# jlk9/MPAS-Ocean.jl

Hardware: AMD Instinct MI355X
Metric: cell-updates/sec per RK4 step (higher is better)
Workload: dtype f64

## Files before the change

### include/moka_hip.h

```cpp
#ifndef MOKA_HIP_H
#define MOKA_HIP_H
#include <stdint.h>

#ifdef __cplusplus
extern "C" {
#endif

typedef struct moka_ctx   moka_ctx;
typedef struct moka_plan  moka_plan;
typedef struct moka_mesh  moka_mesh;
typedef struct moka_state moka_state;

typedef enum {
    MOKA_OK = 0,
    MOKA_ERR_ARG = -1,
    MOKA_ERR_HIP = -2,
    MOKA_ERR_NO_DEVICE = -3,
    MOKA_ERR_ALLOC = -4,
    MOKA_ERR_UNSUPPORTED = -5,
    MOKA_ERR_COMM = -6
} moka_status;

typedef enum {
    MOKA_ORDER_DEFAULT = 0,
    MOKA_ORDER_NONE = 1,
    MOKA_ORDER_RCM = 2,
    MOKA_ORDER_RCB = 3
} moka_ordering;

typedef struct moka_mesh_desc {
    int32_t nCells, nEdges, nVertices;
    int32_t maxEdges, maxEdges2, vertexDegree;
    int32_t nVertLevels;
    int32_t edgeSignOnVertexLD;
    const double  *xCell, *yCell, *zCell;
    const int32_t *nEdgesOnCell;
    const int32_t *edgesOnCell;
    const int32_t *edgeSignOnCell;
    const double  *areaCell;
    const int32_t *cellsOnEdge;
    const int32_t *verticesOnEdge;
    const int32_t *nEdgesOnEdge;
    const int32_t *edgesOnEdge;
    const double  *weightsOnEdge;
    const double  *dvEdge, *dcEdge, *fEdge;
    const int32_t *edgesOnVertex;
    const int32_t *cellsOnVertex;
    const int32_t *edgeSignOnVertex;
    const double  *areaTriangle;
    const int32_t *maxLevelEdgeTop;
    const double  *restingThicknessSum;
    int32_t ordering;
    int32_t patch_cells;
    const int32_t *cellClass;
    int32_t stateBytes;
    const double *kiteAreasOnVertex;
    const double *fVertex;
} moka_mesh_desc;

typedef struct moka_mesh_info {
    int32_t nCells, nEdges, nVertices, nVertLevels;
    int32_t ordering, patch_cells, nPatches;
    int32_t maxEdgesUsed, maxEdges2Used;
    int32_t lanesPerColumn;
    int64_t meshBytesDevice;
    int64_t cellBandwidth;
    int32_t maxPatchRows;
    int32_t ldsBytesPerBlock;
    int32_t maxPatchCells, maxPatchEdges;
} moka_mesh_info;

enum { MOKA_CELL = 0, MOKA_EDGE = 1, MOKA_VERTEX = 2 };

typedef enum {
    MOKA_F_SSH = 0,
    MOKA_F_NORMAL_VELOCITY = 1,
    MOKA_F_LAYER_THICKNESS = 2,
    MOKA_F_LAYER_THICKNESS_EDGE = 3,
    MOKA_F_THICKNESS_FLUX = 4,
    MOKA_F_VELOCITY_DIV_CELL = 5,
    MOKA_F_RELATIVE_VORTICITY = 6,
    MOKA_F_TEND_NORMAL_VELOCITY = 7,
    MOKA_F_TEND_LAYER_THICKNESS = 8
} moka_field;

#define MOKA_FE_STALE_HEDGE      1
#define MOKA_FE_ACCUM_VORT       2
#define MOKA_FE_LEVEL1_ONLY      4
#define MOKA_FE_REFERENCE_COMPAT 7

typedef enum { MOKA_FORWARD_EULER = 0, MOKA_RUNGE_KUTTA_4 = 1 } moka_integrator;

const char *moka_version(void);
int  moka_ctx_create(int device, moka_ctx **out);
void moka_ctx_destroy(moka_ctx *ctx);
const char *moka_last_error(const moka_ctx *ctx);
int  moka_sync(moka_ctx *ctx);
int  moka_timer_start(moka_ctx *ctx);
int  moka_timer_stop(moka_ctx *ctx, float *elapsed_ms);

int  moka_plan_create(const moka_mesh_desc *desc, moka_plan **out);
void moka_plan_destroy(moka_plan *plan);
int  moka_plan_info(const moka_plan *plan, moka_mesh_info *info);
int  moka_plan_permutation(const moka_plan *plan, int kind, int32_t *new_to_old);
int  moka_plan_patch_ranges(const moka_plan *plan, int32_t *cellStart, int32_t *edgeStart, int32_t *vertexStart);
int  moka_plan_class_ranges(const moka_plan *plan, int32_t capacity, int32_t *nClasses, int32_t *patchStart,
                            int32_t *cellStart, int32_t *edgeStart);

enum {
    MOKA_PA_EOC = 0, MOKA_PA_COC, MOKA_PA_MLTC, MOKA_PA_SDV, MOKA_PA_INVAREA, MOKA_PA_AREACELL, MOKA_PA_RSUM,
    MOKA_PA_EHDR, MOKA_PA_EOE, MOKA_PA_WOE, MOKA_PA_GINVDC, MOKA_PA_DCEDGE, MOKA_PA_DVEDGE, MOKA_PA_FEDGE,
    MOKA_PA_EOV, MOKA_PA_CV, MOKA_PA_HALO_START, MOKA_PA_HALO_EDGE, MOKA_PA_LEOC, MOKA_PA_LEOE,
    MOKA_PA_CREC, MOKA_PA_EREC, MOKA_PA_FEOE, MOKA_PA_PVSTART, MOKA_PA_PVLIST, MOKA_PA_LVOE,
    MOKA_PA_NLEV
};
int  moka_plan_array(const moka_plan *plan, int which, const void **data, int64_t *count);

int  moka_mesh_create(moka_ctx *ctx, const moka_mesh_desc *desc, moka_mesh **out);
void moka_mesh_destroy(moka_mesh *mesh);
int  moka_mesh_info_get(const moka_mesh *mesh, moka_mesh_info *info);

int moka_gradient_on_edge(moka_mesh *mesh, const double *scalarCell, double *gradEdge);
int moka_divergence_on_cell(moka_mesh *mesh, const double *vecEdge, double *tempEdge, double *divCell);
int moka_curl_on_vertex(moka_mesh *mesh, const double *vecEdge, double *curlVertex);
int moka_interpolate_cell2edge(moka_mesh *mesh, const double *cellValue, double *edgeValue, int nlev);

int moka_gradient_on_edge_vjp(moka_mesh *mesh, double *dGradEdge , double *dScalarCell );
int moka_gradient_on_edge_jvp(moka_mesh *mesh, const double *dScalarCell, double *dGradEdge);
int moka_divergence_on_cell_vjp(moka_mesh *mesh, double *dDivCell , double *dVecEdge ,
                                double *dTempEdge );
int moka_divergence_on_cell_jvp(moka_mesh *mesh, const double *dVecEdge, double *dTempEdge , double *dDivCell);
int moka_curl_on_vertex_vjp(moka_mesh *mesh, const double *dCurlVertex, double *dVecEdge );
int moka_curl_on_vertex_jvp(moka_mesh *mesh, const double *dVecEdge, double *dCurlVertex );

int  moka_state_create(moka_ctx *ctx, moka_mesh *mesh, moka_state **out);
void moka_state_destroy(moka_state *st);
int  moka_state_upload(moka_state *st, int field, int time_level, const double *host);
int  moka_state_download(moka_state *st, int field, int time_level, double *host);

int  moka_state_download_rows(moka_state *st, int field, int time_level, int64_t nRows, const int32_t *rows, double *host);

int  moka_state_array_address(moka_state *st, int field, int time_level, uint64_t *address);

int  moka_state_optimize_placement(moka_state *st, int max_tries, double *ms_before, double *ms_after);
typedef struct { int32_t field; double ms_old, ms_new; int32_t kept; } moka_placement_trial;
int  moka_state_placement_log(const moka_state *st, int32_t capacity, moka_placement_trial *out, int32_t *n);
int64_t moka_state_placement_launches(const moka_state *st);

int moka_advance_time_levels(moka_state *st, int flags);
int moka_diagnostic_compute(moka_state *st, int flags);
int moka_compute_normal_velocity_tendency(moka_state *st, int flags);
int moka_compute_layer_thickness_tendency(moka_state *st, int flags);
int moka_tendencies(moka_state *st);
int moka_step_fe(moka_state *st, double dt, int flags);
int moka_step_rk4(moka_state *st, double dt);
int moka_run(moka_state *st, int integrator, double dt, int64_t nsteps, int flags);
int moka_sum_sq(moka_state *st, int field, int time_level, double *out);

typedef struct moka_halo moka_halo;
int  moka_ctx_streams(moka_ctx *ctx, void **compute_stream, void **comm_stream);
int  moka_mesh_permutation(const moka_mesh *mesh, int kind, int32_t *new_to_old);
int  moka_mesh_class_ranges(const moka_mesh *mesh, int32_t capacity, int32_t *nClasses, int32_t *patchStart,
                            int32_t *cellStart, int32_t *edgeStart);
int  moka_halo_create(moka_state *st, int32_t nNeighbors, const int32_t *sendCells, const int64_t *sendCellOff,
                      const int32_t *sendEdges, const int64_t *sendEdgeOff, const int32_t *recvCells,
                      const int64_t *recvCellOff, const int32_t *recvEdges, const int64_t *recvEdgeOff,
                      int32_t nPatchesBoundary, int32_t nPatchesOwned, moka_halo **out);
void moka_halo_destroy(moka_halo *h);
int  moka_halo_buffer_elems(const moka_halo *h, int64_t *sendElems, int64_t *recvElems);
int  moka_halo_pack(moka_halo *h, int what, void *sendbuf_device);
int  moka_halo_unpack(moka_halo *h, int what, const void *recvbuf_device);

typedef struct {
    unsigned char ipc[15][64];
    uint64_t ptr[15];
    uint64_t flagPtr;
    char     shmName[64];
    int32_t  dstCell, dstEdge;
    int32_t  nCells, nEdges;
    int32_t  slot;
    int32_t  nNeighbors, pid, device, stateBytes, nVertLevels;
} moka_halo_peer_info;
int  moka_halo_set_overlap(moka_halo *h, int mode);
int  moka_halo_set_acquire(moka_halo *h, int on);
int  moka_halo_pack_fields(moka_halo *h, const void *uField, const void *hField, const void *sField, void *sendbuf);
int  moka_halo_unpack_fields(moka_halo *h, void *uField, void *hField, void *sField, const void *recvbuf);
int  moka_halo_direct_available(const moka_halo *h);
int  moka_halo_export(moka_halo *h, int32_t nbr, int32_t shared, moka_halo_peer_info *out);
int  moka_halo_connect(moka_halo *h, int32_t nbr, const moka_halo_peer_info *peer, int32_t shared);
int  moka_halo_push_begin(moka_halo *h, int what);
int  moka_halo_push_signal(moka_halo *h);
int  moka_halo_push_wait(moka_halo *h, double timeout_s);

int  moka_halo_set_stream_flags(moka_halo *h, int on);

typedef struct {
    int64_t steps, exchanges, boundary_launches, interior_launches;
    double host_step_ms, host_signal_wait_ms, host_flag_store_ms, host_wait_ms, boundary_launch_ms, interior_launch_ms;
} moka_halo_stats;
int  moka_halo_stats_enable(moka_halo *h, int on);
int  moka_halo_stats_read(moka_halo *h, moka_halo_stats *out);

int  moka_rk4_dist_begin(moka_halo *h, double dt);
int  moka_rk4_dist_stage(moka_halo *h, int stage, int part);
int  moka_rk4_dist_parts_available(const moka_halo *h);
int  moka_rk4_dist_stage_launch(moka_halo *h, int stage);
int  moka_rk4_dist_end(moka_halo *h);
typedef int (*moka_transport_fn)(void *user, int what, void *sendbuf_device, void *recvbuf_device);
int  moka_rk4_dist_step(moka_halo *h, double dt, moka_transport_fn transport, void *user, void *sendbuf_device,
                        void *recvbuf_device, double timeout_s);
int  moka_fe_dist_launch(moka_halo *h, double dt, int flags, int part);
int  moka_fe_dist_end(moka_halo *h);
int  moka_fe_dist_step(moka_halo *h, double dt, int flags, moka_transport_fn transport, void *user, void *sendbuf_device,
                       void *recvbuf_device, double timeout_s);

int moka_kernel_variant_available(int variant);
int moka_set_kernel_variant(moka_ctx *ctx, int variant);
int moka_set_tuning(int key, int value);
int moka_get_tuning(int key, int *value);
int moka_state_rk4_streams(const moka_state *st);
int moka_stage_timing(moka_ctx *ctx, int enable);
int moka_stage_timing_read(moka_ctx *ctx, double ms[4], int64_t *steps);
int moka_ctx_pci_bus_id(moka_ctx *ctx, char *buf, int32_t len);
int moka_mark(moka_ctx *ctx);
int moka_marks_reset(moka_ctx *ctx);
int moka_marks_read(moka_ctx *ctx, int64_t capacity, double *ms, int64_t *n);
int moka_bw_probe(moka_ctx *ctx, int64_t bytes, int iters, double gbs[4]);
int moka_bw_probe_streams(moka_ctx *ctx, int iters, double *gbs);
int moka_bw_probe_reread(moka_ctx *ctx, int64_t region, int reps, int iters, double *gbs);
int moka_bw_probe_gather_big(moka_ctx *ctx, int64_t bytes, int iters, double *gbs);
int moka_last_fe_path(const moka_state *st);
int moka_fe_lazy_pending(const moka_state *st);

int  moka_set_nonlinear(moka_state *st, int on);
int  moka_set_viscosity_del2(moka_state *st, double viscDel2);
int  moka_set_viscosity_del4(moka_state *st, double viscDel4, const double *meshScalingDel4);
int  moka_state_del4_path(const moka_state *st);

int  moka_set_tracers(moka_state *st, int32_t nTracers);
int  moka_tracer_upload(moka_state *st, int32_t j, int time_level, const double *host);
int  moka_tracer_download(moka_state *st, int32_t j, int time_level, double *host);
int  moka_state_tracer_path(const moka_state *st);
int  moka_set_tracer_diffusion(moka_state *st, const double *kappa);
int  moka_tracer_diffusion(const moka_state *st, int32_t j, double *out);
int  moka_set_tracer_biharmonic(moka_state *st, const double *kappa4);
int  moka_tracer_biharmonic(const moka_state *st, int32_t j, double *out);
int  moka_tracer_source_upload(moka_state *st, int32_t j, const double *host);
int  moka_tracer_source_download(moka_state *st, int32_t j, double *host);
int  moka_tracer_has_source(const moka_state *st, int32_t j, int *out);
int  moka_set_tracer_vertical_diffusion(moka_state *st, const double *kappaV);
int  moka_tracer_vertical_diffusion(const moka_state *st, int32_t j, double *out);
int  moka_state_tracer_vmix_path(const moka_state *st);
int  moka_tracer_vertical_field_upload(moka_state *st, int32_t j, const double *host);
int  moka_tracer_vertical_field_download(moka_state *st, int32_t j, double *host);
int  moka_tracer_has_vertical_field(const moka_state *st, int32_t j, int *out);

int  moka_set_vertical_viscosity(moka_state *st, double nuV, double bottomDrag);
int  moka_vertical_viscosity(const moka_state *st, double *nuV, double *bottomDrag);
int  moka_surface_stress_upload(moka_state *st, const double *host);
int  moka_surface_stress_download(moka_state *st, double *host);
int  moka_has_surface_stress(const moka_state *st, int *out);
int  moka_state_momentum_vmix_path(const moka_state *st);

typedef struct moka_tracer_tape moka_tracer_tape;
int  moka_tracer_tape_create(moka_state *st, int64_t capacity_steps, moka_tracer_tape **out);
void moka_tracer_tape_destroy(moka_tracer_tape *t);
int  moka_step_rk4_tracer_taped(moka_tracer_tape *t, double dt);
int  moka_tracer_tape_steps(const moka_tracer_tape *t, int64_t *n);
int  moka_tracer_adjoint_seed(moka_tracer_tape *t, int32_t j, const double *host);
int  moka_tracer_adjoint_sweep(moka_tracer_tape *t);
int  moka_tracer_adjoint_download(moka_tracer_tape *t, int32_t j, double *host);
int  moka_tracer_adjoint_path(const moka_tracer_tape *t);
int  moka_tracer_adjoint_vmix_path(const moka_tracer_tape *t);
int  moka_tracer_adjoint_want_source_gradient(moka_tracer_tape *t, int32_t j, int on);
int  moka_tracer_adjoint_source_download(moka_tracer_tape *t, int32_t j, double *host);
enum { MOKA_TRACER_GRAD_KAPPA = 1, MOKA_TRACER_GRAD_KAPPA4 = 2 };
int  moka_tracer_adjoint_want_diffusivity_gradient(moka_tracer_tape *t, int32_t j, int what, int on);
int  moka_tracer_adjoint_diffusivity_gradient(moka_tracer_tape *t, int32_t j, int what, double *out);
int  moka_tracer_adjoint_diffusivity_density_download(moka_tracer_tape *t, int32_t j, int what, double *host);
int  moka_tracer_adjoint_want_vertical_gradient(moka_tracer_tape *t, int32_t j, int on);
int  moka_tracer_adjoint_vertical_gradient(moka_tracer_tape *t, int32_t j, double *out);
enum { MOKA_VGRAD_INTERFACE = 0, MOKA_VGRAD_CELL = 1, MOKA_VGRAD_PROFILE = 2 };
int  moka_tracer_adjoint_vertical_density_download(moka_tracer_tape *t, int32_t j, int view, double *host);

typedef struct moka_tape moka_tape;
int  moka_tape_create(moka_state *st, int64_t capacity_steps, moka_tape **out);
void moka_tape_destroy(moka_tape *t);
int  moka_step_fe_taped(moka_tape *t, double dt, int flags);
int  moka_step_rk4_taped(moka_tape *t, double dt);
int  moka_adjoint_seed_sum_sq_ssh(moka_tape *t);
int  moka_adjoint_sweep(moka_tape *t);
int  moka_tape_record_rk4(moka_tape *t, int slot, int what);
int  moka_tape_commit_rk4(moka_tape *t, double dt);
int  moka_adjoint_rk4_stage_fields(moka_tape *t, int stage, void **fieldU, void **fieldH, void **scratchS);
int  moka_adjoint_rk4_stage(moka_tape *t, int stage);
int  moka_adjoint_rk4_stage_part(moka_tape *t, int stage, int part);
int  moka_adjoint_rk4_parts_available(const moka_tape *t);
int  moka_adjoint_rk4_stage_out_fields(moka_tape *t, int stage, void **fieldU, void **fieldH, void **scratchS);
int  moka_tape_record_fe(moka_tape *t, int flags, int after);
int  moka_tape_commit_fe(moka_tape *t, double dt, int flags);
int  moka_adjoint_fe_step_fields(moka_tape *t, void **fieldU, void **fieldH, void **fieldS);
int  moka_adjoint_fe_step(moka_tape *t);
int  moka_adjoint_download(moka_tape *t, int field, double *host);

#ifdef __cplusplus
}
#endif
#endif
```

### mpas-ocean.jl_amd/csrc/api.hip

```cpp
#include <hip/hip_runtime.h>

#include <algorithm>
#include <atomic>
#include <climits>
#include <cmath>
#include <cstdio>
#include <cstdlib>
#include <cstring>
#include <map>
#include <mutex>
#include <new>
#include <string>
#include <unordered_set>
#include <utility>
#include <vector>

#include <mutex>
#include <unordered_set>

#include "state.hpp"

namespace moka {

void fill_mesh_info(const Plan &p, moka_mesh_info *info);

struct TuningEntry {
    int mask, max;
    std::atomic<int> value;
    TuningEntry(int def, int m, int x) : mask(m), max(x), value(def) {}
    bool accepts(int v) const { return mask ? (v & ~mask) == 0 : v >= 0 && v <= max; }
};
static TuningEntry g_tuning[] = {
    {0, 0, -1},
    {1 << 0, 0x7f | 1 << 10 | 1 << 11, 0},
    {1, 0, 1},
    {1, 0, 1},
    {1, 0, 1},
    {0, 0, 3},
    {0, 0, INT_MAX},
    {0, 0, 1},
    {1 << 0 | 1 << 1 | 1 << 7, 0xf | 7 << 7 | 1 << 16, 0},
    {1, 0, 1},
};
constexpr int N_TUNING = sizeof(g_tuning) / sizeof(g_tuning[0]);

int tuning(TuningKey key) { return g_tuning[key].value.load(); }

}

namespace mk {

static std::mutex g_liveMutex;
static std::unordered_set<const moka_state *> g_liveStates;
void state_attach(moka_state *st, bool halo)
{
    std::lock_guard<std::mutex> lk(g_liveMutex);
    if (g_liveStates.count(st)) { ++st->attached; st->halos += halo; }
}
void state_detach(moka_state *st, bool halo)
{
    std::lock_guard<std::mutex> lk(g_liveMutex);
    if (g_liveStates.count(st)) { --st->attached; st->halos -= halo; }
}

int fail(moka_ctx *ctx, int code, const std::string &msg)
{
    set_error(msg);
    if (ctx) ctx->err = msg;
    return code;
}

int lanes_per_column(int K)
{
    int l = 1;
    while (l < K && l < 64) l <<= 1;
    return l;
}

int h2d(moka_ctx *ctx, void *dst, const void *src, size_t bytes)
{
    if (!bytes) return MOKA_OK;
    HIPCHK(ctx, hipMemcpyAsync(dst, src, bytes, hipMemcpyHostToDevice, ctx->stream));
    HIPCHK(ctx, hipStreamSynchronize(ctx->stream));
    return MOKA_OK;
}

template <class T>
int upload_vec(moka_mesh *m, const std::vector<T> &v, const T **out)
{
    void *d = nullptr;
    const size_t bytes = std::max<size_t>(v.size() * sizeof(T), 16);
    HIPCHK(m->ctx, hipMalloc(&d, bytes));
    m->allocs.push_back(d);
    if (int rc = h2d(m->ctx, d, v.data(), v.size() * sizeof(T))) return rc;
    *out = static_cast<const T *>(d);
    return MOKA_OK;
}

int ensure_op_bufs(moka_mesh *m)
{
    const Plan &p = m->plan;
    const size_t need = (size_t)p.K * std::max(p.nE, std::max(p.nC, p.nV));
    if (m->opBufElems >= need) return MOKA_OK;
    for (auto &b : m->opBuf) {
        if (b) HIPCHK(m->ctx, hipFree(b));
        b = nullptr;
    }
    for (auto &b : m->opBuf) HIPCHK(m->ctx, hipMalloc((void **)&b, need * sizeof(double)));
    m->opBufElems = need;
    return MOKA_OK;
}

int alloc_field(moka_state *st, double **out, size_t elems, size_t elemBytes)
{
    void *d = nullptr;
    HIPCHK(st->ctx, hipMalloc(&d, std::max<size_t>(elems * elemBytes, 16)));
    st->allocs.push_back(d);
    HIPCHK(st->ctx, hipMemsetAsync(d, 0, elems * elemBytes, st->ctx->stream));
    *out = static_cast<double *>(d);
    return MOKA_OK;
}

int ensure_rk_bufs(moka_state *st)
{
    if (st->rk[1].ssh) return MOKA_OK;
    const Plan &p = st->mesh->plan;
    LevelBufs tmp[2];
    const size_t mark = st->allocs.size();
    const size_t sb = st->f32 ? 4 : 8;
    int rc = MOKA_OK;
    for (auto &r : tmp) {
        if (rc == MOKA_OK) rc = alloc_field(st, &r.u, (size_t)p.K * p.nE, sb);
        if (rc == MOKA_OK) rc = alloc_field(st, &r.h, (size_t)p.K * p.nC, sb);
        if (rc == MOKA_OK) rc = alloc_field(st, &r.ssh, (size_t)p.nC, sb);
    }
    if (rc != MOKA_OK) {
        (void)hipStreamSynchronize(st->ctx->stream);
        while (st->allocs.size() > mark) { (void)hipFree(st->allocs.back()); st->allocs.pop_back(); }
        return rc;
    }
    st->rk[0] = tmp[0]; st->rk[1] = tmp[1];
    st->phys[2] = tmp[0]; st->phys[3] = tmp[1];
    return MOKA_OK;
}

int ensure_spare(moka_state *st)
{
    if (st->spare.ssh) return MOKA_OK;
    const Plan &p = st->mesh->plan;
    LevelBufs tmp;
    const size_t mark = st->allocs.size();
    const size_t sb = st->f32 ? 4 : 8;
    int rc = alloc_field(st, &tmp.u, (size_t)p.K * p.nE, sb);
    if (rc == MOKA_OK) rc = alloc_field(st, &tmp.h, (size_t)p.K * p.nC, sb);
    if (rc == MOKA_OK) rc = alloc_field(st, &tmp.ssh, (size_t)p.nC, sb);
    if (rc != MOKA_OK) {
        (void)hipStreamSynchronize(st->ctx->stream);
        while (st->allocs.size() > mark) { (void)hipFree(st->allocs.back()); st->allocs.pop_back(); }
        return rc;
    }
    st->spare = tmp;
    st->phys[4] = tmp;
    return MOKA_OK;
}

LevelBufs &fe_new_level(moka_state *st) { return st->spare.ssh ? st->spare : st->lev[0]; }

void fe_rotate_levels(moka_state *st)
{
    if (st->spare.ssh) {
        const LevelBufs oldPrev = st->lev[0];
        st->lev[0] = st->lev[1];
        st->lev[1] = st->spare;
        st->spare = oldPrev;
    } else {
        std::swap(st->lev[0], st->lev[1]);
    }
}

struct FieldRef {
    double *ptr;
    int kind;
    int64_t n;
    int K;
    bool f32 = false;
};

int field_ref(moka_state *st, int field, int level, FieldRef *r)
{
    const Plan &p = st->mesh->plan;
    if (level != 0 && level != 1) return fail(st->ctx, MOKA_ERR_ARG, "time_level must be 0 (previous) or 1 (current)");
    switch (field) {
        case MOKA_F_SSH: *r = {st->lev[level].ssh, MOKA_CELL, p.nC, 1}; break;
        case MOKA_F_NORMAL_VELOCITY: *r = {st->lev[level].u, MOKA_EDGE, p.nE, p.K}; break;
        case MOKA_F_LAYER_THICKNESS: *r = {st->lev[level].h, MOKA_CELL, p.nC, p.K}; break;
        case MOKA_F_LAYER_THICKNESS_EDGE: *r = {st->hEdge[0], MOKA_EDGE, p.nE, p.K}; break;
        case MOKA_F_THICKNESS_FLUX: *r = {st->F, MOKA_EDGE, p.nE, p.K}; break;
        case MOKA_F_VELOCITY_DIV_CELL: *r = {st->div, MOKA_CELL, p.nC, p.K}; break;
        case MOKA_F_RELATIVE_VORTICITY: *r = {st->vort, MOKA_VERTEX, p.nV, p.K}; break;
// ... 365 lines not shown
    ctx->marksUsed = 0;
    return MOKA_OK;
}

int moka_marks_read(moka_ctx *ctx, int64_t capacity, double *ms, int64_t *n)
{
    if (!ctx || !n || (capacity > 0 && !ms)) return fail(ctx, MOKA_ERR_ARG, "NULL argument");
    HIPCHK(ctx, hipStreamSynchronize(ctx->stream));
    const int64_t have = ctx->marksUsed > 0 ? (int64_t)ctx->marksUsed - 1 : 0;
    *n = have;
    for (int64_t i = 0; i < have && i < capacity; ++i) {
        float t = 0.f;
        HIPCHK(ctx, hipEventElapsedTime(&t, ctx->marks[i], ctx->marks[i + 1]));
        ms[i] = t;
    }
    return MOKA_OK;
}

int moka_bw_probe(moka_ctx *ctx, int64_t bytes, int iters, double gbs[4])
{
    if (!ctx) return fail(nullptr, MOKA_ERR_ARG, "ctx is NULL");
    HIPCHK(ctx, hipSetDevice(ctx->device));
    if (bytes <= 0) {
        HIPCHK(ctx, hipStreamSynchronize(ctx->stream));
        if (ctx->bwBuf) HIPCHK(ctx, hipFree(ctx->bwBuf));
        ctx->bwBuf = nullptr; ctx->bwBytes = 0;
        return MOKA_OK;
    }
    if (!gbs || iters < 1) return fail(ctx, MOKA_ERR_ARG, "gbs is NULL or iters < 1");
    const size_t half = ((size_t)bytes / 2) & ~(size_t)4095;
    if (half < ((size_t)1 << 20)) return fail(ctx, MOKA_ERR_ARG, "bandwidth probe: at least 2 MiB");
    hipStream_t s = ctx->stream;
    if (ctx->bwBytes != 2 * half) {
        if (ctx->bwBuf) { HIPCHK(ctx, hipStreamSynchronize(s)); HIPCHK(ctx, hipFree(ctx->bwBuf)); ctx->bwBuf = nullptr; ctx->bwBytes = 0; }
        hipError_t e = hipMalloc(&ctx->bwBuf, 2 * half + 64);
        if (e != hipSuccess) return fail(ctx, MOKA_ERR_ALLOC, std::string("bandwidth probe: hipMalloc: ") + hipGetErrorString(e));
        ctx->bwBytes = 2 * half;
        HIPCHK(ctx, hipMemsetAsync(ctx->bwBuf, 0x5A, 2 * half + 64, s));
    }
    unsigned char *a = static_cast<unsigned char *>(ctx->bwBuf), *b = a + half;
    uint32_t *sink = reinterpret_cast<uint32_t *>(a + 2 * half);
    double bestCopy = 0.0, bestRead = 0.0, sumCopy = 0.0, bestGather = 0.0;
    const uint32_t rowB = 480;
    for (int pass = 0; pass < 3; ++pass)
        for (int i = 0; i < iters; ++i) {
            HIPCHK(ctx, hipEventRecord(ctx->ev0, s));
            if (pass == 0) HIPCHK(ctx, launch_bw_copy(b, a, (int64_t)half, ctx->nCUs, s));
            else if (pass == 1) HIPCHK(ctx, launch_bw_read(a, (int64_t)(2 * half), sink, ctx->nCUs, s));
            else HIPCHK(ctx, launch_bw_gather(a, (int64_t)(2 * half), rowB, sink, ctx->nCUs, s));
            HIPCHK(ctx, hipEventRecord(ctx->ev1, s));
            HIPCHK(ctx, hipEventSynchronize(ctx->ev1));
            float ms = 0.f;
            HIPCHK(ctx, hipEventElapsedTime(&ms, ctx->ev0, ctx->ev1));
            const double r = (double)(2 * half) / ((double)ms * 1e-3) / 1e9;
            if (pass == 0) { bestCopy = std::max(bestCopy, r); sumCopy += r; }
            else if (pass == 1) bestRead = std::max(bestRead, r);
            else bestGather = std::max(bestGather, (double)((2 * half) / rowB * rowB) / ((double)ms * 1e-3) / 1e9);
        }
    gbs[0] = bestCopy; gbs[1] = bestRead; gbs[2] = sumCopy / iters; gbs[3] = bestGather;
    return MOKA_OK;
}

int moka_bw_probe_streams(moka_ctx *ctx, int iters, double *gbs)
{
    if (!ctx || !gbs || iters < 1) return fail(ctx, MOKA_ERR_ARG, "NULL argument or iters < 1");
    if (!ctx->bwBuf || ctx->bwBytes < ((size_t)5 << 20)) return fail(ctx, MOKA_ERR_ARG, "moka_bw_probe first: it owns the buffer");
    HIPCHK(ctx, hipSetDevice(ctx->device));
    hipStream_t s = ctx->stream;
    const int64_t n = (int64_t)(ctx->bwBytes / 5 / 16);
    double best = 0.0;
    for (int i = 0; i < iters; ++i) {
        HIPCHK(ctx, hipEventRecord(ctx->ev0, s));
        HIPCHK(ctx, launch_bw_streams(ctx->bwBuf, (int64_t)ctx->bwBytes, s));
        HIPCHK(ctx, hipEventRecord(ctx->ev1, s));
        HIPCHK(ctx, hipEventSynchronize(ctx->ev1));
        float ms = 0.f;
        HIPCHK(ctx, hipEventElapsedTime(&ms, ctx->ev0, ctx->ev1));
        best = std::max(best, (double)(5 * 16 * n) / ((double)ms * 1e-3) / 1e9);
    }
    HIPCHK(ctx, hipMemsetAsync(ctx->bwBuf, 0x5A, ctx->bwBytes + 64, s));
    *gbs = best;
    return MOKA_OK;
}

int moka_bw_probe_reread(moka_ctx *ctx, int64_t region, int reps, int iters, double *gbs)
{
    if (!ctx || !gbs || iters < 1 || reps < 1) return fail(ctx, MOKA_ERR_ARG, "NULL argument or iters / reps < 1");
    if (!ctx->bwBuf || region < ((int64_t)1 << 20) || (size_t)region > ctx->bwBytes) return fail(ctx, MOKA_ERR_ARG, "moka_bw_probe first: it owns the buffer (region must fit it)");
    HIPCHK(ctx, hipSetDevice(ctx->device));
    hipStream_t s = ctx->stream;
    unsigned char *a = static_cast<unsigned char *>(ctx->bwBuf);
    uint32_t *sink = reinterpret_cast<uint32_t *>(a + ctx->bwBytes);
    region &= ~(int64_t)4095;
    double best = 0.0;
    HIPCHK(ctx, launch_bw_read(a, region, sink, ctx->nCUs, s));
    for (int i = 0; i < iters; ++i) {
        HIPCHK(ctx, hipEventRecord(ctx->ev0, s));
        for (int r = 0; r < reps; ++r) HIPCHK(ctx, launch_bw_read(a, region, sink, ctx->nCUs, s));
        HIPCHK(ctx, hipEventRecord(ctx->ev1, s));
        HIPCHK(ctx, hipEventSynchronize(ctx->ev1));
        float ms = 0.f;
        HIPCHK(ctx, hipEventElapsedTime(&ms, ctx->ev0, ctx->ev1));
        best = std::max(best, (double)region * reps / ((double)ms * 1e-3) / 1e9);
    }
    *gbs = best;
    return MOKA_OK;
}

int moka_bw_probe_gather_big(moka_ctx *ctx, int64_t bytes, int iters, double *gbs)
{
    if (!ctx || !gbs || iters < 1 || bytes < ((int64_t)1 << 24)) return fail(ctx, MOKA_ERR_ARG, "NULL argument, iters < 1 or less than 16 MiB");
    HIPCHK(ctx, hipSetDevice(ctx->device));
    hipStream_t s = ctx->stream;
    void *buf = nullptr;
    hipError_t e = hipMalloc(&buf, (size_t)bytes + 64);
    if (e != hipSuccess) return fail(ctx, MOKA_ERR_ALLOC, std::string("big gather probe: hipMalloc: ") + hipGetErrorString(e));
    const uint32_t rowB = 480;
    const int64_t nRows = bytes / rowB, nFetch = nRows / 4;
    uint32_t *sink = reinterpret_cast<uint32_t *>(static_cast<unsigned char *>(buf) + bytes);
    double best = 0.0;
    hipError_t rc = hipMemsetAsync(buf, 0x5A, (size_t)bytes + 64, s);
    for (int i = 0; i < iters && rc == hipSuccess; ++i) {
        if ((rc = hipEventRecord(ctx->ev0, s)) != hipSuccess) break;
        if ((rc = launch_bw_gather_n(buf, nRows, rowB, nFetch, sink, ctx->nCUs, s)) != hipSuccess) break;
        if ((rc = hipEventRecord(ctx->ev1, s)) != hipSuccess) break;
        if ((rc = hipEventSynchronize(ctx->ev1)) != hipSuccess) break;
        float ms = 0.f;
        if ((rc = hipEventElapsedTime(&ms, ctx->ev0, ctx->ev1)) != hipSuccess) break;
        best = std::max(best, (double)nFetch * rowB / ((double)ms * 1e-3) / 1e9);
    }
    (void)hipStreamSynchronize(s);
    (void)hipFree(buf);
    HIPCHK(ctx, rc);
    *gbs = best;
    return MOKA_OK;
}

int moka_set_tuning(int key, int value)
{
    if (key < 1 || key >= N_TUNING) return fail(nullptr, MOKA_ERR_ARG, "unknown tuning key");
    if (!g_tuning[key].accepts(value)) return fail(nullptr, MOKA_ERR_ARG, "tuning key " + std::to_string(key) + ": value names no kernel instance");
    g_tuning[key].value.store(value);
    return MOKA_OK;
}

int moka_get_tuning(int key, int *value)
{
    if (!value) return fail(nullptr, MOKA_ERR_ARG, "value is NULL");
    if (key < 1 || key >= N_TUNING) return fail(nullptr, MOKA_ERR_ARG, "unknown tuning key");
    *value = g_tuning[key].value.load();
    return MOKA_OK;
}

int moka_kernel_variant_available(int variant)
{
    return variant == 0 || variant == 3 || variant == 4 || variant == 11;
}

int moka_set_kernel_variant(moka_ctx *ctx, int variant)
{
    if (!ctx) return fail(nullptr, MOKA_ERR_ARG, "ctx is NULL");
    if (variant < 0 || variant > 14) return fail(ctx, MOKA_ERR_ARG, "variant must be 0..14");
    if (!moka_kernel_variant_available(variant))
        return fail(ctx, MOKA_ERR_UNSUPPORTED, "this kernel variant was an experiment of rounds 1-3 and no longer exists (0, 3, 4, 11 do)");
    ctx->variant = variant;
    return MOKA_OK;
}

int moka_mesh_create(moka_ctx *ctx, const moka_mesh_desc *desc, moka_mesh **out)
{
    if (!ctx || !out) return fail(ctx, MOKA_ERR_ARG, "NULL argument");
    *out = nullptr;
    moka_mesh *m = new (std::nothrow) moka_mesh();
    if (!m) return fail(ctx, MOKA_ERR_ALLOC, "out of host memory");
    m->ctx = ctx;
    int rc;
    try {
        rc = build_plan(desc, m->plan);
    } catch (const std::bad_alloc &) {
        rc = fail(ctx, MOKA_ERR_ALLOC, "out of host memory while building the mesh plan");
    }
    if (rc != MOKA_OK) {
        ctx->err = moka::get_error();
        delete m;
        return rc;
    }
    const Plan &p = m->plan;
    if (p.ME > 8 || p.ME2 > 14) {
        delete m;
        return fail(ctx, MOKA_ERR_UNSUPPORTED, "cells with more than 8 edges are not supported by the gfx950 kernels");
    }
    HIPCHK(ctx, hipSetDevice(ctx->device));
    MeshDev &d = m->dev;
    d.nC = p.nC; d.nE = p.nE; d.nV = p.nV; d.K = p.K; d.ME = p.ME; d.ME2 = p.ME2; d.VD = p.VD; d.nPatches = p.nPatches;
    d.tailPatch = -1;
    m->lpc = lanes_per_column(p.K);
#define UP(field)                                                \
    if ((rc = upload_vec(m, p.field, &d.field)) != MOKA_OK) {    \
        moka_mesh_destroy(m);                                    \
        return rc;                                               \
    }
    UP(patchCellStart) UP(patchEdgeStart) UP(patchVertStart)
    UP(eoc) UP(coc) UP(mltc) UP(sdv) UP(invArea) UP(areaCell) UP(rsum)
    UP(ehdr) UP(eoe) UP(woe) UP(gInvDc) UP(dcEdge) UP(dvEdge) UP(fEdge)
    UP(eov) UP(cv) UP(cellN2O) UP(edgeN2O) UP(vertN2O)
    UP(leoe) UP(cRec) UP(eRec) UP(feoe) UP(vRec) UP(rowStart) UP(rowEdge)
    if (p.nlOk) { UP(voe) UP(cov) UP(kite) UP(invAreaTri) UP(fVertex) UP(keCoef) UP(invDc) UP(keoc) UP(rowVoe) }
    if (p.nl5Ok) { UP(pvStart) UP(pvList) UP(lvoe) }
#undef UP
    d.maxPV = p.nl5Ok ? p.maxPV : 0;
    if (!p.nl5Ok) { d.pvStart = nullptr; d.pvList = nullptr; d.lvoe = nullptr; }
    d.CI = p.CI; d.EI = p.EI;
    m->colOk = p.colOk;

    d.maxRows = p.maxRows; d.maxOwnE = p.maxOwnE; d.maxOwnC = p.maxOwnC;
    d.maxOwnV = p.maxOwnV;
    if (p.vRec.empty()) d.vRec = nullptr;
    *out = m;
    return MOKA_OK;
}

void moka_mesh_destroy(moka_mesh *mesh)
{
    if (!mesh) return;
    (void)hipSetDevice(mesh->ctx->device);
    (void)hipStreamSynchronize(mesh->ctx->stream);
    for (void *q : mesh->allocs) (void)hipFree(q);
    for (auto b : mesh->opBuf)
        if (b) (void)hipFree(b);
    delete mesh;
}

int moka_mesh_permutation(const moka_mesh *mesh, int kind, int32_t *new_to_old)
{
    if (!mesh || !new_to_old) return fail(nullptr, MOKA_ERR_ARG, "NULL argument");
    const Plan &p = mesh->plan;
    const std::vector<int32_t> *v = kind == MOKA_CELL ? &p.cellN2O : kind == MOKA_EDGE ? &p.edgeN2O : kind == MOKA_VERTEX ? &p.vertN2O : nullptr;
    if (!v) return fail(mesh->ctx, MOKA_ERR_ARG, "kind must be MOKA_CELL, MOKA_EDGE or MOKA_VERTEX");
    std::copy(v->begin(), v->end(), new_to_old);
    return MOKA_OK;
}

int moka_mesh_class_ranges(const moka_mesh *mesh, int32_t capacity, int32_t *nClasses, int32_t *patchStart, int32_t *cellStart,
                           int32_t *edgeStart)
{
    if (!mesh || !nClasses) return fail(nullptr, MOKA_ERR_ARG, "NULL argument");
    const Plan &p = mesh->plan;
    const int n = (int)p.classPatchStart.size() - 1;
    *nClasses = n;
    for (int k = 0; k <= n && k < capacity; ++k) {
        if (patchStart) patchStart[k] = p.classPatchStart[k];
        if (cellStart) cellStart[k] = p.classCellStart[k];
        if (edgeStart) edgeStart[k] = p.classEdgeStart[k];
    }
    return MOKA_OK;
}

int moka_mesh_info_get(const moka_mesh *mesh, moka_mesh_info *info)
{
    if (!mesh || !info) return fail(nullptr, MOKA_ERR_ARG, "NULL argument");
    fill_mesh_info(mesh->plan, info);
    return MOKA_OK;
}

static int run_operator(moka_mesh *m, int op, int nlev, const double *in, int inKind, double *out, int outKind,
                        bool out_is_inout)
{
    if (!m || !in || !out) return fail(m ? m->ctx : nullptr, MOKA_ERR_ARG, "NULL argument");
    const Plan &p = m->plan;
    auto count = [&](int kind) -> int64_t { return kind == MOKA_CELL ? p.nC : kind == MOKA_EDGE ? p.nE : p.nV; };
    int rc = ensure_op_bufs(m);
    if (rc) return rc;
    hipStream_t s = m->ctx->stream;
    HIPCHK(m->ctx, hipSetDevice(m->ctx->device));
    if ((rc = put_rows(m, m->opBuf[0], in, inKind, count(inKind), p.K))) return rc;
    if (out_is_inout) {
        if ((rc = put_rows(m, m->opBuf[1], out, outKind, count(outKind), p.K))) return rc;
    } else {
        if (op == OP_INTERP && nlev < p.K) {
            if ((rc = put_rows(m, m->opBuf[1], out, outKind, count(outKind), p.K))) return rc;
        }
    }
    OpArgs a{op, nlev, m->opBuf[0], m->opBuf[1]};
    HIPCHK(m->ctx, launch_operator(m->dev, a, m->lpc, s));
    return get_rows(m, out, m->opBuf[1], outKind, count(outKind), p.K);
}

int moka_gradient_on_edge(moka_mesh *mesh, const double *scalarCell, double *gradEdge)
{
    return run_operator(mesh, OP_GRADIENT, 0, scalarCell, MOKA_CELL, gradEdge, MOKA_EDGE, false);
}

int moka_interpolate_cell2edge(moka_mesh *mesh, const double *cellValue, double *edgeValue, int nlev)
{
    if (mesh && (nlev < 1 || nlev > mesh->plan.K)) return fail(mesh->ctx, MOKA_ERR_ARG, "nlev out of range");
    return run_operator(mesh, OP_INTERP, nlev, cellValue, MOKA_CELL, edgeValue, MOKA_EDGE, false);
}

int moka_curl_on_vertex(moka_mesh *mesh, const double *vecEdge, double *curlVertex)
{
    return run_operator(mesh, OP_CURL, 0, vecEdge, MOKA_EDGE, curlVertex, MOKA_VERTEX, true);
}

static int ensure_op_transposes(moka_mesh *m)
{
    if (m->opESign) return MOKA_OK;
    const Plan &p = m->plan;
    std::vector<std::vector<std::pair<std::pair<int32_t, int32_t>, int32_t>>> lists(p.nE);
    for (int v = 0; v < p.nV; ++v)
        for (int j = 0; j < p.VD; ++j) {
            const int e = p.eov[(size_t)v * p.VD + j];
            if (e >= 0) lists[e].push_back({{p.vertN2O[v], j}, v});
        }
    int W = 1;
    for (auto &l : lists) { std::sort(l.begin(), l.end()); W = std::max(W, (int)l.size()); }
    std::vector<int32_t> tv((size_t)p.nE * W, -1);
    std::vector<double> tc((size_t)p.nE * W, 0.0), es((size_t)p.nE * 2, 0.0);
    for (int e = 0; e < p.nE; ++e) {
        for (size_t q = 0; q < lists[e].size(); ++q) {
            const int v = lists[e][q].second, j = lists[e][q].first.second;
            tv[(size_t)e * W + q] = v;
            tc[(size_t)e * W + q] = p.cv[(size_t)v * p.VD + j];
        }
        for (int q = 0; q < 2; ++q) {
            const int c = p.ehdr[(size_t)e * 4 + q];
            for (int i = 0; i < p.ME; ++i)
                if (p.eoc[(size_t)c * p.ME + i] == e) { es[(size_t)e * 2 + q] = p.sdv[(size_t)c * p.ME + i] < 0.0 ? -1.0 : 1.0; break; }
        }
    }
    int rc;
    if ((rc = upload_vec(m, tv, &m->opTVert)) || (rc = upload_vec(m, tc, &m->opTCoef))) return rc;
    if ((rc = upload_vec(m, es, &m->opESign))) return rc;
    m->opTW = W;
    return MOKA_OK;
}

int moka_gradient_on_edge_vjp(moka_mesh *m, double *dGradEdge, double *dScalarCell)
{
    if (!m || !dGradEdge || !dScalarCell) return fail(m ? m->ctx : nullptr, MOKA_ERR_ARG, "NULL argument");
    const Plan &p = m->plan;
    int rc = ensure_op_bufs(m);
    if (rc) return rc;
    HIPCHK(m->ctx, hipSetDevice(m->ctx->device));
    if ((rc = put_rows(m, m->opBuf[0], dGradEdge, MOKA_EDGE, p.nE, p.K))) return rc;
    if ((rc = put_rows(m, m->opBuf[1], dScalarCell, MOKA_CELL, p.nC, p.K))) return rc;
    OpArgs a{OP_GRAD_T, 0, m->opBuf[0], m->opBuf[1]};
    HIPCHK(m->ctx, launch_operator(m->dev, a, m->lpc, m->ctx->stream));
    if ((rc = get_rows(m, dScalarCell, m->opBuf[1], MOKA_CELL, p.nC, p.K))) return rc;
    std::memset(dGradEdge, 0, sizeof(double) * (size_t)p.K * p.nE);
    return MOKA_OK;
}

int moka_gradient_on_edge_jvp(moka_mesh *m, const double *dScalarCell, double *dGradEdge)
{
    return moka_gradient_on_edge(m, dScalarCell, dGradEdge);
}

int moka_divergence_on_cell_vjp(moka_mesh *m, double *dDivCell, double *dVecEdge, double *dTempEdge)
{
    if (!m || !dDivCell || !dVecEdge) return fail(m ? m->ctx : nullptr, MOKA_ERR_ARG, "NULL argument");
    const Plan &p = m->plan;
    int rc = ensure_op_bufs(m);
    if (rc) return rc;
    HIPCHK(m->ctx, hipSetDevice(m->ctx->device));
    if ((rc = ensure_op_transposes(m))) return rc;
    if ((rc = put_rows(m, m->opBuf[0], dDivCell, MOKA_CELL, p.nC, p.K))) return rc;
    if ((rc = put_rows(m, m->opBuf[1], dVecEdge, MOKA_EDGE, p.nE, p.K))) return rc;
    if (dTempEdge && (rc = put_rows(m, m->opBuf[3], dTempEdge, MOKA_EDGE, p.nE, p.K))) return rc;
    OpArgs a{OP_DIV_T, 0, m->opBuf[0], m->opBuf[1]};
    a.in2 = dTempEdge ? m->opBuf[3] : nullptr;
// ... 2286 lines not shown
```

### mpas-ocean.jl_amd/csrc/kernels.hip

```cpp
#include <mutex>
#include <set>
#include <utility>

#include "kernels_common.hpp"

namespace moka {


template <int ME, int ME2, int MODE, int NT = BLOCK>
__global__ __launch_bounds__(NT) void k_stage_rec2c(const ColMesh m, const StageArgs a, int maxOwnE, int maxOwnC)
{
    extern __shared__ __align__(16) unsigned char smem[];
    const int pl_ = patch_of_block(m.nPatches);
    if (pl_ >= m.nPatches) return;
    const int p = m.pairEnd ? m.patchBegin + 2 * pl_ : (m.tailPlus1 && pl_ == m.nPatches - 1) ? m.tailPlus1 - 1 : pl_ + m.patchBegin;
    const int pEnd = m.pairEnd ? (p + 2 < m.pairEnd ? p + 2 : m.pairEnd) : p + 1;
    constexpr int NG = NT / 32;
    const int tid = threadIdx.x;
    const int grp = tid >> 5, l = tid & 31;
    const int K = m.K, K2 = K >> 1;
    const uint32_t voff = (uint32_t)l * 16u, rowB = (uint32_t)K * 8u;
    const RecLds L = rec_carve(smem, m, ME, ME2, maxOwnE, maxOwnC);
    const size_t recBytes = ((size_t)maxOwnE * (2 * ME2 + 1) * 8 + (size_t)maxOwnC * (ME + 2) * 8 +
                             ((size_t)maxOwnE * m.EI + (size_t)maxOwnC * m.CI) * 4 + 15) & ~(size_t)15;
    double2 *ubuf2 = reinterpret_cast<double2 *>(smem + recBytes);
    const unsigned char *ubytes = reinterpret_cast<const unsigned char *>(ubuf2) + voff;
    const int c0 = cptr(m.patchCellStart)[p], c1 = cptr(m.patchCellStart)[pEnd];
    const int e0 = cptr(m.patchEdgeStart)[p], e1 = cptr(m.patchEdgeStart)[pEnd];
    const int nOwnC = c1 - c0, nOwnE = e1 - e0;
    const uint32_t e0B = (uint32_t)e0 * rowB, nOwnB = (uint32_t)nOwnE * rowB;
    double *Lvw = reinterpret_cast<double *>(smem + recBytes + (size_t)maxOwnE * rowB);
    uint32_t *Lvo = reinterpret_cast<uint32_t *>(Lvw + (size_t)m.maxOwnV * 3);
    constexpr bool LEAN = MODE >= 10;
    constexpr int BASE = LEAN ? MODE - 5 : MODE;
    constexpr bool FE = BASE >= 4 && BASE <= 6, STALE = BASE == 4, PREV = BASE == 6;
    int v0 = 0, nOwnV = 0;
    if constexpr (FE) {
        if (a.vort) {
            v0 = cptr(m.patchVertStart)[p];
            nOwnV = cptr(m.patchVertStart)[p + 1] - v0;
        }
    }

    {
        const double2 *src = reinterpret_cast<const double2 *>(a.pu) + (size_t)e0 * K2;
        const int nU = nOwnE * K2, nER = nOwnE * m.EI, nW = nOwnE * ME2, nCR = nOwnC * m.CI, nS = nOwnC * ME;
        constexpr int UU = 6, UE = 3, UW = 2;
        double2 vU[UU];
        uint32_t vE[UE], vC;
        double vW[UW], vF[UW], vG, vS, vA, vR;
#pragma unroll
        for (int j = 0; j < UU; ++j) vU[j] = (tid + j * NT < nU) ? src[tid + j * NT] : make_double2(0.0, 0.0);
#pragma unroll
        for (int j = 0; j < UE; ++j) vE[j] = (tid + j * NT < nER) ? m.eRec[(size_t)e0 * m.EI + tid + j * NT] : 0u;
#pragma unroll
        for (int j = 0; j < UW; ++j) {
            vW[j] = (tid + j * NT < nW) ? m.woe[(size_t)e0 * ME2 + tid + j * NT] : 0.0;
            vF[j] = (tid + j * NT < nW) ? m.feoe[(size_t)e0 * ME2 + tid + j * NT] : 0.0;
        }
        vG = tid < nOwnE ? m.gInvDc[e0 + tid] : 0.0;
        vC = tid < nCR ? m.cRec[(size_t)c0 * m.CI + tid] : 0u;
        vS = tid < nS ? m.sdv[(size_t)c0 * ME + tid] : 0.0;
        vA = tid < nOwnC ? m.invArea[c0 + tid] : 0.0;
        vR = tid < nOwnC ? m.rsum[c0 + tid] : 0.0;
        uint32_t vVo = 0u;
        double vVw = 0.0;
        if constexpr (FE) {
            if (tid < nOwnV * 4) vVo = m.vRec[(size_t)v0 * 4 + tid];
            if (tid < nOwnV * 3) vVw = m.cv[(size_t)v0 * 3 + tid];
        }
#pragma unroll
        for (int j = 0; j < UU; ++j) if (tid + j * NT < nU) ubuf2[tid + j * NT] = vU[j];
#pragma unroll
        for (int j = 0; j < UE; ++j) if (tid + j * NT < nER) L.eRec[tid + j * NT] = vE[j];
#pragma unroll
        for (int j = 0; j < UW; ++j)
            if (tid + j * NT < nW) {
                L.woe[tid + j * NT] = vW[j];
                L.feoe[tid + j * NT] = vF[j];
            }
        if (tid < nOwnE) L.g[tid] = vG;
        if (tid < nCR) L.cRec[tid] = vC;
        if (tid < nS) L.sdv[tid] = vS;
        if (tid < nOwnC) {
            L.invA[tid] = vA;
            L.rsum[tid] = vR;
        }
        if constexpr (FE) {
            if (tid < nOwnV * 4) Lvo[tid] = vVo;
            if (tid < nOwnV * 3) Lvw[tid] = vVw;
            for (int i = tid + NT; i < nOwnV * 4; i += NT) Lvo[i] = m.vRec[(size_t)v0 * 4 + i];
            for (int i = tid + NT; i < nOwnV * 3; i += NT) Lvw[i] = m.cv[(size_t)v0 * 3 + i];
        }
        for (int i = tid + UU * NT; i < nU; i += NT) ubuf2[i] = src[i];
        for (int i = tid + UE * NT; i < nER; i += NT) L.eRec[i] = m.eRec[(size_t)e0 * m.EI + i];
        for (int i = tid + UW * NT; i < nW; i += NT) {
            L.woe[i] = m.woe[(size_t)e0 * ME2 + i];
            L.feoe[i] = m.feoe[(size_t)e0 * ME2 + i];
        }
        for (int i = tid + NT; i < nOwnE; i += NT) L.g[i] = m.gInvDc[e0 + i];
        for (int i = tid + NT; i < nCR; i += NT) L.cRec[i] = m.cRec[(size_t)c0 * m.CI + i];
        for (int i = tid + NT; i < nS; i += NT) L.sdv[i] = m.sdv[(size_t)c0 * ME + i];
        for (int i = tid + NT; i < nOwnC; i += NT) {
            L.invA[i] = m.invArea[c0 + i];
            L.rsum[i] = m.rsum[c0 + i];
        }
    }
    __syncthreads();

    const int k0 = 2 * l;
    const bool act = k0 < K;
    const lds_bytes_t ubytesL = (lds_bytes_t)ubytes;
    const glb_bytes_t puG = (glb_bytes_t)a.pu;
    const uint32_t ldsU = (uint32_t)(size_t)ubytesL;
    auto urow_addr = [&](uint32_t off, bool &cached) -> uint32_t {
        const uint32_t loc = off - e0B;
        cached = loc < nOwnB;
        return ldsU + (cached ? loc : 0u);
    };

    double2 pA = make_double2(0.0, 0.0), pB = pA, pD = pA, pE = pA;
    double pS = 0.0;
    uint32_t pOff = 0;
    int pC = 0;
    bool pend = false;
    auto flush_cell = [&]() {
        if (act) {
            if constexpr (MODE == 0) gstore2o(a.tendH, pOff, pA);
            if constexpr (MODE == 1 || MODE == 2) {
                gstore2o(a.ph_out, pOff, pA);
                gstore2o(a.nh_out, pOff, pB);
            }
            if constexpr (MODE == 3 || MODE == 9) gstore2o(a.nh_out, pOff, pB);
            if constexpr (MODE == 7 || MODE == 8) gstore2o(a.ph_out, pOff, pA);
            if constexpr (LEAN) gstore2o(a.ph_out, pOff, pA);
            if constexpr (FE && !LEAN) {
                if (a.ph_out) gstore2o(a.ph_out, pOff, pA);
                if (a.tendH) gstore2o(a.tendH, pOff, pB);
                if (a.div) gstore2o(a.div, pOff, pD);
            }
        }
        if constexpr (MODE != 0)
            if (l == 0 && (!FE || LEAN || a.ssh_out)) a.ssh_out[pC] = pS;
    };
#pragma nounroll
    for (int ci = grp; ci < nOwnC; ci += NG) {
        const int c = c0 + ci;
        const uint32_t *r = L.cRec + (size_t)ci * m.CI;
        const double *rs = L.sdv + (size_t)ci * ME;
        const uint32_t mask = r[2 * ME], all = r[2 * ME + 1];
        const double invA = L.invA[ci];
        const uint32_t own = (uint32_t)c * rowB + voff;
        double2 hc = make_double2(0.0, 0.0), uv[ME], hv[ME], cur = hc, nin = hc, hpc = hc, q3 = hc;
        if (act) {
            bool cached[ME];
            uint32_t ad[ME], goff[ME];
            v4u_t raw[ME];
            hc = gload2(a.ph, own);
            if constexpr (PREV) hpc = gload2(a.hPrev, own);
#pragma unroll
            for (int i = 0; i < ME; ++i) {
                const uint32_t off = r[i];
                hv[i] = STALE ? gload2(a.hEdgeOld, off + voff) : gload2(PREV ? a.hPrev : a.ph, r[ME + i] + voff);
                ad[i] = urow_addr(off, cached[i]);
                goff[i] = off + voff;
                asm("" : "+v"(goff[i]));
            }
            lds_burst<ME>(raw, ad);
#pragma unroll
            for (int i = 0; i < ME; ++i) {
                uv[i] = __builtin_bit_cast(double2, raw[i]);
                if (!cached[i]) uv[i] = glb_row2(puG + goff[i]);
            }
            if constexpr (MODE == 2 || MODE == 8 || MODE == 9) cur = gload2(a.ch, own);
            if constexpr (MODE == 2 || MODE == 3 || MODE == 9) nin = gload2(a.nh_in, own);
            if constexpr (MODE == 9) q3 = gload2(a.q3h, own);
        }
        double area = 1.0;
        if constexpr (FE && !LEAN) if (a.div) area = a.areaCell[c];
        __builtin_amdgcn_s_waitcnt(0x0F70);
        if (pend) flush_cell();
        double2 t = make_double2(0.0, 0.0);
        const bool plain = __builtin_amdgcn_ballot_w64(!(mask == (1u << ME) - 1u && all)) == 0;
        double2 dv = make_double2(0.0, 0.0);
        const double2 hself = PREV ? hpc : hc;
        auto hE = [&](int i) { return STALE ? hv[i] : make_double2(0.5 * (hself.x + hv[i].x), 0.5 * (hself.y + hv[i].y)); };
        if (plain) {
            if (act) {
#pragma unroll
                for (int i = 0; i < ME; ++i) {
                    const double2 he = hE(i);
                    t.x += uv[i].x * he.x * rs[i] * invA;
                    t.y += uv[i].y * he.y * rs[i] * invA;
                    if constexpr (FE && !LEAN) {
                        dv.x -= uv[i].x * rs[i];
                        dv.y -= uv[i].y * rs[i];
                    }
                }
            }
        } else if (act) {
#pragma unroll
            for (int i = 0; i < ME; ++i) {
                const int ml = all ? K : cptr(m.mltc)[(size_t)c * ME + i];
                const bool on = (mask >> i) & 1u;
                const double2 he = hE(i);
                const double dx = uv[i].x * he.x * rs[i] * invA;
                const double dy = uv[i].y * he.y * rs[i] * invA;
                if (on && k0 < ml) t.x += dx;
                if (on && k0 + 1 < ml) t.y += dy;
                if constexpr (FE && !LEAN) {
                    if (on) {
                        dv.x -= uv[i].x * rs[i];
                        dv.y -= uv[i].y * rs[i];
                    }
                }
            }
        }
        double2 hs = make_double2(0.0, 0.0);
        if (act) {
            if constexpr (MODE == 0) pA = t;
            if constexpr (MODE == 1 || MODE == 2) {
                const double2 hcur = MODE == 2 ? cur : hc;
                const double2 nb = MODE == 2 ? nin : hcur;
                hs = make_double2(hcur.x + a.a * t.x, hcur.y + a.a * t.y);
                pA = hs;
                pB = make_double2(nb.x + a.b * t.x, nb.y + a.b * t.y);
            }
            if constexpr (MODE == 3) {
                hs = make_double2(nin.x + a.b * t.x, nin.y + a.b * t.y);
                pB = hs;
            }
            if constexpr (MODE == 7 || MODE == 8) {
                const double2 hcur = MODE == 8 ? cur : hc;
                hs = make_double2(hcur.x + a.a * t.x, hcur.y + a.a * t.y);
                pA = hs;
            }
            if constexpr (MODE == 9) {
                hs = make_double2(rk13_combine(cur.x, nin.x, q3.x, hc.x, a.b, t.x), rk13_combine(cur.y, nin.y, q3.y, hc.y, a.b, t.y));
                pB = hs;
            }
            if constexpr (FE) {
                hs = make_double2(hc.x + a.a * t.x, hc.y + a.a * t.y);
                pA = hs;
                if constexpr (!LEAN) {
                    pB = t;
                    if (a.div) pD = make_double2(dv.x / area, dv.y / area);
                }
            }
        }
        if constexpr (MODE != 0) {
#pragma unroll
            for (int sft = 16; sft >= 1; sft >>= 1) {
                const double ox = __shfl_xor(hs.x, sft, 32), oy = __shfl_xor(hs.y, sft, 32);
                hs = make_double2(hs.x + ox, hs.y + oy);
            }
            pS = (hs.x + hs.y) - L.rsum[ci];
        }
        pOff = own;
        pC = c;
        pend = true;
    }
    if (pend) flush_cell();
    pend = false;
    auto flush_edge = [&]() {
        if (act) {
            if constexpr (MODE == 0) gstore2o(a.tendU, pOff, pA);
            if constexpr (MODE == 1 || MODE == 2) {
                gstore2o(a.pu_out, pOff, pA);
                gstore2o(a.nu_out, pOff, pB);
            }
            if constexpr (MODE == 3 || MODE == 9) gstore2o(a.nu_out, pOff, pB);
            if constexpr (MODE == 7 || MODE == 8) gstore2o(a.pu_out, pOff, pA);
            if constexpr (LEAN) gstore2o(a.pu_out, pOff, pA);
            if constexpr (FE && !LEAN) {
                if (a.pu_out) gstore2o(a.pu_out, pOff, pA);
                if (a.tendU) gstore2o(a.tendU, pOff, pB);
                if (a.F) gstore2o(a.F, pOff, pD);
                if (a.hEdgeNew) gstore2o(a.hEdgeNew, pOff, pE);
            }
        }
    };

#pragma nounroll
    for (int ei = grp; ei < nOwnE; ei += NG) {
        const int e = e0 + ei;
        const uint32_t *r = L.eRec + (size_t)ei * m.EI;
        const double *rw = L.woe + (size_t)ei * ME2;
        const double *rf = L.feoe + (size_t)ei * ME2;
        const uint32_t mask = r[ME2 + 2];
        const int mlt = (int)r[ME2 + 3];
        const double g = L.g[ei];
        const uint32_t own = (uint32_t)e * rowB + voff;
        double sv = 0.0;
        double2 uv[ME2], cur = make_double2(0.0, 0.0), nin = cur, hx = cur, hy = cur, hEo = cur, q3 = cur;
        if (act) {
            bool cached[ME2];
            uint32_t ad[ME2], goff[ME2];
            v4u_t raw[ME2];
#pragma unroll
            for (int i = 0; i < ME2; ++i) {
                const uint32_t off = r[i];
                ad[i] = urow_addr(off, cached[i]);
                goff[i] = off + voff;
                asm("" : "+v"(goff[i]));
            }
            lds_burst<ME2>(raw, ad);
#pragma unroll
            for (int i = 0; i < ME2; ++i) {
                uv[i] = __builtin_bit_cast(double2, raw[i]);
                if (!cached[i]) uv[i] = glb_row2(puG + goff[i]);
            }
            if constexpr (MODE == 2 || MODE == 8 || MODE == 9) cur = gload2(a.cu, own);
            if constexpr (MODE == 2 || MODE == 3 || MODE == 9) nin = gload2(a.nu_in, own);
            if constexpr (MODE == 9) q3 = gload2(a.q3u, own);
            if constexpr (FE && !LEAN) {
                if (a.hEdgeNew || (MODE == 5 && a.F)) {
                    hx = gload2(a.ph, r[ME2] * rowB + voff);
                    hy = gload2(a.ph, r[ME2 + 1] * rowB + voff);
                }
                if (a.F) {
                    if constexpr (STALE) hEo = gload2(a.hEdgeOld, own);
                    if constexpr (PREV) {
                        const double2 px = gload2(a.hPrev, r[ME2] * rowB + voff), py = gload2(a.hPrev, r[ME2 + 1] * rowB + voff);
                        hEo = make_double2(0.5 * (px.x + py.x), 0.5 * (px.y + py.y));
                    }
                }
            }
        }
        if (l < 2) sv = a.ssh[r[ME2 + l]];
        __builtin_amdgcn_s_waitcnt(0x0F70);
        if (pend) flush_edge();
        const double ds = __shfl(sv, 1, 32) - __shfl(sv, 0, 32);
        const bool plain = __builtin_amdgcn_ballot_w64(!(mask == (1u << ME2) - 1u && mlt >= K)) == 0;
        if (act) {
            const bool ax = k0 < mlt, ay = k0 + 1 < mlt;
            double2 t = make_double2(0.0, 0.0);
            if (plain) {
                t.x -= g * ds;
                t.y -= g * ds;
#pragma unroll
                for (int i = 0; i < ME2; ++i) {
                    t.x += rw[i] * uv[i].x * rf[i];
                    t.y += rw[i] * uv[i].y * rf[i];
                }
            } else {
                if (ax) t.x -= g * ds;
                if (ay) t.y -= g * ds;
#pragma unroll
                for (int i = 0; i < ME2; ++i) {
                    const bool on = (mask >> i) & 1u;
                    const double px = rw[i] * uv[i].x * rf[i], py = rw[i] * uv[i].y * rf[i];
                    if (on && ax) t.x += px;
                    if (on && ay) t.y += py;
                }
            }
            if constexpr (MODE == 0) pA = t;
            if constexpr (MODE == 1) {
                const double2 up = ubuf2[(size_t)ei * K2 + l];
                pA = make_double2(up.x + a.a * t.x, up.y + a.a * t.y);
                pB = make_double2(up.x + a.b * t.x, up.y + a.b * t.y);
            }
            if constexpr (MODE == 2) {
                pA = make_double2(cur.x + a.a * t.x, cur.y + a.a * t.y);
                pB = make_double2(nin.x + a.b * t.x, nin.y + a.b * t.y);
            }
            if constexpr (MODE == 3) pB = make_double2(nin.x + a.b * t.x, nin.y + a.b * t.y);
            if constexpr (MODE == 7) {
                const double2 up = ubuf2[(size_t)ei * K2 + l];
                pA = make_double2(up.x + a.a * t.x, up.y + a.a * t.y);
            }
            if constexpr (MODE == 8) pA = make_double2(cur.x + a.a * t.x, cur.y + a.a * t.y);
            if constexpr (MODE == 9) {
                const double2 up = ubuf2[(size_t)ei * K2 + l];
                pB = make_double2(rk13_combine(cur.x, nin.x, q3.x, up.x, a.b, t.x), rk13_combine(cur.y, nin.y, q3.y, up.y, a.b, t.y));
            }
            if constexpr (LEAN) {
                const double2 up = ubuf2[(size_t)ei * K2 + l];
                pA = make_double2(up.x + a.a * t.x, up.y + a.a * t.y);
            }
            if constexpr (FE && !LEAN) {
                const double2 up = ubuf2[(size_t)ei * K2 + l];
                pE = make_double2(0.5 * (hx.x + hy.x), 0.5 * (hx.y + hy.y));
                const double2 hF = (STALE || PREV) ? hEo : pE;
                pD = make_double2(up.x * hF.x, up.y * hF.y);
                pA = make_double2(up.x + a.a * t.x, up.y + a.a * t.y);
                pB = t;
            }
        }
        pOff = own;
        pend = true;
    }
    if (pend) flush_edge();

    if constexpr (FE) {
#pragma nounroll
        for (int vi = grp; vi < nOwnV; vi += NG) {
            if (!act) continue;
            const uint32_t *rv = Lvo + (size_t)vi * 4;
            const double *wv = Lvw + (size_t)vi * 3;
            const uint32_t own = (uint32_t)(v0 + vi) * rowB + voff;
            bool cached[3];
            uint32_t ad[3], goff[3];
            v4u_t raw[3];
            double2 uv[3];
#pragma unroll
            for (int j = 0; j < 3; ++j) {
                const uint32_t off = rv[j];
                ad[j] = urow_addr(off, cached[j]);
                goff[j] = off + voff;
                asm("" : "+v"(goff[j]));
            }
            double2 c = a.accumVort ? gload2(a.vort, own) : make_double2(0.0, 0.0);
            lds_burst<3>(raw, ad);
#pragma unroll
            for (int j = 0; j < 3; ++j) {
                uv[j] = __builtin_bit_cast(double2, raw[j]);
                if (!cached[j]) uv[j] = glb_row2(puG + goff[j]);
            }
#pragma unroll
            for (int j = 0; j < 3; ++j) {
                c.x += wv[j] * uv[j].x;
                c.y += wv[j] * uv[j].y;
            }
            gstore2(a.vort, own, c);
        }
    }
}

struct d4 {
    double x, y, z, w;
};
__device__ __forceinline__ d4 widen4(float4 v) { return d4{(double)v.x, (double)v.y, (double)v.z, (double)v.w}; }
__device__ __forceinline__ float4 narrow4(d4 v) { return make_float4((float)v.x, (float)v.y, (float)v.z, (float)v.w); }
__device__ __forceinline__ float4 gload4f(const double *base, uint32_t off)
{
    return *reinterpret_cast<const float4 *>(reinterpret_cast<const char *>(base) + off);
}
__device__ __forceinline__ d4 gload4(const double *base, uint32_t off)
{
    return widen4(*reinterpret_cast<const float4 *>(reinterpret_cast<const char *>(base) + off));
}
__device__ __forceinline__ void gstore4(double *base, uint32_t off, d4 v)
{
    *reinterpret_cast<float4 *>(reinterpret_cast<char *>(base) + off) = narrow4(v);
}
__device__ __forceinline__ d4 axpy4(d4 x, double a, d4 t)
{
    return d4{x.x + a * t.x, x.y + a * t.y, x.z + a * t.z, x.w + a * t.w};
}
__device__ __forceinline__ d4 round4(d4 v) { return widen4(narrow4(v)); }

template <int ME, int ME2, int MODE, int NT = BLOCK, int WPE = 3>
__global__ __launch_bounds__(NT, WPE) void k_stage_rec2c_f32(const ColMesh m, const StageArgs a, int maxOwnE, int maxOwnC)
{
    extern __shared__ __align__(16) unsigned char smem[];
    const int pl_ = patch_of_block(m.nPatches);
    if (pl_ >= m.nPatches) return;
    const int p = (m.tailPlus1 && pl_ == m.nPatches - 1) ? m.tailPlus1 - 1 : pl_ + m.patchBegin;
    const int tid = threadIdx.x;
    const int K = m.K, K4 = K >> 2;
    const int EPW = 64 / K4, NG = (NT / 64) * EPW;
    const int lane = tid & 63, sub = lane / K4;
    const int l = lane - sub * K4, gbase = sub * K4;
    const bool lane_on = sub < EPW;
    const int grp = lane_on ? (tid >> 6) * EPW + sub : (1 << 28);
    auto gxor = [&](double v, int sft) -> double {
        const int pl = l ^ sft;
        const double o = __shfl(v, gbase + (pl < K4 ? pl : l), 64);
        return pl < K4 ? o : 0.0;
    };
    const uint32_t voff = (uint32_t)l * 16u, rowB = (uint32_t)K * 4u;
    const RecLds L = rec_carve(smem, m, ME, ME2, maxOwnE, maxOwnC);
    const size_t recBytes = ((size_t)maxOwnE * (2 * ME2 + 1) * 8 + (size_t)maxOwnC * (ME + 2) * 8 +
                             ((size_t)maxOwnE * m.EI + (size_t)maxOwnC * m.CI) * 4 + 15) & ~(size_t)15;
    float4 *ubuf4 = reinterpret_cast<float4 *>(smem + recBytes);
    const unsigned char *ubytes = reinterpret_cast<const unsigned char *>(ubuf4) + voff;
    const int c0 = cptr(m.patchCellStart)[p], c1 = cptr(m.patchCellStart)[p + 1];
    const int e0 = cptr(m.patchEdgeStart)[p], e1 = cptr(m.patchEdgeStart)[p + 1];
    const int nOwnC = c1 - c0, nOwnE = e1 - e0;
    const uint32_t e0B = (uint32_t)e0 * rowB, nOwnB = (uint32_t)nOwnE * rowB;
    const float *sshf = reinterpret_cast<const float *>(a.ssh);
    double *Lvw = reinterpret_cast<double *>(smem + recBytes + (((size_t)maxOwnE * rowB + 15) & ~(size_t)15));
    uint32_t *Lvo = reinterpret_cast<uint32_t *>(Lvw + (size_t)m.maxOwnV * 3);
    constexpr bool LEAN = MODE >= 10;
    constexpr int BASE = LEAN ? MODE - 5 : MODE;
    int v0 = 0, nOwnV = 0;
    if constexpr (BASE >= 4) {
        if (a.vort) {
            v0 = cptr(m.patchVertStart)[p];
            nOwnV = cptr(m.patchVertStart)[p + 1] - v0;
        }
    }

    {
        const float4 *src = reinterpret_cast<const float4 *>(a.pu) + (size_t)e0 * K4;
        const int nU = nOwnE * K4, nER = nOwnE * m.EI, nW = nOwnE * ME2, nCR = nOwnC * m.CI, nS = nOwnC * ME;
        constexpr int UU = 6, UE = 4, UW = 3, UC = 2;
        float4 vU[UU];
        uint32_t vE[UE], vC[UC];
        double vW[UW], vF[UW], vG, vS, vA, vR;
#pragma unroll
        for (int j = 0; j < UU; ++j) vU[j] = (tid + j * NT < nU) ? src[tid + j * NT] : make_float4(0.f, 0.f, 0.f, 0.f);
#pragma unroll
        for (int j = 0; j < UE; ++j) vE[j] = (tid + j * NT < nER) ? m.eRec[(size_t)e0 * m.EI + tid + j * NT] : 0u;
// ... 790 lines not shown

hipError_t launch_bw_streams(void *buf, int64_t bytes, hipStream_t s)
{
    const int64_t n = bytes / 5 / 16;
    bw_v4u *p = static_cast<bw_v4u *>(buf);
    hipLaunchKernelGGL(k_bw_streams, dim3((unsigned)((n + BLOCK - 1) / BLOCK)), dim3(BLOCK), 0, s, p + 3 * n, p + 4 * n, p, p + n, p + 2 * n, n);
    return hipGetLastError();
}

hipError_t launch_bw_copy(void *dst, const void *src, int64_t bytes, int, hipStream_t s)
{
    const int64_t n = bytes / 16;
    hipLaunchKernelGGL(k_bw_copy, dim3((unsigned)((n + BLOCK - 1) / BLOCK)), dim3(BLOCK), 0, s, static_cast<bw_v4u *>(dst),
                       static_cast<const bw_v4u *>(src), n);
    return hipGetLastError();
}

hipError_t launch_bw_read(const void *src, int64_t bytes, uint32_t *sink, int, hipStream_t s)
{
    const int64_t n = bytes / 16;
    hipLaunchKernelGGL(k_bw_read, dim3((unsigned)((n + 4 * BLOCK - 1) / (4 * BLOCK))), dim3(BLOCK), 0, s, static_cast<const bw_v4u *>(src), n, sink);
    return hipGetLastError();
}

hipError_t launch_bw_gather(const void *src, int64_t bytes, uint32_t rowB, uint32_t *sink, int nCUs, hipStream_t s)
{
    const int64_t nRows = bytes / rowB;
    hipLaunchKernelGGL(k_bw_gather, dim3((unsigned)(nCUs * 16)), dim3(BLOCK), 0, s, static_cast<const unsigned char *>(src), nRows, rowB, nRows, sink);
    return hipGetLastError();
}

hipError_t launch_bw_gather_n(const void *src, int64_t nRows, uint32_t rowB, int64_t nFetch, uint32_t *sink, int nCUs, hipStream_t s)
{
    hipLaunchKernelGGL(k_bw_gather, dim3((unsigned)(nCUs * 16)), dim3(BLOCK), 0, s, static_cast<const unsigned char *>(src), nRows, rowB, nFetch, sink);
    return hipGetLastError();
}

template <int LPC>
static hipError_t launch_fe_lpc(const MeshDev &m, const FeArgs &a, hipStream_t s)
{
    const dim3 g(patch_grid(m)), b(BLOCK);
    if (m.ME == 6 && m.ME2 == 10) hipLaunchKernelGGL((k_fe<LPC, 6, 10>), g, b, 0, s, m, a);
    else if (m.ME == 8 && m.ME2 == 14) hipLaunchKernelGGL((k_fe<LPC, 8, 14>), g, b, 0, s, m, a);
    else if (m.ME <= 6 && m.ME2 <= 14) hipLaunchKernelGGL((k_fe<LPC, 6, 14>), g, b, 0, s, m, a);
    else return hipErrorInvalidValue;
    return hipGetLastError();
}


template <int ME, int ME2, int NT>
static bool launch_rec2c_nt(const ColMesh &m, const StageArgs &a, int mode, dim3 g, size_t lds, int mE, int mC, hipStream_t s)
{
    const dim3 b(NT);
    switch (mode) {
        case 0: hipLaunchKernelGGL((k_stage_rec2c<ME, ME2, 0, NT>), g, b, lds, s, m, a, mE, mC); return true;
        case 1: hipLaunchKernelGGL((k_stage_rec2c<ME, ME2, 1, NT>), g, b, lds, s, m, a, mE, mC); return true;
        case 2: hipLaunchKernelGGL((k_stage_rec2c<ME, ME2, 2, NT>), g, b, lds, s, m, a, mE, mC); return true;
        case 3: hipLaunchKernelGGL((k_stage_rec2c<ME, ME2, 3, NT>), g, b, lds, s, m, a, mE, mC); return true;
        case 4: hipLaunchKernelGGL((k_stage_rec2c<ME, ME2, 4, NT>), g, b, lds, s, m, a, mE, mC); return true;
        case 5: hipLaunchKernelGGL((k_stage_rec2c<ME, ME2, 5, NT>), g, b, lds, s, m, a, mE, mC); return true;
        case 6: hipLaunchKernelGGL((k_stage_rec2c<ME, ME2, 6, NT>), g, b, lds, s, m, a, mE, mC); return true;
        case 7: hipLaunchKernelGGL((k_stage_rec2c<ME, ME2, 7, NT>), g, b, lds, s, m, a, mE, mC); return true;
        case 8: hipLaunchKernelGGL((k_stage_rec2c<ME, ME2, 8, NT>), g, b, lds, s, m, a, mE, mC); return true;
        case 9: hipLaunchKernelGGL((k_stage_rec2c<ME, ME2, 9, NT>), g, b, lds, s, m, a, mE, mC); return true;
        case 10: hipLaunchKernelGGL((k_stage_rec2c<ME, ME2, 10, NT>), g, b, lds, s, m, a, mE, mC); return true;
        case 11: hipLaunchKernelGGL((k_stage_rec2c<ME, ME2, 11, NT>), g, b, lds, s, m, a, mE, mC); return true;
    }
    return false;
}

template <int ME, int ME2>
static bool launch_rec2c(const ColMesh &m, const StageArgs &a, int mode, dim3 g, dim3, size_t lds, int mE, int mC, hipStream_t s)
{
    if (m.nPatches <= 512) return launch_rec2c_nt<ME, ME2, 512>(m, a, mode, g, lds, mE, mC, s);
    return launch_rec2c_nt<ME, ME2, BLOCK>(m, a, mode, g, lds, mE, mC, s);
}

hipError_t raise_dyn_lds(std::initializer_list<const void *> fns, int bytes)
{
    static std::mutex mu;
    static std::set<std::pair<int, const void *>> done;
    int dev = 0;
    if (hipError_t e = hipGetDevice(&dev); e != hipSuccess) return e;
    std::lock_guard<std::mutex> lk(mu);
    for (const void *fn : fns) {
        if (done.count({dev, fn})) continue;
        if (hipError_t e = hipFuncSetAttribute(fn, hipFuncAttributeMaxDynamicSharedMemorySize, bytes); e != hipSuccess) return e;
        done.insert({dev, fn});
    }
    return hipSuccess;
}

template <int ME, int ME2>
static hipError_t launch_rec2c_pair(const ColMesh &m, const StageArgs &a, int mode, dim3 g, size_t lds, int mE, int mC, hipStream_t s)
{
    const dim3 b(512);
#define PAIR_CASE(M)                                                                                                   \
    case M:                                                                                                            \
        if (lds > 64 * 1024)                                                                                           \
            if (hipError_t e = raise_dyn_lds({(const void *)k_stage_rec2c<ME, ME2, M, 512>}, 160 * 1024); e != hipSuccess) \
                return e;                                                                                              \
        hipLaunchKernelGGL((k_stage_rec2c<ME, ME2, M, 512>), g, b, lds, s, m, a, mE, mC);                               \
        return hipGetLastError();
    switch (mode) {
        PAIR_CASE(0) PAIR_CASE(1) PAIR_CASE(2) PAIR_CASE(3) PAIR_CASE(7) PAIR_CASE(8) PAIR_CASE(9)
    }
#undef PAIR_CASE
    return hipErrorNotSupported;
}

size_t rec2c_lds_bytes(const MeshDev &md)
{
    return ((rec_lds_bytes(md) + 15) & ~(size_t)15) + (size_t)md.maxOwnE * md.K * 8 + 16;
}

static inline size_t vert_lds_bytes(const MeshDev &md) { return (size_t)md.maxOwnV * (3 * 8 + 4 * 4) + 16; }

bool stage_curl_fused(const MeshDev &md)
{
    return tuning(TUNE_CURL_FUSED) && md.vRec != nullptr && md.VD == 3 && md.patchVertStart != nullptr && md.maxOwnV > 0;
}

bool stage_curl_fits(const MeshDev &md, bool f32)
{
    if (!stage_curl_fused(md)) return false;
    const size_t rows = (size_t)md.maxOwnE * md.K * (f32 ? 4 : 8);
    const size_t lds = ((rec_lds_bytes(md) + 15) & ~(size_t)15) + rows + 16 + vert_lds_bytes(md) + 16;
    return f32 ? (stage_f32_supported(md) && lds <= 160 * 1024) : (rec2c_supported(md) && lds <= 64 * 1024);
}

static inline ColMesh col_mesh(const MeshDev &md, int nLaunch)
{
    return ColMesh{md.nC, md.nE, md.K, nLaunch, md.patchBegin, md.CI, md.EI, md.patchCellStart, md.patchEdgeStart,
                   md.cRec, md.eRec, md.mltc, md.sdv, md.invArea, md.rsum, md.woe, md.feoe, md.gInvDc, md.tailPatch >= 0 ? md.tailPatch + 1 : 0,
                   md.patchVertStart, md.vRec, md.cv, md.maxOwnV, 0};
}

bool rec2c_supported(const MeshDev &md)
{
    const bool shape = (md.ME == 6 && md.ME2 == 10) || (md.ME == 8 && md.ME2 == 14) || (md.ME <= 6 && md.ME2 <= 14);
    return md.cRec && md.eRec && md.K <= 64 && !(md.K & 1) && rec2c_lds_bytes(md) <= 64 * 1024 && md.maxOwnC >= 1 && md.maxOwnE >= 1 && shape;
}

hipError_t launch_stage_rec2c(const MeshDev &md, const StageArgs &a, hipStream_t s)
{
    const int nLaunch = md.nPatches + (md.tailPatch >= 0 ? 1 : 0);
    const dim3 g(8 * ((nLaunch + 7) / 8)), b(BLOCK);
    const ColMesh m = col_mesh(md, nLaunch);
    int mode = colp_mode(a);
    if (a.vort && (mode < 4 || !stage_curl_fused(md))) return hipErrorNotSupported;
    if (tuning(TUNE_FE_LEAN_INST) && colp_lean(a, mode)) mode += 5;
    const size_t lds = rec2c_lds_bytes(md) + (a.vort ? vert_lds_bytes(md) : 0);
    if (mode < 0 || md.K > 64 || (md.K & 1) || lds > 64 * 1024 || md.maxOwnC < 1 || md.maxOwnE < 1) return hipErrorNotSupported;
    const int pair = tuning(TUNE_PAIR);
    if (((pair >> mode) & 1) && md.tailPatch < 0 && (md.nPatches >= 4096 || ((pair >> 16) & 1)) && md.nPatches >= 2 &&
        md.ME == 6 && md.ME2 == 10) {
        MeshDev two = md;
        two.maxOwnE = 2 * md.maxOwnE; two.maxOwnC = 2 * md.maxOwnC;
        const size_t lds2 = rec2c_lds_bytes(two);
        if (2 * lds2 + 2048 <= 160 * 1024) {
            const int nPair = (md.nPatches + 1) / 2;
            ColMesh mp = col_mesh(md, nPair);
            mp.pairEnd = md.patchBegin + md.nPatches;
            const hipError_t e = launch_rec2c_pair<6, 10>(mp, a, mode, dim3(8 * ((nPair + 7) / 8)), lds2, two.maxOwnE, two.maxOwnC, s);
            if (e != hipErrorNotSupported) return e;
        }
    }
    bool ok = false;
    if (md.ME == 6 && md.ME2 == 10) ok = launch_rec2c<6, 10>(m, a, mode, g, b, lds, md.maxOwnE, md.maxOwnC, s);
    else if (md.ME == 8 && md.ME2 == 14) ok = launch_rec2c<8, 14>(m, a, mode, g, b, lds, md.maxOwnE, md.maxOwnC, s);
    else if (md.ME <= 6 && md.ME2 <= 14) ok = launch_rec2c<6, 14>(m, a, mode, g, b, lds, md.maxOwnE, md.maxOwnC, s);
    return ok ? hipGetLastError() : hipErrorNotSupported;
}

template <int ME, int ME2, int NT, int WPE>
static hipError_t launch_rec2c_f32_nt(const ColMesh &m, const StageArgs &a, int mode, dim3 g, size_t lds, int mE, int mC, hipStream_t s)
{
    if (lds > 64 * 1024) {
        const hipError_t e = raise_dyn_lds({(const void *)k_stage_rec2c_f32<ME, ME2, 0, NT, WPE>, (const void *)k_stage_rec2c_f32<ME, ME2, 1, NT, WPE>,
                                            (const void *)k_stage_rec2c_f32<ME, ME2, 2, NT, WPE>, (const void *)k_stage_rec2c_f32<ME, ME2, 3, NT, WPE>,
                                            (const void *)k_stage_rec2c_f32<ME, ME2, 4, NT, WPE>, (const void *)k_stage_rec2c_f32<ME, ME2, 5, NT, WPE>,
                                            (const void *)k_stage_rec2c_f32<ME, ME2, 6, NT, WPE>, (const void *)k_stage_rec2c_f32<ME, ME2, 10, NT, WPE>,
                                            (const void *)k_stage_rec2c_f32<ME, ME2, 11, NT, WPE>},
                                           160 * 1024);
        if (e != hipSuccess) return e;
    }
    const dim3 b(NT);
    switch (mode) {
        case 0: hipLaunchKernelGGL((k_stage_rec2c_f32<ME, ME2, 0, NT, WPE>), g, b, lds, s, m, a, mE, mC); return hipGetLastError();
        case 1: hipLaunchKernelGGL((k_stage_rec2c_f32<ME, ME2, 1, NT, WPE>), g, b, lds, s, m, a, mE, mC); return hipGetLastError();
        case 2: hipLaunchKernelGGL((k_stage_rec2c_f32<ME, ME2, 2, NT, WPE>), g, b, lds, s, m, a, mE, mC); return hipGetLastError();
        case 3: hipLaunchKernelGGL((k_stage_rec2c_f32<ME, ME2, 3, NT, WPE>), g, b, lds, s, m, a, mE, mC); return hipGetLastError();
        case 4: hipLaunchKernelGGL((k_stage_rec2c_f32<ME, ME2, 4, NT, WPE>), g, b, lds, s, m, a, mE, mC); return hipGetLastError();
        case 5: hipLaunchKernelGGL((k_stage_rec2c_f32<ME, ME2, 5, NT, WPE>), g, b, lds, s, m, a, mE, mC); return hipGetLastError();
        case 6: hipLaunchKernelGGL((k_stage_rec2c_f32<ME, ME2, 6, NT, WPE>), g, b, lds, s, m, a, mE, mC); return hipGetLastError();
        case 10: hipLaunchKernelGGL((k_stage_rec2c_f32<ME, ME2, 10, NT, WPE>), g, b, lds, s, m, a, mE, mC); return hipGetLastError();
        case 11: hipLaunchKernelGGL((k_stage_rec2c_f32<ME, ME2, 11, NT, WPE>), g, b, lds, s, m, a, mE, mC); return hipGetLastError();
    }
    return hipErrorNotSupported;
}

template <int ME, int ME2>
static hipError_t launch_rec2c_f32(const ColMesh &m, const StageArgs &a, int mode, dim3 g, size_t lds, int mE, int mC, hipStream_t s)
{
    if (((tuning(TUNE_F32_WIDE) >> mode) & 1) && 2 * lds <= 160 * 1024)
        return launch_rec2c_f32_nt<ME, ME2, 512, 4>(m, a, mode, g, lds, mE, mC, s);
    return launch_rec2c_f32_nt<ME, ME2, BLOCK, 3>(m, a, mode, g, lds, mE, mC, s);
}

bool stage_f32_supported(const MeshDev &md)
{
    const size_t lds = ((rec_lds_bytes(md) + 15) & ~(size_t)15) + (size_t)md.maxOwnE * md.K * 4 + 16;
    const bool shape = (md.ME == 6 && md.ME2 == 10) || (md.ME == 8 && md.ME2 == 14) || (md.ME <= 6 && md.ME2 <= 14);
    return md.cRec && md.eRec && md.K >= 4 && md.K <= 128 && (md.K & 3) == 0 && lds <= 160 * 1024 && md.maxOwnC >= 1 &&
           md.maxOwnE >= 1 && shape;
}

hipError_t launch_stage_rec2c_f32(const MeshDev &md, const StageArgs &a, hipStream_t s)
{
    const int nLaunch = md.nPatches + (md.tailPatch >= 0 ? 1 : 0);
    const dim3 g(8 * ((nLaunch + 7) / 8));
    const ColMesh m = col_mesh(md, nLaunch);
    int mode = colp_mode(a);
    if (mode < 0 || !stage_f32_supported(md)) return hipErrorNotSupported;
    if (a.vort && (mode < 4 || !stage_curl_fused(md))) return hipErrorNotSupported;
    if (tuning(TUNE_FE_LEAN_INST) && colp_lean(a, mode)) mode += 5;
    const size_t lds = ((rec_lds_bytes(md) + 15) & ~(size_t)15) + (size_t)md.maxOwnE * md.K * 4 + 16 + (a.vort ? vert_lds_bytes(md) + 16 : 0);
    if (lds > 160 * 1024) return hipErrorNotSupported;
    if (md.ME == 6 && md.ME2 == 10) return launch_rec2c_f32<6, 10>(m, a, mode, g, lds, md.maxOwnE, md.maxOwnC, s);
    if (md.ME == 8 && md.ME2 == 14) return launch_rec2c_f32<8, 14>(m, a, mode, g, lds, md.maxOwnE, md.maxOwnC, s);
    if (md.ME <= 6 && md.ME2 <= 14) return launch_rec2c_f32<6, 14>(m, a, mode, g, lds, md.maxOwnE, md.maxOwnC, s);
    return hipErrorNotSupported;
}

hipError_t launch_curl2(const MeshDev &m, const double *u, double *vort, bool accum, hipStream_t s)
{
    if (m.K > 64 || (m.K & 1) || (size_t)std::max(m.nE, m.nV) * m.K * 8 >= ((size_t)1 << 32)) return hipErrorNotSupported;
    if (m.VD == 3) hipLaunchKernelGGL((k_curl3<3>), dim3(patch_grid(m)), dim3(BLOCK), 0, s, m, u, vort, accum ? 1 : 0);
    else hipLaunchKernelGGL(k_curl2, dim3(patch_grid(m)), dim3(BLOCK), 0, s, m, u, vort, accum ? 1 : 0);
    return hipGetLastError();
}

hipError_t launch_curl_f32(const MeshDev &m, const float *u, float *vort, bool accum, hipStream_t s)
{
    if ((m.K & 3) || m.VD != 3) return hipErrorNotSupported;
    hipLaunchKernelGGL((k_curl3_f32<3>), dim3(patch_grid(m)), dim3(BLOCK), 0, s, m, u, vort, accum ? 1 : 0);
    return hipGetLastError();
}

hipError_t launch_fe(const MeshDev &m, const FeArgs &a, int lpc, hipStream_t s)
{
#define CALL(L) launch_fe_lpc<L>(m, a, s)
    DISPATCH_LPC(lpc, CALL)
#undef CALL
}

template <int LPC>
static hipError_t launch_operator_lpc(const MeshDev &m, const OpArgs &a, hipStream_t s)
{
    hipLaunchKernelGGL((k_operator<LPC>), dim3(patch_grid(m)), dim3(BLOCK), 0, s, m, a);
    return hipGetLastError();
}

hipError_t launch_operator(const MeshDev &m, const OpArgs &a, int lpc, hipStream_t s)
{
#define CALL(L) launch_operator_lpc<L>(m, a, s)
    DISPATCH_LPC(lpc, CALL)
#undef CALL
}

template <int LPC, class T>
static hipError_t launch_update_ssh_lpc(const MeshDev &m, const T *h, T *ssh, int nlev, hipStream_t s)
{
    const int ng = BLOCK / LPC;
    int grid = (m.nC + ng - 1) / ng;
    if (grid > 16384) grid = 16384;
    hipLaunchKernelGGL((k_update_ssh<LPC, T>), dim3(grid), dim3(BLOCK), 0, s, m, h, ssh, nlev);
    return hipGetLastError();
}

hipError_t launch_update_ssh(const MeshDev &m, const double *h, double *ssh, int nlev, int lpc, hipStream_t s)
{
#define CALL(L) launch_update_ssh_lpc<L, double>(m, h, ssh, nlev, s)
    DISPATCH_LPC(lpc, CALL)
#undef CALL
}

hipError_t launch_update_ssh_f32(const MeshDev &m, const float *h, float *ssh, int nlev, int lpc, hipStream_t s)
{
#define CALL(L) launch_update_ssh_lpc<L, float>(m, h, ssh, nlev, s)
    DISPATCH_LPC(lpc, CALL)
#undef CALL
}

hipError_t launch_permute_rows(double *dst, const double *src, const int32_t *n2o, int64_t n, int K, int to_device,
                               hipStream_t s)
{
    int64_t blocks = (n * K + BLOCK - 1) / BLOCK;
    if (blocks > 65536) blocks = 65536;
    if (blocks < 1) blocks = 1;
    hipLaunchKernelGGL(k_permute_rows, dim3((unsigned)blocks), dim3(BLOCK), 0, s, dst, src, n2o, n, K, to_device);
    return hipGetLastError();
}

hipError_t launch_sum_sq_serial(const double *a, int64_t n, double *out, hipStream_t s)
{
    hipLaunchKernelGGL(k_sum_sq_serial, dim3(1), dim3(64), 0, s, a, n, out);
    return hipGetLastError();
}

hipError_t launch_pack_rows(double *buf, const double *field, const int32_t *rows, int64_t n, int K, int unpack, hipStream_t s)
{
    if (n <= 0) return hipSuccess;
    int64_t blocks = (n * K + BLOCK - 1) / BLOCK;
    if (blocks > 16384) blocks = 16384;
    hipLaunchKernelGGL(k_pack_rows, dim3((unsigned)blocks), dim3(BLOCK), 0, s, buf, const_cast<double *>(field), rows, n, K, unpack);
    return hipGetLastError();
}
// ... 42 lines not shown
```

### mpas-ocean.jl_amd/csrc/kernels.hpp

```cpp
#pragma once
#include <hip/hip_runtime.h>

#include <initializer_list>

#include "moka_internal.hpp"

namespace moka {

struct StageArgs {
    const double *pu, *ph;
    const double *ssh;
    const double *cu, *ch;
    const double *nu_in, *nh_in;
    double *nu_out, *nh_out;
    double *pu_out, *ph_out;
    double *ssh_out;
    double *tendU, *tendH;
    double a, b;
    int feMode;
    const double *hEdgeOld;
    const double *hPrev;
    double *hEdgeNew, *F, *div;
    const double *areaCell;
    double *vort;
    int accumVort;
    int rkMode;
    const double *q3u, *q3h;
};

struct ColMesh {
    int32_t nC, nE, K, nPatches, patchBegin, CI, EI;
    const int32_t *patchCellStart, *patchEdgeStart;
    const uint32_t *cRec, *eRec;
    const int32_t *mltc;
    const double *sdv, *invArea, *rsum, *woe, *feoe, *gInvDc;
    int32_t tailPlus1;
    const int32_t *patchVertStart;
    const uint32_t *vRec;
    const double *cv;
    int32_t maxOwnV;
    int32_t pairEnd;
};

enum : int {
    FE_FLUX = 1, FE_DIV = 2, FE_CURL = 4, FE_HEDGE = 8, FE_TENDU = 16, FE_TENDH = 32, FE_UPDATE = 64,
    FE_TENDH_FROM_F = 128
};

struct FeArgs {
    int ops, flags, nlev;
    double dt;
    const double *u, *h, *ssh;
    const double *hEdgeOld;
    const double *Fin;
    double *hEdgeNew, *F, *div, *vort, *tendU, *tendH;
    double *u_new, *h_new, *ssh_new;
};

enum : int { OP_GRADIENT = 0, OP_INTERP = 1, OP_DIV_P1 = 2, OP_DIV_P2 = 3, OP_CURL = 4, OP_GRAD_T = 5, OP_DIV_T = 6, OP_CURL_T = 7 };

struct OpArgs {
    int op, nlev;
    const double *in;
    double *out;
    const double *in2 = nullptr;
    const int32_t *auxI = nullptr;
    const double *auxD = nullptr;
    int auxW = 0;
};

hipError_t launch_stage(const MeshDev &m, const StageArgs &a, int lpc, hipStream_t s);
hipError_t launch_stage_col(const MeshDev &m, const StageArgs &a, hipStream_t s);
hipError_t launch_stage_rec2c(const MeshDev &m, const StageArgs &a, hipStream_t s);
bool rec2c_supported(const MeshDev &m);
bool stage_curl_fused(const MeshDev &m);
bool stage_curl_fits(const MeshDev &m, bool f32);
bool stage_f32_supported(const MeshDev &m);
hipError_t launch_stage_rec2c_f32(const MeshDev &m, const StageArgs &a, hipStream_t s);

enum TuningKey : int {
    TUNE_F32_WIDE = 1,
    TUNE_FE_PREV = 2,
    TUNE_CURL_FUSED = 3,
    TUNE_FE_LEAN = 4,
    TUNE_NL_SHAPE = 5,
    TUNE_NL_CAP = 6,
    TUNE_RK13 = 7,
    TUNE_PAIR = 8,
    TUNE_FE_LEAN_INST = 9,
};
int tuning(TuningKey key);

hipError_t raise_dyn_lds(std::initializer_list<const void *> fns, int bytes);
hipError_t launch_update_ssh_f32(const MeshDev &m, const float *h, float *ssh, int nlev, int lpc, hipStream_t s);
hipError_t launch_permute_rows_f32(void *dst, const void *src, const int32_t *n2o, int64_t n, int K, int to_device,
                                   hipStream_t s);
hipError_t launch_halo_map_f32(float *buf, float *h, float *ssh, float *u, const uint32_t *map, int64_t n, int unpack,
                               hipStream_t s);
hipError_t launch_fe(const MeshDev &m, const FeArgs &a, int lpc, hipStream_t s);
hipError_t launch_curl2(const MeshDev &m, const double *u, double *vort, bool accum, hipStream_t s);
hipError_t launch_curl_f32(const MeshDev &m, const float *u, float *vort, bool accum, hipStream_t s);
hipError_t launch_operator(const MeshDev &m, const OpArgs &a, int lpc, hipStream_t s);
hipError_t launch_update_ssh(const MeshDev &m, const double *h, double *ssh, int nlev, int lpc, hipStream_t s);
hipError_t launch_permute_rows(double *dst, const double *src, const int32_t *n2o, int64_t n, int K, int to_device,
                               hipStream_t s);
hipError_t launch_sum_sq_serial(const double *a, int64_t n, double *out, hipStream_t s);
hipError_t launch_copy(double *dst, const double *src, int64_t n, hipStream_t s);
hipError_t launch_bw_copy(void *dst, const void *src, int64_t bytes, int nCUs, hipStream_t s);
hipError_t launch_bw_streams(void *buf, int64_t bytes, hipStream_t s);
hipError_t launch_bw_gather_n(const void *src, int64_t nRows, uint32_t rowB, int64_t nFetch, uint32_t *sink, int nCUs, hipStream_t s);
hipError_t launch_bw_read(const void *src, int64_t bytes, uint32_t *sink, int nCUs, hipStream_t s);
hipError_t launch_bw_gather(const void *src, int64_t bytes, uint32_t rowB, uint32_t *sink, int nCUs, hipStream_t s);
hipError_t launch_halo_map(double *buf, double *h, double *ssh, double *u, const uint32_t *map, int64_t n, int unpack,
                           hipStream_t s);
hipError_t launch_pack_rows(double *buf, const double *field, const int32_t *rows, int64_t n, int K, int unpack, hipStream_t s);

struct NlArgs {
    double *qv;
    double *fq;
    double *ke;
    double *zv;
    double *divc;
    double visc;
    const double *div4;
    const double *curl4;
    const double *coef4;
};
bool nl_stage_is_nl5(const MeshDev &m, int lpc, bool rowsOk, int form);
bool nl_patch_forms(const MeshDev &m, int lpc, int form);
hipError_t launch_nl_prepare(const MeshDev &m, const double *u, const double *h, const NlArgs &nl, int lpc, int form, hipStream_t s);
hipError_t launch_stage_nl(const MeshDev &m, const StageArgs &a, const NlArgs &nl, int lpc, bool rowsOk, int form, hipStream_t s);
struct D4Rows {
    const int32_t *start;
    const int32_t *row;
    const uint16_t *locC;
    const uint16_t *locV;
    int32_t maxRows;
};
int del4_path(const MeshDev &m, const D4Rows &r, int lpc, int form);
hipError_t launch_del4(const MeshDev &m, const D4Rows &r, const double *divc, const double *zv, double *div4, double *curl4, int path,
                       hipStream_t s);

struct TracerArgs {
    int nT, stage;
    int64_t stride;
    const double *pu, *ph;
    const double *hcur;
    const double *hnext;
    const double *pphi;
    const double *cphi;
    double *pphi_out;
    double *qn;
    double a, b;
    const double *kappa, *dvdc;
    const double *const *src;
    const double *kappa4, *lap;
};
struct TracerKernel {
    int form;
    size_t lds;
    int chunk;
};
TracerKernel tracer_kernel(const MeshDev &m, int lpc, int nT, bool generic, bool diff, bool bih);
hipError_t launch_tracers(const MeshDev &m, const TracerArgs &a, int lpc, bool generic, hipStream_t s);

struct TracerLapArgs {
    int nT;
    int64_t stride;
    const double *ph;
    const double *x;
    const double *kappa4, *dvdc;
    double *out;
};
hipError_t launch_tracer_lap(const MeshDev &m, const TracerLapArgs &a, int lpc, bool generic, hipStream_t s);

struct TracerAdjArgs {
    int nT, rs;
    int64_t stride;
    const double *pu, *ph;
    const double *y;
    const double *g;
    double *S;
    double *out;
    double cb, ca;
    const double *kappa, *dvdc;
    double *const *G;
    const double *kappa4, *lapy;
};
inline TracerKernel tracer_adjoint_kernel(const MeshDev &m, int lpc, int nT, bool generic, bool diff, bool bih)
{
    return tracer_kernel(m, lpc, nT, generic, diff, bih);
}
hipError_t launch_tracer_adjoint(const MeshDev &m, const TracerAdjArgs &a, int lpc, bool generic, hipStream_t s);
hipError_t launch_tracer_adj_seed(const MeshDev &m, const double *X, const double *hn, double *g, double *y, double b4, int nT,
                                  double *const *G, hipStream_t s);

struct TracerKgradArgs {
    int nF;
    int64_t stride;
    const double *ph, *L, *y, *M;
    const int32_t *tracer;
    double *const *W;
};
hipError_t launch_tracer_kgrad(const MeshDev &m, const TracerKgradArgs &a, int lpc, hipStream_t s);

struct VmixArgs {
    int nT, nC, K;
    int64_t stride;
    const double *h;
    double *x;
    const double *kv;
    double dt;
    const int32_t *nLev;
    double *scratch;
    const int32_t *gslot;
    const double *p;
    double *D;
    const double *const *fld;
};
struct VmixKernel {
    int form;
    size_t lds;
    int tc;
};
VmixKernel vmix_kernel(int K, bool generic, int sets = 3);
hipError_t launch_tracer_vmix(const VmixArgs &a, bool reverse, bool generic, hipStream_t s);

struct MomVmixArgs {
    int nE, K;
    const int32_t *ehdr;
    double *u;
    const double *h;
    const double *tau;
    double dt, nu, drag;
    double *scratch;
};
int momentum_vmix_form(int K, bool generic);
hipError_t launch_momentum_vmix(const MomVmixArgs &a, bool generic, hipStream_t s);

struct AdjMesh {
    int32_t nC, nE, K, ME, W;
    const int32_t *eoc;
    const int32_t *csgn;
    const int32_t *ehdr;
// ... 32 lines not shown
```

### mpas-ocean.jl_amd/csrc/moka_internal.hpp

```cpp
#pragma once
#include <cstdint>
#include <string>
#include <vector>

#include "../../include/moka_hip.h"

namespace moka {

void set_error(const std::string &msg);
const char *get_error();

struct Plan {
    int32_t nC = 0, nE = 0, nV = 0, K = 1;
    int32_t ME = 0;
    int32_t ME2 = 0;
    int32_t VD = 3;
    int32_t ordering = 0, P = 0, nPatches = 0;
    int32_t stateBytes = 8;
    int64_t cellBandwidth = 0;

    std::vector<int32_t> cellN2O, cellO2N, edgeN2O, edgeO2N, vertN2O, vertO2N;
    std::vector<int32_t> patchCellStart, patchEdgeStart, patchVertStart;
    std::vector<int32_t> classPatchStart, classCellStart, classEdgeStart;

    std::vector<int32_t> eoc;
    std::vector<int32_t> coc;
    std::vector<int32_t> mltc;
    std::vector<double>  sdv;
    std::vector<double>  dvdc;
    std::vector<int32_t> nLev;
    std::vector<double>  invArea;
    std::vector<double>  areaCell;
    std::vector<double>  rsum;
    std::vector<int32_t> ehdr;
    std::vector<int32_t> eoe;
    std::vector<double>  woe;
    std::vector<double>  gInvDc;
    std::vector<double>  dcEdge, dvEdge, fEdge;
    std::vector<uint32_t> cRec, eRec;
    std::vector<double>   feoe;
    std::vector<uint32_t> vRec;
    int32_t maxOwnV = 0;
    int32_t CI = 0, EI = 0;
    bool colOk = false;
    std::vector<int32_t> rowStart;
    std::vector<int32_t> rowEdge;
    std::vector<int32_t> haloStart;
    std::vector<int32_t> haloEdge;
    std::vector<uint8_t> leoc;
    std::vector<uint8_t> leoe;
    int32_t maxRows = 0, maxOwnE = 0, maxOwnC = 0;
    int32_t maxOwnELaunch = 0, maxOwnCLaunch = 0, nPatchesLaunch = 0;
    bool ldsOk = false;
    std::vector<int32_t> eov;
    std::vector<double>  cv;
    bool nlOk = false;
    std::vector<int32_t> voe;
    std::vector<int32_t> cov;
    std::vector<double>  kite;
    std::vector<double>  invAreaTri, fVertex;
    std::vector<double>  keCoef, invDc;
    std::vector<double>  keoc;
    std::vector<int32_t> rowVoe;
    std::vector<int32_t> pvStart, pvList;
    std::vector<uint16_t> lvoe;
    int32_t maxPV = 0;
    bool nl5Ok = false;
};

int build_plan(const moka_mesh_desc *d, Plan &out);

struct MeshDev {
    int32_t nC, nE, nV, K, ME, ME2, VD, nPatches;
    int32_t patchBegin;
    const int32_t *patchCellStart, *patchEdgeStart, *patchVertStart;
    const int32_t *eoc, *coc, *mltc;
    const double  *sdv, *invArea, *areaCell, *rsum;
    const int32_t *ehdr, *eoe;
    const double  *woe, *gInvDc, *dcEdge, *dvEdge, *fEdge;
    const int32_t *eov;
    const double  *cv;
    const int32_t *cellN2O, *edgeN2O, *vertN2O;
    const uint32_t *cRec, *eRec;
    const double *feoe;
    const uint32_t *vRec;
    int32_t maxOwnV;
    int32_t CI, EI;
    const int32_t *rowStart, *rowEdge;
    const uint8_t *leoe;
    int32_t maxRows, maxOwnE, maxOwnC;
    const int32_t *voe, *cov;
    const double *kite, *invAreaTri, *fVertex, *keCoef, *invDc, *keoc;
    const int32_t *rowVoe;
    const int32_t *pvStart, *pvList;
    const uint16_t *lvoe;
    int32_t maxPV, pvCap;
    int32_t tailPatch;
};

inline int64_t lds_stage_bytes(int K, int ME, int ME2, int maxRows, int maxOwnE, int maxOwnC)
{
    int64_t dbl = (int64_t)maxRows * K + maxRows + (int64_t)maxOwnE * ME2 + maxOwnE + (int64_t)maxOwnC * ME + 2 * maxOwnC;
    int64_t i32 = (int64_t)maxOwnE * 4 + 2 * (int64_t)maxOwnC * ME + (int64_t)maxOwnE * 4 + (int64_t)maxOwnC * 2;
    return dbl * 8 + i32 * 4 + 16;
}

}

struct moka_plan {
    moka::Plan p;
};
```

### mpas-ocean.jl_amd/csrc/plan.cpp

```cpp
#include <algorithm>
#include <array>
#include <cmath>
#include <new>
#include <numeric>
#include <queue>

#include "moka_internal.hpp"

namespace moka {

static thread_local std::string g_err;
void set_error(const std::string &msg) { g_err = msg; }
const char *get_error() { return g_err.c_str(); }

namespace {

inline int64_t IX(int i, int64_t j, int ld) { return j * ld + i; }

#define REQUIRE(cond, msg)                 \
    do {                                   \
        if (!(cond)) {                     \
            set_error(msg);                \
            return MOKA_ERR_ARG;           \
        }                                  \
    } while (0)

std::vector<int> partition_by_class(const moka_mesh_desc *d, std::vector<int32_t> &n2o)
{
    std::vector<int> bounds{0};
    if (!d->cellClass) { bounds.push_back((int)n2o.size()); return bounds; }
    int maxc = 0;
    for (int c = 0; c < d->nCells; ++c) maxc = std::max(maxc, (int)d->cellClass[c]);
    std::vector<int32_t> out;
    out.reserve(n2o.size());
    for (int k = 0; k <= maxc; ++k) {
        for (int32_t c : n2o) if (d->cellClass[c] == k) out.push_back(c);
        bounds.push_back((int)out.size());
    }
    n2o.swap(out);
    return bounds;
}

void rcb_order(const moka_mesh_desc *d, int P, std::vector<int32_t> &n2o)
{
    const int n = d->nCells;
    n2o.resize(n);
    std::iota(n2o.begin(), n2o.end(), 0);
    const double *X[3] = {d->xCell, d->yCell, d->zCell};
    struct Range { int lo, hi; };
    std::vector<Range> stack;
    {
        const std::vector<int> b = partition_by_class(d, n2o);
        for (size_t i = b.size() - 1; i >= 1; --i) if (b[i] > b[i - 1]) stack.push_back({b[i - 1], b[i]});
    }
    while (!stack.empty()) {
        Range r = stack.back();
        stack.pop_back();
        const int cnt = r.hi - r.lo;
        if (cnt <= P) {
            continue;
        }
        int axis = 0;
        double best = -1.0;
        for (int a = 0; a < 3; ++a) {
            if (!X[a]) continue;
            double mn = 1e300, mx = -1e300;
            for (int i = r.lo; i < r.hi; ++i) {
                double v = X[a][n2o[i]];
                mn = std::min(mn, v);
                mx = std::max(mx, v);
            }
            if (mx - mn > best) { best = mx - mn; axis = a; }
        }
        const int leaves = (cnt + P - 1) / P;
        const int left = (leaves / 2) * P;
        const double *xa = X[axis];
        std::nth_element(n2o.begin() + r.lo, n2o.begin() + r.lo + left, n2o.begin() + r.hi,
                         [xa](int32_t a, int32_t b) { return xa[a] < xa[b] || (xa[a] == xa[b] && a < b); });
        stack.push_back({r.lo + left, r.hi});
        stack.push_back({r.lo, r.lo + left});
    }
}

void rcm_order(const moka_mesh_desc *d, std::vector<int32_t> &n2o)
{
    const int n = d->nCells;
    std::vector<int32_t> deg(n, 0), start(n + 1, 0), adj;
    for (int64_t e = 0; e < d->nEdges; ++e) {
        int a = d->cellsOnEdge[2 * e] - 1, b = d->cellsOnEdge[2 * e + 1] - 1;
        if (a >= 0 && b >= 0 && a != b) { ++deg[a]; ++deg[b]; }
    }
    for (int i = 0; i < n; ++i) start[i + 1] = start[i] + deg[i];
    adj.resize(start[n]);
    std::vector<int32_t> fill(start.begin(), start.end() - 1);
    for (int64_t e = 0; e < d->nEdges; ++e) {
        int a = d->cellsOnEdge[2 * e] - 1, b = d->cellsOnEdge[2 * e + 1] - 1;
        if (a >= 0 && b >= 0 && a != b) { adj[fill[a]++] = b; adj[fill[b]++] = a; }
    }
    std::vector<char> seen(n, 0);
    std::vector<int32_t> order;
    order.reserve(n);
    auto bfs_far = [&](int s, std::vector<int32_t> &lvl) {
        std::vector<int32_t> q{s};
        lvl.assign(n, -1);
        lvl[s] = 0;
        size_t h = 0;
        while (h < q.size()) {
            int u = q[h++];
            for (int k = start[u]; k < start[u + 1]; ++k)
                if (lvl[adj[k]] < 0 && !seen[adj[k]]) { lvl[adj[k]] = lvl[u] + 1; q.push_back(adj[k]); }
        }
        return q.back();
    };
    std::vector<int32_t> lvl;
    for (int s0 = 0; s0 < n; ++s0) {
        if (seen[s0]) continue;
        int s = bfs_far(bfs_far(s0, lvl), lvl);
        std::vector<int32_t> q{s};
        seen[s] = 1;
        size_t h = 0;
        std::vector<int32_t> nb;
        while (h < q.size()) {
            int u = q[h++];
            nb.clear();
            for (int k = start[u]; k < start[u + 1]; ++k)
                if (!seen[adj[k]]) { seen[adj[k]] = 1; nb.push_back(adj[k]); }
            std::sort(nb.begin(), nb.end(), [&](int a, int b) { return deg[a] < deg[b] || (deg[a] == deg[b] && a < b); });
            q.insert(q.end(), nb.begin(), nb.end());
        }
        order.insert(order.end(), q.begin(), q.end());
    }
    n2o.assign(order.rbegin(), order.rend());
}

}

int build_plan(const moka_mesh_desc *d, Plan &p)
{
    REQUIRE(d != nullptr, "mesh descriptor is NULL");
    REQUIRE(d->nCells > 0 && d->nEdges > 0 && d->nVertices > 0, "mesh counts must be positive");
    REQUIRE(d->nVertLevels >= 1, "nVertLevels must be >= 1");
    REQUIRE(d->maxEdges >= 3 && d->maxEdges2 >= 1 && d->vertexDegree >= 3, "bad maxEdges/maxEdges2/vertexDegree");
    REQUIRE(d->nEdgesOnCell && d->edgesOnCell && d->edgeSignOnCell && d->areaCell, "PrimaryCells arrays missing");
    REQUIRE(d->cellsOnEdge && d->nEdgesOnEdge && d->edgesOnEdge && d->weightsOnEdge && d->dvEdge && d->dcEdge && d->fEdge,
            "Edges arrays missing");
    REQUIRE(d->edgesOnVertex && d->edgeSignOnVertex && d->areaTriangle, "DualCells arrays missing");
    REQUIRE(d->restingThicknessSum, "restingThicknessSum missing");
    const int nC = d->nCells, nE = d->nEdges, nV = d->nVertices, VD = d->vertexDegree;
    const int ldSV = d->edgeSignOnVertexLD > 0 ? d->edgeSignOnVertexLD : VD;
    REQUIRE(ldSV >= VD, "edgeSignOnVertexLD < vertexDegree");

    int maxEoC = 0, maxEoE = 0;
    for (int c = 0; c < nC; ++c) {
        int n = d->nEdgesOnCell[c];
        REQUIRE(n >= 1 && n <= d->maxEdges, "nEdgesOnCell out of range");
// ... 200 lines not shown
        for (int q = 0; q < p.nPatches; ++q) { ce[q + 1] += ce[q]; cv[q + 1] += cv[q]; }
        p.patchEdgeStart = ce;
        p.patchVertStart = cv;
        p.classEdgeStart.resize(p.classPatchStart.size());
        for (size_t k = 0; k < p.classPatchStart.size(); ++k) p.classEdgeStart[k] = ce[p.classPatchStart[k]];
    }

    const int ME = p.ME, ME2 = p.ME2;
    p.eoc.assign((size_t)nC * ME, -1);
    p.coc.assign((size_t)nC * ME, -1);
    p.mltc.assign((size_t)nC * ME, 0);
    p.sdv.assign((size_t)nC * ME, 0.0);
    p.dvdc.assign((size_t)nC * ME, 0.0);
    p.nLev.assign(nC, 0);
    p.invArea.resize(nC); p.areaCell.resize(nC); p.rsum.resize(nC);
    p.cellBandwidth = 0;
    for (int cn = 0; cn < nC; ++cn) {
        const int co = p.cellN2O[cn];
        const int n = d->nEdgesOnCell[co];
        for (int i = 0; i < n; ++i) {
            const int eo = d->edgesOnCell[IX(i, co, d->maxEdges)] - 1;
            const int a = d->cellsOnEdge[2 * (int64_t)eo] - 1, b = d->cellsOnEdge[2 * (int64_t)eo + 1] - 1;
            REQUIRE(a == co || b == co, "edgesOnCell / cellsOnEdge are inconsistent");
            const int other = (a == co) ? b : a;
            p.eoc[IX(i, cn, ME)] = p.edgeO2N[eo];
            p.coc[IX(i, cn, ME)] = p.cellO2N[other];
            p.mltc[IX(i, cn, ME)] = d->maxLevelEdgeTop ? d->maxLevelEdgeTop[eo] : 1;
            p.sdv[IX(i, cn, ME)] = d->dvEdge[eo] * (double)d->edgeSignOnCell[IX(i, co, d->maxEdges)];
            p.dvdc[IX(i, cn, ME)] = d->dvEdge[eo] / d->dcEdge[eo];
            p.nLev[cn] = std::max(p.nLev[cn], std::min(p.mltc[IX(i, cn, ME)], p.K));
            p.cellBandwidth = std::max<int64_t>(p.cellBandwidth, std::abs((int64_t)p.cellO2N[other] - cn));
        }
        p.invArea[cn] = 1. / d->areaCell[co];
        p.areaCell[cn] = d->areaCell[co];
        p.rsum[cn] = d->restingThicknessSum[co];
    }
    p.ehdr.resize((size_t)nE * 4);
    p.eoe.assign((size_t)nE * ME2, -1);
    p.woe.assign((size_t)nE * ME2, 0.0);
    p.gInvDc.resize(nE); p.dcEdge.resize(nE); p.dvEdge.resize(nE); p.fEdge.resize(nE);
    for (int en = 0; en < nE; ++en) {
        const int eo = p.edgeN2O[en];
        const int n = d->nEdgesOnEdge[eo];
        p.ehdr[4 * (size_t)en + 0] = p.cellO2N[d->cellsOnEdge[2 * (int64_t)eo] - 1];
        p.ehdr[4 * (size_t)en + 1] = p.cellO2N[d->cellsOnEdge[2 * (int64_t)eo + 1] - 1];
        p.ehdr[4 * (size_t)en + 2] = n;
        p.ehdr[4 * (size_t)en + 3] = d->maxLevelEdgeTop ? d->maxLevelEdgeTop[eo] : 1;
        for (int i = 0; i < n; ++i) {
            const int x = d->edgesOnEdge[IX(i, eo, d->maxEdges2)];
            p.eoe[IX(i, en, ME2)] = x == 0 ? -1 : p.edgeO2N[x - 1];
            p.woe[IX(i, en, ME2)] = d->weightsOnEdge[IX(i, eo, d->maxEdges2)];
        }
        const double invDc = 1. / d->dcEdge[eo];
        p.gInvDc[en] = 9.80616 * invDc;
        p.dcEdge[en] = d->dcEdge[eo];
        p.dvEdge[en] = d->dvEdge[eo];
        p.fEdge[en] = d->fEdge[eo];
    }
    p.eov.resize((size_t)nV * VD);
    p.cv.resize((size_t)nV * VD);
    for (int vn = 0; vn < nV; ++vn) {
        const int vo = p.vertN2O[vn];
        const double invA = 1.0 / d->areaTriangle[vo];
        for (int j = 0; j < VD; ++j) {
            const int eo = d->edgesOnVertex[IX(j, vo, VD)] - 1;
            p.eov[IX(j, vn, VD)] = p.edgeO2N[eo];
            p.cv[IX(j, vn, VD)] = (d->dcEdge[eo] * invA) * (double)d->edgeSignOnVertex[IX(j, vo, ldSV)];
        }
    }
    p.nlOk = d->kiteAreasOnVertex && d->fVertex && d->verticesOnEdge && d->cellsOnVertex;
    if (p.nlOk) {
        p.voe.resize((size_t)nE * 2); p.cov.resize((size_t)nV * VD); p.kite.resize((size_t)nV * VD);
        p.invAreaTri.resize(nV); p.fVertex.resize(nV); p.keCoef.resize(nE); p.invDc.resize(nE);
        for (int en = 0; en < nE; ++en) {
            const int eo = p.edgeN2O[en];
            for (int q = 0; q < 2; ++q) {
                const int v = d->verticesOnEdge[2 * (int64_t)eo + q];
                REQUIRE(v >= 1 && v <= nV, "verticesOnEdge out of range");
                p.voe[(size_t)en * 2 + q] = p.vertO2N[v - 1];
            }
            p.keCoef[en] = 0.25 * d->dcEdge[eo] * d->dvEdge[eo];
            p.invDc[en] = 1. / d->dcEdge[eo];
        }
        for (int vn = 0; vn < nV; ++vn) {
            const int vo = p.vertN2O[vn];
            p.invAreaTri[vn] = 1.0 / d->areaTriangle[vo];
            p.fVertex[vn] = d->fVertex[vo];
            for (int j = 0; j < VD; ++j) {
                const int c = d->cellsOnVertex[IX(j, vo, VD)];
                REQUIRE(c >= 1 && c <= nC, "cellsOnVertex out of range");
                p.cov[IX(j, vn, VD)] = p.cellO2N[c - 1];
                p.kite[IX(j, vn, VD)] = d->kiteAreasOnVertex[IX(j, vo, VD)];
            }
        }
    }

    {
        const uint64_t rowB = (uint64_t)p.K * p.stateBytes;
        p.colOk = rowB * (uint64_t)std::max(nE, std::max(nC, nV)) < (1ull << 32) - 1024;
        p.CI = ((2 * ME + 2) + 3) & ~3;
        p.EI = ((ME2 + 4) + 3) & ~3;
        p.cRec.clear(); p.eRec.clear(); p.feoe.clear();
        if (p.colOk) {
            p.cRec.assign((size_t)nC * p.CI, 0u);
            p.eRec.assign((size_t)nE * p.EI, 0u);
            p.feoe.assign((size_t)nE * ME2, 0.0);
            for (int c = 0; c < nC; ++c) {
                uint32_t *r = &p.cRec[(size_t)c * p.CI];
                uint32_t mask = 0, all = 1;
                for (int i = 0; i < ME; ++i) {
                    const int e = p.eoc[IX(i, c, ME)];
                    if (e >= 0) {
                        mask |= 1u << i;
                        r[i] = (uint32_t)((uint64_t)e * rowB);
                        r[ME + i] = (uint32_t)((uint64_t)p.coc[IX(i, c, ME)] * rowB);
                        if (p.mltc[IX(i, c, ME)] < p.K) all = 0;
                    } else {
                        r[i] = (uint32_t)((uint64_t)p.eoc[IX(0, c, ME)] * rowB);
                        r[ME + i] = (uint32_t)((uint64_t)c * rowB);
                    }
                }
                r[2 * ME] = mask;
                r[2 * ME + 1] = all;
            }
            for (int e = 0; e < nE; ++e) {
                uint32_t *r = &p.eRec[(size_t)e * p.EI];
                uint32_t mask = 0;
                for (int i = 0; i < ME2; ++i) {
                    const int x = p.eoe[IX(i, e, ME2)];
                    if (x >= 0) {
                        mask |= 1u << i;
                        r[i] = (uint32_t)((uint64_t)x * rowB);
                        p.feoe[IX(i, e, ME2)] = p.fEdge[x];
                    } else {
                        r[i] = (uint32_t)((uint64_t)e * rowB);
                    }
                }
                r[ME2] = (uint32_t)p.ehdr[4 * (size_t)e];
                r[ME2 + 1] = (uint32_t)p.ehdr[4 * (size_t)e + 1];
                r[ME2 + 2] = mask;
                r[ME2 + 3] = (uint32_t)p.ehdr[4 * (size_t)e + 3];
            }
        }
        p.vRec.clear();
        if (p.colOk && p.VD == 3) {
            p.vRec.assign((size_t)nV * 4, 0u);
            for (int v = 0; v < nV; ++v)
                for (int j = 0; j < 3; ++j) p.vRec[(size_t)v * 4 + j] = (uint32_t)((uint64_t)p.eov[(size_t)v * 3 + j] * rowB);
        }
        p.maxOwnV = 0;
        for (int q = 0; q < p.nPatches; ++q) p.maxOwnV = std::max(p.maxOwnV, p.patchVertStart[q + 1] - p.patchVertStart[q]);
    }

    p.haloStart.assign(p.nPatches + 1, 0);
    p.haloEdge.clear();
    p.leoc.assign((size_t)nC * 8, 0xFF);
    p.leoe.assign((size_t)nE * 16, 0xFF);
    p.maxRows = p.maxOwnE = p.maxOwnC = 0;
    p.maxOwnELaunch = p.maxOwnCLaunch = 0;
    for (int q = 0; q < p.nPatches; ++q) {
        const int nE_q = p.patchEdgeStart[q + 1] - p.patchEdgeStart[q], nC_q = p.patchCellStart[q + 1] - p.patchCellStart[q];
        p.maxOwnE = std::max(p.maxOwnE, nE_q);
        p.maxOwnC = std::max(p.maxOwnC, nC_q);
        const bool launched = !d->cellClass || d->cellClass[p.cellN2O[p.patchCellStart[q]]] < 2;
        if (launched) {
            p.nPatchesLaunch = q + 1;
            p.maxOwnELaunch = std::max(p.maxOwnELaunch, nE_q);
            p.maxOwnCLaunch = std::max(p.maxOwnCLaunch, nC_q);
        }
    }
    p.ldsOk = (ME <= 8 && ME2 <= 16);
    {
        std::vector<int32_t> local(nE, -1), touched;
        for (int q = 0; q < p.nPatches && p.ldsOk; ++q) {
            const int c0 = p.patchCellStart[q], c1 = p.patchCellStart[q + 1];
            const int e0 = p.patchEdgeStart[q], e1 = p.patchEdgeStart[q + 1];
            const int nOwn = e1 - e0;
            int rows = nOwn;
            touched.clear();
            auto local_of = [&](int e) {
                if (e >= e0 && e < e1) return e - e0;
                if (local[e] < 0) { local[e] = rows++; touched.push_back(e); p.haloEdge.push_back(e); }
                return local[e];
            };
            for (int c = c0; c < c1; ++c)
                for (int i = 0; i < ME; ++i) {
                    const int e = p.eoc[IX(i, c, ME)];
                    if (e >= 0) { int r = local_of(e); p.leoc[(size_t)c * 8 + i] = (uint8_t)std::min(r, 255); }
                }
            for (int e = e0; e < e1; ++e)
                for (int i = 0; i < ME2; ++i) {
                    const int x = p.eoe[IX(i, e, ME2)];
                    if (x >= 0) { int r = local_of(x); p.leoe[(size_t)e * 16 + i] = (uint8_t)std::min(r, 255); }
                }
            for (int e : touched) local[e] = -1;
            p.haloStart[q + 1] = (int32_t)p.haloEdge.size();
            if (rows > 254) p.ldsOk = false;
            p.maxRows = std::max(p.maxRows, rows);
        }
        if (!p.ldsOk) { p.haloEdge.clear(); std::fill(p.haloStart.begin(), p.haloStart.end(), 0); }
        p.haloEdge.push_back(0);
    }
    p.rowStart.assign(p.nPatches + 1, 0);
    p.rowEdge.clear();
    if (p.ldsOk) {
        for (int q = 0; q < p.nPatches; ++q) {
            for (int e = p.patchEdgeStart[q]; e < p.patchEdgeStart[q + 1]; ++e) p.rowEdge.push_back(e);
            for (int j = p.haloStart[q]; j < p.haloStart[q + 1]; ++j) p.rowEdge.push_back(p.haloEdge[j]);
            p.rowStart[q + 1] = (int32_t)p.rowEdge.size();
        }
    }
    p.rowEdge.push_back(0);
    if (p.nlOk) {
        p.rowVoe.resize(2 * p.rowEdge.size());
        for (size_t r = 0; r < p.rowEdge.size(); ++r) {
            p.rowVoe[2 * r] = p.voe[2 * (size_t)p.rowEdge[r]]; p.rowVoe[2 * r + 1] = p.voe[2 * (size_t)p.rowEdge[r] + 1];
        }
        p.keoc.assign((size_t)nC * ME, 0.0);
        for (int c = 0; c < nC; ++c)
            for (int i = 0; i < ME; ++i)
                if (p.eoc[IX(i, c, ME)] >= 0) p.keoc[IX(i, c, ME)] = p.keCoef[p.eoc[IX(i, c, ME)]];
    }
    p.pvStart.assign(p.nPatches + 1, 0);
    p.pvList.clear(); p.lvoe.clear();
    p.maxPV = 0; p.nl5Ok = false;
    if (p.nlOk && ME2 <= 10) {
        p.nl5Ok = true;
        p.lvoe.assign((size_t)nE * 24, 0);
        std::vector<int32_t> lv(p.nV, -1);
        for (int q = 0; q < p.nPatches; ++q) {
            const size_t base = p.pvList.size();
            auto lid = [&](int v) {
                if (lv[v] < 0) { lv[v] = (int32_t)(p.pvList.size() - base); p.pvList.push_back(v); }
                return (uint16_t)std::min(lv[v], 65535);
            };
            for (int e = p.patchEdgeStart[q]; e < p.patchEdgeStart[q + 1]; ++e) {
                uint16_t *r = &p.lvoe[(size_t)e * 24];
                r[20] = lid(p.voe[2 * (size_t)e]); r[21] = lid(p.voe[2 * (size_t)e + 1]);
                for (int i = 0; i < 10; ++i) {
                    const int x = i < ME2 ? p.eoe[IX(i, e, ME2)] : -1;
                    r[2 * i] = x >= 0 ? lid(p.voe[2 * (size_t)x]) : r[20];
                    r[2 * i + 1] = x >= 0 ? lid(p.voe[2 * (size_t)x + 1]) : r[21];
                }
            }
            const int n = (int)(p.pvList.size() - base);
            if (n > 65535) p.nl5Ok = false;
            p.maxPV = std::max(p.maxPV, n);
            for (size_t j = base; j < p.pvList.size(); ++j) lv[p.pvList[j]] = -1;
            p.pvStart[q + 1] = (int32_t)p.pvList.size();
        }
    }
    p.pvList.push_back(0);

    return MOKA_OK;
}

}

extern "C" {

int moka_plan_create(const moka_mesh_desc *desc, moka_plan **out)
{
    if (!out) { moka::set_error("out is NULL"); return MOKA_ERR_ARG; }
    *out = nullptr;
    moka_plan *pl = new (std::nothrow) moka_plan();
    if (!pl) { moka::set_error("out of host memory"); return MOKA_ERR_ALLOC; }
    int rc;
    try {
        rc = moka::build_plan(desc, pl->p);
    } catch (const std::bad_alloc &) {
        moka::set_error("out of host memory while building the mesh plan");
        rc = MOKA_ERR_ALLOC;
    }
    if (rc != MOKA_OK) { delete pl; return rc; }
    *out = pl;
    return MOKA_OK;
}

void moka_plan_destroy(moka_plan *plan) { delete plan; }

static int lanes_per_column(int K)
{
    int l = 1;
    while (l < K && l < 64) l <<= 1;
    return l;
}

static void fill_info(const moka::Plan &p, moka_mesh_info *info)
{
    info->nCells = p.nC; info->nEdges = p.nE; info->nVertices = p.nV; info->nVertLevels = p.K;
    info->ordering = p.ordering; info->patch_cells = p.P; info->nPatches = p.nPatches;
    info->maxEdgesUsed = p.ME; info->maxEdges2Used = p.ME2;
    info->lanesPerColumn = lanes_per_column(p.K);
    info->cellBandwidth = p.cellBandwidth;
    info->maxPatchRows = p.maxRows;
    info->maxPatchCells = p.maxOwnC;
    info->maxPatchEdges = p.maxOwnE;
    info->ldsBytesPerBlock = (p.ldsOk && p.K % 2 == 0)
                                 ? (int32_t)moka::lds_stage_bytes(p.K, p.ME, p.ME2, p.maxRows, p.maxOwnE, p.maxOwnC) : 0;
    info->meshBytesDevice =
        (int64_t)p.nC * (p.ME * (3 * 4 + 8) + 3 * 8) + (int64_t)p.nE * (16 + p.ME2 * 12 + 4 * 8) +
        (int64_t)p.nV * p.VD * 12 + (int64_t)(p.nPatches + 1) * 12 + 4ll * (p.nC + p.nE + p.nV);
}

int moka_plan_info(const moka_plan *plan, moka_mesh_info *info)
{
    if (!plan || !info) { moka::set_error("NULL argument"); return MOKA_ERR_ARG; }
    fill_info(plan->p, info);
    return MOKA_OK;
}

int moka_plan_permutation(const moka_plan *plan, int kind, int32_t *new_to_old)
{
    if (!plan || !new_to_old) { moka::set_error("NULL argument"); return MOKA_ERR_ARG; }
    const std::vector<int32_t> *v = kind == MOKA_CELL ? &plan->p.cellN2O : kind == MOKA_EDGE ? &plan->p.edgeN2O
                                  : kind == MOKA_VERTEX ? &plan->p.vertN2O : nullptr;
    if (!v) { moka::set_error("kind must be MOKA_CELL, MOKA_EDGE or MOKA_VERTEX"); return MOKA_ERR_ARG; }
    std::copy(v->begin(), v->end(), new_to_old);
    return MOKA_OK;
}

int moka_plan_patch_ranges(const moka_plan *plan, int32_t *cellStart, int32_t *edgeStart, int32_t *vertexStart)
{
    if (!plan) { moka::set_error("NULL argument"); return MOKA_ERR_ARG; }
    const moka::Plan &p = plan->p;
    if (cellStart) std::copy(p.patchCellStart.begin(), p.patchCellStart.end(), cellStart);
    if (edgeStart) std::copy(p.patchEdgeStart.begin(), p.patchEdgeStart.end(), edgeStart);
    if (vertexStart) std::copy(p.patchVertStart.begin(), p.patchVertStart.end(), vertexStart);
    return MOKA_OK;
}

int moka_plan_class_ranges(const moka_plan *plan, int32_t capacity, int32_t *nClasses, int32_t *patchStart, int32_t *cellStart,
                           int32_t *edgeStart)
{
    if (!plan || !nClasses) { moka::set_error("NULL argument"); return MOKA_ERR_ARG; }
    const moka::Plan &p = plan->p;
    const int n = (int)p.classPatchStart.size() - 1;
    *nClasses = n;
    for (int k = 0; k <= n && k < capacity; ++k) {
        if (patchStart) patchStart[k] = p.classPatchStart[k];
        if (cellStart) cellStart[k] = p.classCellStart[k];
        if (edgeStart) edgeStart[k] = p.classEdgeStart[k];
    }
    return MOKA_OK;
}

int moka_plan_array(const moka_plan *plan, int which, const void **data, int64_t *count)
{
    if (!plan || !data || !count) { moka::set_error("NULL argument"); return MOKA_ERR_ARG; }
    const moka::Plan &p = plan->p;
#define VEC(id, v) case id: *data = p.v.data(); *count = (int64_t)p.v.size(); return MOKA_OK;
    switch (which) {
        VEC(MOKA_PA_EOC, eoc) VEC(MOKA_PA_COC, coc) VEC(MOKA_PA_MLTC, mltc) VEC(MOKA_PA_SDV, sdv)
        VEC(MOKA_PA_INVAREA, invArea) VEC(MOKA_PA_AREACELL, areaCell) VEC(MOKA_PA_RSUM, rsum)
        VEC(MOKA_PA_EHDR, ehdr) VEC(MOKA_PA_EOE, eoe) VEC(MOKA_PA_WOE, woe) VEC(MOKA_PA_GINVDC, gInvDc)
        VEC(MOKA_PA_DCEDGE, dcEdge) VEC(MOKA_PA_DVEDGE, dvEdge) VEC(MOKA_PA_FEDGE, fEdge)
        VEC(MOKA_PA_EOV, eov) VEC(MOKA_PA_CV, cv)
        VEC(MOKA_PA_HALO_START, haloStart) VEC(MOKA_PA_HALO_EDGE, haloEdge) VEC(MOKA_PA_LEOC, leoc) VEC(MOKA_PA_LEOE, leoe)
        VEC(MOKA_PA_CREC, cRec) VEC(MOKA_PA_EREC, eRec) VEC(MOKA_PA_FEOE, feoe)
        VEC(MOKA_PA_PVSTART, pvStart) VEC(MOKA_PA_PVLIST, pvList) VEC(MOKA_PA_LVOE, lvoe)
        VEC(MOKA_PA_NLEV, nLev)
        default: moka::set_error("unknown plan array id"); return MOKA_ERR_ARG;
    }
#undef VEC
}

}

namespace moka { void fill_mesh_info(const Plan &p, moka_mesh_info *info) { fill_info(p, info); } }
```

### mpas-ocean.jl_amd/moka_hip/lib.py

```python
from __future__ import annotations

import ctypes as C
import os
import subprocess

import numpy as np

PKG_DIR = os.path.dirname(os.path.dirname(os.path.abspath(__file__)))
LIB_PATH = os.environ.get("MOKA_HIP_LIB") or os.path.join(PKG_DIR, "libmoka_hip.so")

_i32p = C.POINTER(C.c_int32)
_f64p = C.POINTER(C.c_double)

OK = 0
ERR_ARG, ERR_HIP, ERR_NO_DEVICE, ERR_ALLOC, ERR_UNSUPPORTED, ERR_COMM = -1, -2, -3, -4, -5, -6
ORDER_DEFAULT, ORDER_NONE, ORDER_RCM, ORDER_RCB = 0, 1, 2, 3
TRACER_GRAD_KAPPA, TRACER_GRAD_KAPPA4 = 1, 2
VGRAD_INTERFACE, VGRAD_CELL, VGRAD_PROFILE = 0, 1, 2
CELL, EDGE, VERTEX = 0, 1, 2
(F_SSH, F_NORMAL_VELOCITY, F_LAYER_THICKNESS, F_LAYER_THICKNESS_EDGE, F_THICKNESS_FLUX,
 F_VELOCITY_DIV_CELL, F_RELATIVE_VORTICITY, F_TEND_NORMAL_VELOCITY, F_TEND_LAYER_THICKNESS) = range(9)
FE_STALE_HEDGE, FE_ACCUM_VORT, FE_LEVEL1_ONLY, FE_REFERENCE_COMPAT = 1, 2, 4, 7
FORWARD_EULER, RUNGE_KUTTA_4 = 0, 1


class MokaError(RuntimeError):

    def __init__(self, code, msg):
        super().__init__(f"libmoka_hip error {code}: {msg}")
        self.code = code


class MeshDesc(C.Structure):
    _fields_ = [
        ("nCells", C.c_int32), ("nEdges", C.c_int32), ("nVertices", C.c_int32),
        ("maxEdges", C.c_int32), ("maxEdges2", C.c_int32), ("vertexDegree", C.c_int32),
        ("nVertLevels", C.c_int32), ("edgeSignOnVertexLD", C.c_int32),
        ("xCell", _f64p), ("yCell", _f64p), ("zCell", _f64p),
        ("nEdgesOnCell", _i32p), ("edgesOnCell", _i32p), ("edgeSignOnCell", _i32p), ("areaCell", _f64p),
        ("cellsOnEdge", _i32p), ("verticesOnEdge", _i32p), ("nEdgesOnEdge", _i32p), ("edgesOnEdge", _i32p),
        ("weightsOnEdge", _f64p), ("dvEdge", _f64p), ("dcEdge", _f64p), ("fEdge", _f64p),
        ("edgesOnVertex", _i32p), ("cellsOnVertex", _i32p), ("edgeSignOnVertex", _i32p), ("areaTriangle", _f64p),
        ("maxLevelEdgeTop", _i32p), ("restingThicknessSum", _f64p),
        ("ordering", C.c_int32), ("patch_cells", C.c_int32),
        ("cellClass", _i32p),
        ("stateBytes", C.c_int32),
        ("kiteAreasOnVertex", _f64p), ("fVertex", _f64p),
    ]


class HaloStats(C.Structure):
    _fields_ = [("steps", C.c_int64), ("exchanges", C.c_int64), ("boundary_launches", C.c_int64), ("interior_launches", C.c_int64),
                ("host_step_ms", C.c_double), ("host_signal_wait_ms", C.c_double), ("host_flag_store_ms", C.c_double),
                ("host_wait_ms", C.c_double), ("boundary_launch_ms", C.c_double), ("interior_launch_ms", C.c_double)]


class PlacementTrial(C.Structure):
    _fields_ = [("field", C.c_int32), ("ms_old", C.c_double), ("ms_new", C.c_double), ("kept", C.c_int32)]


class MeshInfo(C.Structure):
    _fields_ = [
        ("nCells", C.c_int32), ("nEdges", C.c_int32), ("nVertices", C.c_int32), ("nVertLevels", C.c_int32),
        ("ordering", C.c_int32), ("patch_cells", C.c_int32), ("nPatches", C.c_int32),
        ("maxEdgesUsed", C.c_int32), ("maxEdges2Used", C.c_int32), ("lanesPerColumn", C.c_int32),
        ("meshBytesDevice", C.c_int64), ("cellBandwidth", C.c_int64),
        ("maxPatchRows", C.c_int32), ("ldsBytesPerBlock", C.c_int32),
        ("maxPatchCells", C.c_int32), ("maxPatchEdges", C.c_int32),
    ]

    def as_dict(self):
        return {n: getattr(self, n) for n, _ in self._fields_}


EXPORTS = [
    "moka_version", "moka_ctx_create", "moka_ctx_destroy", "moka_last_error", "moka_sync",
    "moka_timer_start", "moka_timer_stop",
    "moka_plan_create", "moka_plan_destroy", "moka_plan_info", "moka_plan_permutation", "moka_plan_patch_ranges", "moka_plan_array",
    "moka_mesh_create", "moka_mesh_destroy", "moka_mesh_info_get",
    "moka_gradient_on_edge", "moka_divergence_on_cell", "moka_curl_on_vertex", "moka_interpolate_cell2edge",
    "moka_state_create", "moka_state_destroy", "moka_state_upload", "moka_state_download",
    "moka_advance_time_levels", "moka_diagnostic_compute", "moka_compute_normal_velocity_tendency",
    "moka_compute_layer_thickness_tendency", "moka_tendencies", "moka_step_fe", "moka_step_rk4", "moka_run",
    "moka_sum_sq", "moka_set_kernel_variant", "moka_kernel_variant_available", "moka_stage_timing", "moka_stage_timing_read",
    "moka_ctx_streams", "moka_halo_create", "moka_halo_destroy", "moka_halo_buffer_elems", "moka_halo_pack",
    "moka_halo_unpack", "moka_rk4_dist_begin", "moka_rk4_dist_stage", "moka_rk4_dist_end",
    "moka_plan_class_ranges", "moka_mesh_class_ranges", "moka_mesh_permutation", "moka_halo_direct_available", "moka_halo_set_overlap", "moka_halo_pack_fields", "moka_halo_unpack_fields",
    "moka_tape_record_rk4", "moka_tape_commit_rk4", "moka_adjoint_rk4_stage_fields", "moka_adjoint_rk4_stage",
    "moka_tape_record_fe", "moka_tape_commit_fe", "moka_adjoint_fe_step_fields", "moka_adjoint_fe_step",
    "moka_halo_export", "moka_halo_connect", "moka_halo_push_begin", "moka_halo_push_signal", "moka_halo_push_wait",
    "moka_rk4_dist_stage_launch", "moka_rk4_dist_step", "moka_fe_dist_launch", "moka_fe_dist_end", "moka_fe_dist_step",
    "moka_set_nonlinear", "moka_last_fe_path", "moka_set_viscosity_del2", "moka_set_viscosity_del4", "moka_state_del4_path", "moka_tape_create", "moka_tape_destroy", "moka_step_fe_taped", "moka_step_rk4_taped", "moka_adjoint_seed_sum_sq_ssh", "moka_adjoint_sweep",
    "moka_adjoint_download",
    "moka_mark", "moka_marks_reset", "moka_marks_read", "moka_bw_probe", "moka_bw_probe_streams", "moka_bw_probe_reread", "moka_bw_probe_gather_big", "moka_ctx_pci_bus_id", "moka_halo_set_acquire", "moka_set_tuning", "moka_get_tuning", "moka_rk4_dist_parts_available", "moka_adjoint_rk4_stage_part", "moka_adjoint_rk4_parts_available", "moka_adjoint_rk4_stage_out_fields",
    "moka_gradient_on_edge_vjp", "moka_gradient_on_edge_jvp", "moka_divergence_on_cell_vjp", "moka_divergence_on_cell_jvp",
    "moka_curl_on_vertex_vjp", "moka_curl_on_vertex_jvp", "moka_fe_lazy_pending",
    "moka_state_optimize_placement", "moka_state_placement_log", "moka_state_download_rows",
    "moka_halo_stats_enable", "moka_halo_stats_read", "moka_halo_set_stream_flags", "moka_state_array_address", "moka_state_placement_launches",
    "moka_state_rk4_streams",
    "moka_set_tracers", "moka_tracer_upload", "moka_tracer_download", "moka_state_tracer_path",
    "moka_set_tracer_diffusion", "moka_tracer_diffusion",
    "moka_set_tracer_biharmonic", "moka_tracer_biharmonic",
    "moka_set_tracer_vertical_diffusion", "moka_tracer_vertical_diffusion", "moka_state_tracer_vmix_path", "moka_tracer_adjoint_vmix_path",
    "moka_tracer_source_upload", "moka_tracer_source_download", "moka_tracer_has_source",
    "moka_tracer_vertical_field_upload", "moka_tracer_vertical_field_download", "moka_tracer_has_vertical_field",
    "moka_set_vertical_viscosity", "moka_vertical_viscosity", "moka_surface_stress_upload", "moka_surface_stress_download",
    "moka_has_surface_stress", "moka_state_momentum_vmix_path",
    "moka_tracer_adjoint_want_source_gradient", "moka_tracer_adjoint_source_download",
    "moka_tracer_adjoint_want_diffusivity_gradient", "moka_tracer_adjoint_diffusivity_gradient",
    "moka_tracer_adjoint_diffusivity_density_download",
    "moka_tracer_adjoint_want_vertical_gradient", "moka_tracer_adjoint_vertical_gradient",
    "moka_tracer_adjoint_vertical_density_download",
    "moka_tracer_tape_create", "moka_tracer_tape_destroy", "moka_step_rk4_tracer_taped", "moka_tracer_tape_steps",
    "moka_tracer_adjoint_seed", "moka_tracer_adjoint_sweep", "moka_tracer_adjoint_download", "moka_tracer_adjoint_path",
]


def build(force: bool = False) -> str:
    if force:
        subprocess.check_call(["make", "-C", PKG_DIR, "--no-print-directory", "clean"])
    subprocess.check_call(["make", "-C", PKG_DIR, "--no-print-directory", "-j4"])
    return LIB_PATH


_lib = None


def lib():
    global _lib
    if _lib is not None:
        return _lib
    if not os.path.exists(LIB_PATH):
        raise MokaError(ERR_NO_DEVICE, f"{LIB_PATH} is missing: build it with `make -C {PKG_DIR}` "
                                       "(there is no CPU fallback for the HIP path)")
    try:
        import torch
    except ImportError:
        pass
    L = C.CDLL(LIB_PATH)
    vp = C.c_void_p
    L.moka_version.restype = C.c_char_p
    L.moka_last_error.restype = C.c_char_p
    L.moka_last_error.argtypes = [vp]
    L.moka_ctx_create.argtypes = [C.c_int, C.POINTER(vp)]
    L.moka_ctx_destroy.argtypes = [vp]
    L.moka_ctx_destroy.restype = None
    L.moka_sync.argtypes = [vp]
    L.moka_timer_start.argtypes = [vp]
    L.moka_timer_stop.argtypes = [vp, C.POINTER(C.c_float)]
    L.moka_plan_create.argtypes = [C.POINTER(MeshDesc), C.POINTER(vp)]
    L.moka_plan_destroy.argtypes = [vp]
    L.moka_plan_destroy.restype = None
    L.moka_plan_info.argtypes = [vp, C.POINTER(MeshInfo)]
    L.moka_plan_permutation.argtypes = [vp, C.c_int, _i32p]
    L.moka_plan_patch_ranges.argtypes = [vp, _i32p, _i32p, _i32p]
    L.moka_plan_array.argtypes = [vp, C.c_int, C.POINTER(vp), C.POINTER(C.c_int64)]
    L.moka_mesh_create.argtypes = [vp, C.POINTER(MeshDesc), C.POINTER(vp)]
    L.moka_mesh_destroy.argtypes = [vp]
    L.moka_mesh_destroy.restype = None
    L.moka_mesh_info_get.argtypes = [vp, C.POINTER(MeshInfo)]
    L.moka_gradient_on_edge.argtypes = [vp, _f64p, _f64p]
    L.moka_divergence_on_cell.argtypes = [vp, _f64p, _f64p, _f64p]
    L.moka_curl_on_vertex.argtypes = [vp, _f64p, _f64p]
    L.moka_interpolate_cell2edge.argtypes = [vp, _f64p, _f64p, C.c_int]
    L.moka_gradient_on_edge_vjp.argtypes = [vp, _f64p, _f64p]
    L.moka_gradient_on_edge_jvp.argtypes = [vp, _f64p, _f64p]
    L.moka_divergence_on_cell_vjp.argtypes = [vp, _f64p, _f64p, _f64p]
    L.moka_divergence_on_cell_jvp.argtypes = [vp, _f64p, _f64p, _f64p]
    L.moka_curl_on_vertex_vjp.argtypes = [vp, _f64p, _f64p]
    L.moka_curl_on_vertex_jvp.argtypes = [vp, _f64p, _f64p]
    L.moka_state_create.argtypes = [vp, vp, C.POINTER(vp)]
    L.moka_state_destroy.argtypes = [vp]
    L.moka_state_destroy.restype = None
    L.moka_state_optimize_placement.argtypes = [vp, C.c_int, _f64p, _f64p]
    L.moka_state_placement_launches.argtypes = [vp]
    L.moka_state_rk4_streams.argtypes = [vp]
    L.moka_state_placement_launches.restype = C.c_int64
    L.moka_state_placement_log.argtypes = [vp, C.c_int32, C.POINTER(PlacementTrial), _i32p]
    L.moka_state_array_address.argtypes = [vp, C.c_int, C.c_int, C.POINTER(C.c_uint64)]
    L.moka_state_download_rows.argtypes = [vp, C.c_int, C.c_int, C.c_int64, _i32p, _f64p]
    L.moka_state_upload.argtypes = [vp, C.c_int, C.c_int, _f64p]
    L.moka_state_download.argtypes = [vp, C.c_int, C.c_int, _f64p]
    L.moka_advance_time_levels.argtypes = [vp, C.c_int]
    L.moka_diagnostic_compute.argtypes = [vp, C.c_int]
    L.moka_compute_normal_velocity_tendency.argtypes = [vp, C.c_int]
    L.moka_compute_layer_thickness_tendency.argtypes = [vp, C.c_int]
    L.moka_tendencies.argtypes = [vp]
    L.moka_step_fe.argtypes = [vp, C.c_double, C.c_int]
    L.moka_step_rk4.argtypes = [vp, C.c_double]
    L.moka_run.argtypes = [vp, C.c_int, C.c_double, C.c_int64, C.c_int]
    L.moka_sum_sq.argtypes = [vp, C.c_int, C.c_int, _f64p]
    L.moka_set_kernel_variant.argtypes = [vp, C.c_int]
    L.moka_kernel_variant_available.argtypes = [C.c_int]
    L.moka_stage_timing.argtypes = [vp, C.c_int]
    L.moka_stage_timing_read.argtypes = [vp, C.POINTER(C.c_double), C.POINTER(C.c_int64)]
    L.moka_ctx_streams.argtypes = [vp, C.POINTER(vp), C.POINTER(vp)]
    i64p = C.POINTER(C.c_int64)
    L.moka_halo_create.argtypes = [vp, C.c_int32, _i32p, i64p, _i32p, i64p, _i32p, i64p, _i32p, i64p,
                                   C.c_int32, C.c_int32, C.POINTER(vp)]
    L.moka_halo_destroy.argtypes = [vp]
    L.moka_halo_set_stream_flags.argtypes = [vp, C.c_int]
    L.moka_halo_stats_enable.argtypes = [vp, C.c_int]
    L.moka_halo_stats_read.argtypes = [vp, C.POINTER(HaloStats)]
    L.moka_halo_destroy.restype = None
    L.moka_halo_buffer_elems.argtypes = [vp, C.POINTER(C.c_int64), C.POINTER(C.c_int64)]
    L.moka_halo_pack.argtypes = [vp, C.c_int, vp]
    L.moka_halo_unpack.argtypes = [vp, C.c_int, vp]
    L.moka_rk4_dist_begin.argtypes = [vp, C.c_double]
    L.moka_rk4_dist_stage.argtypes = [vp, C.c_int, C.c_int]
    L.moka_rk4_dist_parts_available.argtypes = [vp]
    L.moka_rk4_dist_end.argtypes = [vp]
    L.moka_plan_class_ranges.argtypes = [vp, C.c_int32, C.POINTER(C.c_int32), _i32p, _i32p, _i32p]
    L.moka_mesh_class_ranges.argtypes = [vp, C.c_int32, C.POINTER(C.c_int32), _i32p, _i32p, _i32p]
    L.moka_mesh_permutation.argtypes = [vp, C.c_int, _i32p]
    L.moka_halo_direct_available.argtypes = [vp]
    L.moka_halo_set_overlap.argtypes = [vp, C.c_int]
    L.moka_halo_set_acquire.argtypes = [vp, C.c_int]
    L.moka_halo_pack_fields.argtypes = [vp, vp, vp, vp, vp]
    L.moka_halo_unpack_fields.argtypes = [vp, vp, vp, vp, vp]
    L.moka_tape_record_rk4.argtypes = [vp, C.c_int, C.c_int]
    L.moka_tape_commit_rk4.argtypes = [vp, C.c_double]
    L.moka_adjoint_rk4_stage_fields.argtypes = [vp, C.c_int, C.POINTER(vp), C.POINTER(vp), C.POINTER(vp)]
    L.moka_adjoint_rk4_stage.argtypes = [vp, C.c_int]
    L.moka_adjoint_rk4_stage_part.argtypes = [vp, C.c_int, C.c_int]
    L.moka_adjoint_rk4_parts_available.argtypes = [vp]
    L.moka_adjoint_rk4_stage_out_fields.argtypes = [vp, C.c_int, C.POINTER(vp), C.POINTER(vp), C.POINTER(vp)]
    L.moka_tape_record_fe.argtypes = [vp, C.c_int, C.c_int]
    L.moka_tape_commit_fe.argtypes = [vp, C.c_double, C.c_int]
    L.moka_adjoint_fe_step_fields.argtypes = [vp, C.POINTER(vp), C.POINTER(vp), C.POINTER(vp)]
    L.moka_adjoint_fe_step.argtypes = [vp]
    L.moka_halo_export.argtypes = [vp, C.c_int32, C.c_int32, C.POINTER(HaloPeerInfo)]
    L.moka_halo_connect.argtypes = [vp, C.c_int32, C.POINTER(HaloPeerInfo), C.c_int32]
    L.moka_halo_push_begin.argtypes = [vp, C.c_int]
    L.moka_halo_push_signal.argtypes = [vp]
    L.moka_halo_push_wait.argtypes = [vp, C.c_double]
    L.moka_rk4_dist_stage_launch.argtypes = [vp, C.c_int]
    L.moka_rk4_dist_step.argtypes = [vp, C.c_double, TRANSPORT_FN, vp, vp, vp, C.c_double]
    L.moka_fe_dist_launch.argtypes = [vp, C.c_double, C.c_int, C.c_int]
    L.moka_fe_dist_end.argtypes = [vp]
    L.moka_fe_dist_step.argtypes = [vp, C.c_double, C.c_int, TRANSPORT_FN, vp, vp, vp, C.c_double]
    L.moka_set_nonlinear.argtypes = [vp, C.c_int]
    L.moka_last_fe_path.argtypes = [vp]
    L.moka_fe_lazy_pending.argtypes = [vp]
    L.moka_set_viscosity_del2.argtypes = [vp, C.c_double]
    L.moka_set_viscosity_del4.argtypes = [vp, C.c_double, vp]
    L.moka_state_del4_path.argtypes = [vp]
    L.moka_set_tracers.argtypes = [vp, C.c_int32]
    L.moka_tracer_upload.argtypes = [vp, C.c_int32, C.c_int, vp]
    L.moka_tracer_download.argtypes = [vp, C.c_int32, C.c_int, vp]
    L.moka_state_tracer_path.argtypes = [vp]
    L.moka_set_tracer_diffusion.argtypes = [vp, vp]
    L.moka_tracer_diffusion.argtypes = [vp, C.c_int32, C.POINTER(C.c_double)]
    L.moka_set_tracer_biharmonic.argtypes = [vp, vp]
    L.moka_tracer_biharmonic.argtypes = [vp, C.c_int32, C.POINTER(C.c_double)]
    L.moka_set_tracer_vertical_diffusion.argtypes = [vp, vp]
    L.moka_tracer_vertical_diffusion.argtypes = [vp, C.c_int32, C.POINTER(C.c_double)]
    L.moka_state_tracer_vmix_path.argtypes = [vp]
    L.moka_tracer_adjoint_vmix_path.argtypes = [vp]
    L.moka_tracer_tape_create.argtypes = [vp, C.c_int64, C.POINTER(vp)]
    L.moka_tracer_tape_destroy.argtypes = [vp]
    L.moka_tracer_tape_destroy.restype = None
    L.moka_step_rk4_tracer_taped.argtypes = [vp, C.c_double]
    L.moka_tracer_tape_steps.argtypes = [vp, C.POINTER(C.c_int64)]
    L.moka_tracer_adjoint_seed.argtypes = [vp, C.c_int32, vp]
    L.moka_tracer_adjoint_sweep.argtypes = [vp]
    L.moka_tracer_adjoint_download.argtypes = [vp, C.c_int32, vp]
    L.moka_tracer_adjoint_path.argtypes = [vp]
    L.moka_tracer_source_upload.argtypes = [vp, C.c_int32, vp]
    L.moka_tracer_source_download.argtypes = [vp, C.c_int32, vp]
    L.moka_tracer_has_source.argtypes = [vp, C.c_int32, C.POINTER(C.c_int)]
    L.moka_tracer_vertical_field_upload.argtypes = [vp, C.c_int32, vp]
    L.moka_tracer_vertical_field_download.argtypes = [vp, C.c_int32, vp]
    L.moka_tracer_has_vertical_field.argtypes = [vp, C.c_int32, C.POINTER(C.c_int)]
    L.moka_set_vertical_viscosity.argtypes = [vp, C.c_double, C.c_double]
    L.moka_vertical_viscosity.argtypes = [vp, C.POINTER(C.c_double), C.POINTER(C.c_double)]
    L.moka_surface_stress_upload.argtypes = [vp, vp]
    L.moka_surface_stress_download.argtypes = [vp, vp]
    L.moka_has_surface_stress.argtypes = [vp, C.POINTER(C.c_int)]
    L.moka_state_momentum_vmix_path.argtypes = [vp]
    L.moka_tracer_adjoint_want_source_gradient.argtypes = [vp, C.c_int32, C.c_int]
    L.moka_tracer_adjoint_source_download.argtypes = [vp, C.c_int32, vp]
    L.moka_tracer_adjoint_want_diffusivity_gradient.argtypes = [vp, C.c_int32, C.c_int, C.c_int]
    L.moka_tracer_adjoint_diffusivity_gradient.argtypes = [vp, C.c_int32, C.c_int, C.POINTER(C.c_double)]
    L.moka_tracer_adjoint_diffusivity_density_download.argtypes = [vp, C.c_int32, C.c_int, vp]
    L.moka_tracer_adjoint_want_vertical_gradient.argtypes = [vp, C.c_int32, C.c_int]
    L.moka_tracer_adjoint_vertical_gradient.argtypes = [vp, C.c_int32, C.POINTER(C.c_double)]
    L.moka_tracer_adjoint_vertical_density_download.argtypes = [vp, C.c_int32, C.c_int, vp]
    L.moka_tape_create.argtypes = [vp, C.c_int64, C.POINTER(vp)]
    L.moka_tape_destroy.argtypes = [vp]
    L.moka_tape_destroy.restype = None
    L.moka_step_fe_taped.argtypes = [vp, C.c_double, C.c_int]
    L.moka_step_rk4_taped.argtypes = [vp, C.c_double]
    L.moka_adjoint_seed_sum_sq_ssh.argtypes = [vp]
    L.moka_adjoint_sweep.argtypes = [vp]
    L.moka_adjoint_download.argtypes = [vp, C.c_int, _f64p]
    L.moka_mark.argtypes = [vp]
    L.moka_marks_reset.argtypes = [vp]
    L.moka_marks_read.argtypes = [vp, C.c_int64, _f64p, C.POINTER(C.c_int64)]
    L.moka_bw_probe.argtypes = [vp, C.c_int64, C.c_int, _f64p]
    L.moka_bw_probe_streams.argtypes = [vp, C.c_int, C.POINTER(C.c_double)]
    L.moka_bw_probe_reread.argtypes = [vp, C.c_int64, C.c_int, C.c_int, C.POINTER(C.c_double)]
    L.moka_bw_probe_gather_big.argtypes = [vp, C.c_int64, C.c_int, C.POINTER(C.c_double)]
    L.moka_ctx_pci_bus_id.argtypes = [vp, C.c_char_p, C.c_int32]
    L.moka_set_tuning.argtypes = [C.c_int, C.c_int]
    L.moka_get_tuning.argtypes = [C.c_int, C.POINTER(C.c_int)]
    _lib = L
    return L


def check(rc, ctx=None):
    if rc != OK:
        msg = lib().moka_last_error(ctx)
        raise MokaError(rc, msg.decode() if msg else "unknown")


def f64(a):
    return a.ctypes.data_as(_f64p)


def i32(a):
    return a.ctypes.data_as(_i32p)


def i64(a):
    return a.ctypes.data_as(C.POINTER(C.c_int64))


def make_desc(mesh, K, resting_thickness_sum=None, max_level_edge_top=None, ordering=ORDER_DEFAULT, patch_cells=0,
              cell_class=None, state_bytes=8):
    keep = {}

    def A(name, dt, val=None):
        arr = np.ascontiguousarray(getattr(mesh, name) if val is None else val, dtype=dt)
        keep[name] = arr
        return arr

    d = MeshDesc()
    d.nCells, d.nEdges, d.nVertices = mesh.nCells, mesh.nEdges, mesh.nVertices
    d.maxEdges, d.maxEdges2, d.vertexDegree = mesh.maxEdges, mesh.maxEdges2, mesh.vertexDegree
    d.nVertLevels = int(K)
    esv = A("edgeSignOnVertex", np.int32)
    d.edgeSignOnVertexLD = esv.shape[1]
    d.edgeSignOnVertex = i32(esv)
    for n in ("xCell", "yCell", "zCell", "areaCell", "weightsOnEdge", "dvEdge", "dcEdge", "fEdge", "areaTriangle"):
        setattr(d, n, f64(A(n, np.float64)))
    for n in ("nEdgesOnCell", "edgesOnCell", "edgeSignOnCell", "cellsOnEdge", "verticesOnEdge", "nEdgesOnEdge",
              "edgesOnEdge", "edgesOnVertex", "cellsOnVertex"):
        setattr(d, n, i32(A(n, np.int32)))
    if max_level_edge_top is None:
        d.maxLevelEdgeTop = None
    else:
        mlt = np.full(mesh.nEdges, int(max_level_edge_top), np.int32) if np.isscalar(max_level_edge_top) \
            else np.asarray(max_level_edge_top)
        d.maxLevelEdgeTop = i32(A("maxLevelEdgeTop", np.int32, mlt))
    if resting_thickness_sum is None:
        resting_thickness_sum = np.ones(mesh.nCells)
    d.restingThicknessSum = f64(A("restingThicknessSum", np.float64, np.asarray(resting_thickness_sum).reshape(-1)))
    d.ordering, d.patch_cells = int(ordering), int(patch_cells)
    d.cellClass = i32(A("cellClass", np.int32, cell_class)) if cell_class is not None else None
    d.stateBytes = int(state_bytes)
    kite = getattr(mesh, "kiteAreasOnVertex", None)
    if kite is not None:
        d.kiteAreasOnVertex = f64(A("kiteAreasOnVertex", np.float64, kite))
        d.fVertex = f64(A("fVertex", np.float64))
    return d, keep


PLAN_ARRAYS = {
    "eoc": (0, np.int32), "coc": (1, np.int32), "mltc": (2, np.int32), "sdv": (3, np.float64),
    "invArea": (4, np.float64), "areaCell": (5, np.float64), "rsum": (6, np.float64),
    "ehdr": (7, np.int32), "eoe": (8, np.int32), "woe": (9, np.float64), "gInvDc": (10, np.float64),
    "dcEdge": (11, np.float64), "dvEdge": (12, np.float64), "fEdge": (13, np.float64),
    "eov": (14, np.int32), "cv": (15, np.float64),
    "haloStart": (16, np.int32), "haloEdge": (17, np.int32), "leoc": (18, np.uint8), "leoe": (19, np.uint8),
    "cRec": (20, np.uint32), "eRec": (21, np.uint32), "feoe": (22, np.float64),
    "pvStart": (23, np.int32), "pvList": (24, np.int32), "lvoe": (25, np.uint16),
    "nLev": (26, np.int32),
}


class HaloPeerInfo(C.Structure):
    _fields_ = [("ipc", (C.c_ubyte * 64) * 15), ("ptr", C.c_uint64 * 15), ("flagPtr", C.c_uint64),
                ("shmName", C.c_char * 64), ("dstCell", C.c_int32), ("dstEdge", C.c_int32), ("nCells", C.c_int32),
                ("nEdges", C.c_int32), ("slot", C.c_int32), ("nNeighbors", C.c_int32), ("pid", C.c_int32),
                ("device", C.c_int32), ("stateBytes", C.c_int32), ("nVertLevels", C.c_int32)]


TRANSPORT_FN = C.CFUNCTYPE(C.c_int, C.c_void_p, C.c_int, C.c_void_p, C.c_void_p)


def class_ranges(handle, of_mesh: bool):
    fn = lib().moka_mesh_class_ranges if of_mesh else lib().moka_plan_class_ranges
    n = C.c_int32()
    check(fn(handle, 0, C.byref(n), None, None, None))
    a, b, c = (np.empty(n.value + 1, dtype=np.int32) for _ in range(3))
    check(fn(handle, n.value + 1, C.byref(n), i32(a), i32(b), i32(c)))
    return a, b, c


class Plan:

    def __init__(self, mesh, K, resting_thickness_sum=None, max_level_edge_top=None, ordering=ORDER_DEFAULT,
                 patch_cells=0, cell_class=None, state_bytes=8):
        self._h = C.c_void_p()
        desc, self._keep = make_desc(mesh, K, resting_thickness_sum, max_level_edge_top, ordering, patch_cells,
                                     cell_class, state_bytes)
        check(lib().moka_plan_create(C.byref(desc), C.byref(self._h)))
        inf = MeshInfo()
        check(lib().moka_plan_info(self._h, C.byref(inf)))
        self.info = inf.as_dict()

    def permutation(self, kind):
        n = {CELL: self.info["nCells"], EDGE: self.info["nEdges"], VERTEX: self.info["nVertices"]}[kind]
        out = np.empty(n, dtype=np.int32)
        check(lib().moka_plan_permutation(self._h, kind, i32(out)))
        return out

    def class_ranges(self):
        return class_ranges(self._h, False)

    def patch_ranges(self):
        n = self.info["nPatches"] + 1
        a, b, c = (np.empty(n, dtype=np.int32) for _ in range(3))
        check(lib().moka_plan_patch_ranges(self._h, i32(a), i32(b), i32(c)))
        return a, b, c

    def array(self, name):
        which, dt = PLAN_ARRAYS[name]
        ptr, cnt = C.c_void_p(), C.c_int64()
        check(lib().moka_plan_array(self._h, which, C.byref(ptr), C.byref(cnt)))
        buf = (C.c_char * (cnt.value * np.dtype(dt).itemsize)).from_address(ptr.value)
        return np.frombuffer(buf, dtype=dt).copy()

    def close(self):
        if self._h:
            lib().moka_plan_destroy(self._h)
            self._h = C.c_void_p()

    def __del__(self):
        try:
            self.close()
        except Exception:
            pass
```

Baseline: 9.174 billion.

## Add compact per-patch byte-indexed stage records for RK stages 2-4

Builds a per-patch contiguous block holding 8-bit local neighbour indices, masks, weights and tables of row offsets and Coriolis values. For RK modes 2, 3 and 8 on hexagonal meshes, the stage kernel loads that block into LDS with one coalesced copy instead of the wider 32-bit records, then decodes the byte indices. The aim is to cut mesh metadata traffic and LDS footprint per patch. The cost is an extra indirection and byte decoding in the inner loops, and the path applies only when the patch count is at least 4096 or the form setting forces it.

```diff
diff --git a/include/moka_hip.h b/include/moka_hip.h
--- a/include/moka_hip.h
+++ b/include/moka_hip.h
@@ -68,6 +68,7 @@
     int32_t maxPatchRows;
     int32_t ldsBytesPerBlock;
     int32_t maxPatchCells, maxPatchEdges;
+    int64_t compactRecordBytes;
 } moka_mesh_info;
 
 enum { MOKA_CELL = 0, MOKA_EDGE = 1, MOKA_VERTEX = 2 };
@@ -112,7 +113,8 @@
     MOKA_PA_EHDR, MOKA_PA_EOE, MOKA_PA_WOE, MOKA_PA_GINVDC, MOKA_PA_DCEDGE, MOKA_PA_DVEDGE, MOKA_PA_FEDGE,
     MOKA_PA_EOV, MOKA_PA_CV, MOKA_PA_HALO_START, MOKA_PA_HALO_EDGE, MOKA_PA_LEOC, MOKA_PA_LEOE,
     MOKA_PA_CREC, MOKA_PA_EREC, MOKA_PA_FEOE, MOKA_PA_PVSTART, MOKA_PA_PVLIST, MOKA_PA_LVOE,
-    MOKA_PA_NLEV
+    MOKA_PA_NLEV,
+    MOKA_PA_CR_IDX, MOKA_PA_CR_BLK
 };
 int  moka_plan_array(const moka_plan *plan, int which, const void **data, int64_t *count);
 
@@ -218,6 +220,9 @@
 int moka_set_kernel_variant(moka_ctx *ctx, int variant);
 int moka_set_tuning(int key, int value);
 int moka_get_tuning(int key, int *value);
+int moka_set_stage_records(int form);
+int moka_get_stage_records(int *form);
+int moka_last_stage_records(int mode, int *form);
 int moka_state_rk4_streams(const moka_state *st);
 int moka_stage_timing(moka_ctx *ctx, int enable);
 int moka_stage_timing_read(moka_ctx *ctx, double ms[4], int64_t *steps);
diff --git a/mpas-ocean.jl_amd/csrc/api.hip b/mpas-ocean.jl_amd/csrc/api.hip
--- a/mpas-ocean.jl_amd/csrc/api.hip
+++ b/mpas-ocean.jl_amd/csrc/api.hip
@@ -45,6 +45,10 @@
 constexpr int N_TUNING = sizeof(g_tuning) / sizeof(g_tuning[0]);
 
 int tuning(TuningKey key) { return g_tuning[key].value.load(); }
+
+static std::atomic<int> g_stageRecords{1}, g_lastStageRecords[12] = {{-1}, {-1}, {-1}, {-1}, {-1}, {-1}, {-1}, {-1}, {-1}, {-1}, {-1}, {-1}};
+int stage_records() { return g_stageRecords.load(); }
+void note_stage_records(int mode, int form) { g_lastStageRecords[mode].store(form); }
 
 }
 
@@ -716,6 +720,28 @@
     return MOKA_OK;
 }
 
+int moka_set_stage_records(int form)
+{
+    if (form < 0 || form > 2) return fail(nullptr, MOKA_ERR_ARG, "stage records: form must be 0, 1 or 2");
+    g_stageRecords.store(form);
+    return MOKA_OK;
+}
+
+int moka_get_stage_records(int *form)
+{
+    if (!form) return fail(nullptr, MOKA_ERR_ARG, "form is NULL");
+    *form = g_stageRecords.load();
+    return MOKA_OK;
+}
+
+int moka_last_stage_records(int mode, int *form)
+{
+    if (!form) return fail(nullptr, MOKA_ERR_ARG, "form is NULL");
+    if (mode < 0 || mode >= 12) return fail(nullptr, MOKA_ERR_ARG, "mode names no instance of the stage kernel");
+    *form = g_lastStageRecords[mode].load();
+    return MOKA_OK;
+}
+
 int moka_kernel_variant_available(int variant)
 {
     return variant == 0 || variant == 3 || variant == 4 || variant == 11;
@@ -780,6 +806,14 @@
     d.maxRows = p.maxRows; d.maxOwnE = p.maxOwnE; d.maxOwnC = p.maxOwnC;
     d.maxOwnV = p.maxOwnV;
     if (p.vRec.empty()) d.vRec = nullptr;
+    d.crIdx = d.crBlk = nullptr; d.crMaxUnits = 0; d.crPatches = 0;
+    if (!p.crBlk.empty()) {
+        if ((rc = upload_vec(m, p.crIdx, &d.crIdx)) != MOKA_OK || (rc = upload_vec(m, p.crBlk, &d.crBlk)) != MOKA_OK) {
+            moka_mesh_destroy(m);
+            return rc;
+        }
+        d.crMaxUnits = p.crMaxUnits; d.crPatches = p.nPatches;
+    }
     *out = m;
     return MOKA_OK;
 }
diff --git a/mpas-ocean.jl_amd/csrc/kernels.hip b/mpas-ocean.jl_amd/csrc/kernels.hip
--- a/mpas-ocean.jl_amd/csrc/kernels.hip
+++ b/mpas-ocean.jl_amd/csrc/kernels.hip
@@ -7,9 +7,10 @@
 namespace moka {
 
 
-template <int ME, int ME2, int MODE, int NT = BLOCK>
-__global__ __launch_bounds__(NT) void k_stage_rec2c(const ColMesh m, const StageArgs a, int maxOwnE, int maxOwnC)
-{
+template <int ME, int ME2, int MODE, int NT = BLOCK, bool CR = false>
+__global__ __launch_bounds__(NT) void k_stage_rec2c(const std::conditional_t<CR, ColMeshC, ColMesh> m, const StageArgs a, int maxOwnE, int maxOwnC)
+{
+    static_assert(!CR || ((MODE == 2 || MODE == 3 || MODE == 8) && ME <= 6 && ME2 <= 10), "compact records: RK stages 2 - 4 of hexagon-width meshes");
     extern __shared__ __align__(16) unsigned char smem[];
     const int pl_ = patch_of_block(m.nPatches);
     if (pl_ >= m.nPatches) return;
@@ -20,15 +21,32 @@
     const int grp = tid >> 5, l = tid & 31;
     const int K = m.K, K2 = K >> 1;
     const uint32_t voff = (uint32_t)l * 16u, rowB = (uint32_t)K * 8u;
-    const RecLds L = rec_carve(smem, m, ME, ME2, maxOwnE, maxOwnC);
-    const size_t recBytes = ((size_t)maxOwnE * (2 * ME2 + 1) * 8 + (size_t)maxOwnC * (ME + 2) * 8 +
-                             ((size_t)maxOwnE * m.EI + (size_t)maxOwnC * m.CI) * 4 + 15) & ~(size_t)15;
+    RecLds L = rec_carve(smem, m, ME, ME2, maxOwnE, maxOwnC);
+    size_t recBytes = ((size_t)maxOwnE * (2 * ME2 + 1) * 8 + (size_t)maxOwnC * (ME + 2) * 8 +
+                       ((size_t)maxOwnE * m.EI + (size_t)maxOwnC * m.CI) * 4 + 15) & ~(size_t)15;
+    if constexpr (CR) recBytes = (size_t)m.crMaxUnits * 16;
     double2 *ubuf2 = reinterpret_cast<double2 *>(smem + recBytes);
     const unsigned char *ubytes = reinterpret_cast<const unsigned char *>(ubuf2) + voff;
     const int c0 = cptr(m.patchCellStart)[p], c1 = cptr(m.patchCellStart)[pEnd];
     const int e0 = cptr(m.patchEdgeStart)[p], e1 = cptr(m.patchEdgeStart)[pEnd];
     const int nOwnC = c1 - c0, nOwnE = e1 - e0;
     const uint32_t e0B = (uint32_t)e0 * rowB, nOwnB = (uint32_t)nOwnE * rowB;
+    uint32_t crFirst = 0, crUnits = 0;
+    const uint32_t *tOffE = nullptr, *tOffC = nullptr, *Lecell = nullptr;
+    const double *tF = nullptr;
+    if constexpr (CR) {
+        const auto ix = cptr(m.crIdx) + 4 * (size_t)p;
+        crFirst = ix[0]; crUnits = ix[1];
+        const CompactCarve v = compact_carve((uint32_t)nOwnE, (uint32_t)nOwnC, ix[2], ix[3], ME, ME2);
+        L.eRec = reinterpret_cast<uint32_t *>(smem + v.e16); L.cRec = reinterpret_cast<uint32_t *>(smem + v.c16);
+        L.woe = reinterpret_cast<double *>(smem + v.woe); L.sdv = reinterpret_cast<double *>(smem + v.sdv);
+        L.g = reinterpret_cast<double *>(smem + v.g); L.invA = reinterpret_cast<double *>(smem + v.invA);
+        L.rsum = reinterpret_cast<double *>(smem + v.rsum); L.feoe = nullptr;
+        Lecell = reinterpret_cast<const uint32_t *>(smem + v.ecell);
+        tOffE = reinterpret_cast<const uint32_t *>(smem + v.offE); tOffC = reinterpret_cast<const uint32_t *>(smem + v.offC);
+        tF = reinterpret_cast<const double *>(smem + v.fE);
+    }
+    auto idb = [](const v4u_t &w, int b) -> uint32_t { return (w[b >> 2] >> (8 * (b & 3))) & 0xFFu; };
     double *Lvw = reinterpret_cast<double *>(smem + recBytes + (size_t)maxOwnE * rowB);
     uint32_t *Lvo = reinterpret_cast<uint32_t *>(Lvw + (size_t)m.maxOwnV * 3);
     constexpr bool LEAN = MODE >= 10;
@@ -42,7 +60,25 @@
         }
     }
 
-    {
+    if constexpr (CR) {
+        const double2 *src = reinterpret_cast<const double2 *>(a.pu) + (size_t)e0 * K2;
+        const v4u_t *blk = reinterpret_cast<const v4u_t *>(m.crBlk) + crFirst;
+        v4u_t *dst = reinterpret_cast<v4u_t *>(smem);
+        const int nU = nOwnE * K2, nB = (int)crUnits;
+        constexpr int UU = 6, UB = 3;
+        double2 vU[UU];
+        v4u_t vB[UB];
+#pragma unroll
+        for (int j = 0; j < UU; ++j) vU[j] = (tid + j * NT < nU) ? src[tid + j * NT] : make_double2(0.0, 0.0);
+#pragma unroll
+        for (int j = 0; j < UB; ++j) vB[j] = (tid + j * NT < nB) ? blk[tid + j * NT] : v4u_t{0u, 0u, 0u, 0u};
+#pragma unroll
+        for (int j = 0; j < UU; ++j) if (tid + j * NT < nU) ubuf2[tid + j * NT] = vU[j];
+#pragma unroll
+        for (int j = 0; j < UB; ++j) if (tid + j * NT < nB) dst[tid + j * NT] = vB[j];
+        for (int i = tid + UU * NT; i < nU; i += NT) ubuf2[i] = src[i];
+        for (int i = tid + UB * NT; i < nB; i += NT) dst[i] = blk[i];
+    } else {
         const double2 *src = reinterpret_cast<const double2 *>(a.pu) + (size_t)e0 * K2;
         const int nU = nOwnE * K2, nER = nOwnE * m.EI, nW = nOwnE * ME2, nCR = nOwnC * m.CI, nS = nOwnC * ME;
         constexpr int UU = 6, UE = 3, UW = 2;
@@ -146,9 +182,11 @@
 #pragma nounroll
     for (int ci = grp; ci < nOwnC; ci += NG) {
         const int c = c0 + ci;
-        const uint32_t *r = L.cRec + (size_t)ci * m.CI;
+        const uint32_t *r = L.cRec + (size_t)ci * (CR ? 4 : m.CI);
         const double *rs = L.sdv + (size_t)ci * ME;
-        const uint32_t mask = r[2 * ME], all = r[2 * ME + 1];
+        v4u_t w = {0u, 0u, 0u, 0u};
+        if constexpr (CR) w = *reinterpret_cast<const v4u_t *>(r);
+        const uint32_t mask = CR ? (w.w & 0xFFu) : r[2 * ME], all = CR ? ((w.w >> 8) & 0xFFu) : r[2 * ME + 1];
         const double invA = L.invA[ci];
         const uint32_t own = (uint32_t)c * rowB + voff;
         double2 hc = make_double2(0.0, 0.0), uv[ME], hv[ME], cur = hc, nin = hc, hpc = hc, q3 = hc;
@@ -160,10 +198,18 @@
             if constexpr (PREV) hpc = gload2(a.hPrev, own);
 #pragma unroll
             for (int i = 0; i < ME; ++i) {
-                const uint32_t off = r[i];
-                hv[i] = STALE ? gload2(a.hEdgeOld, off + voff) : gload2(PREV ? a.hPrev : a.ph, r[ME + i] + voff);
-                ad[i] = urow_addr(off, cached[i]);
-                goff[i] = off + voff;
+                if constexpr (CR) {
+                    const uint32_t ie = idb(w, i);
+                    hv[i] = gload2(a.ph, tOffC[idb(w, ME + i)] + voff);
+                    cached[i] = ie < (uint32_t)nOwnE;
+                    ad[i] = ldsU + (cached[i] ? ie * rowB : 0u);
+                    goff[i] = tOffE[ie] + voff;
+                } else {
+                    const uint32_t off = r[i];
+                    hv[i] = STALE ? gload2(a.hEdgeOld, off + voff) : gload2(PREV ? a.hPrev : a.ph, r[ME + i] + voff);
+                    ad[i] = urow_addr(off, cached[i]);
+                    goff[i] = off + voff;
+                }
                 asm("" : "+v"(goff[i]));
             }
             lds_burst<ME>(raw, ad);
@@ -284,11 +330,17 @@
 #pragma nounroll
     for (int ei = grp; ei < nOwnE; ei += NG) {
         const int e = e0 + ei;
-        const uint32_t *r = L.eRec + (size_t)ei * m.EI;
+        const uint32_t *r = L.eRec + (size_t)ei * (CR ? 4 : m.EI);
         const double *rw = L.woe + (size_t)ei * ME2;
         const double *rf = L.feoe + (size_t)ei * ME2;
-        const uint32_t mask = r[ME2 + 2];
-        const int mlt = (int)r[ME2 + 3];
+        v4u_t w = {0u, 0u, 0u, 0u};
+        if constexpr (CR) w = *reinterpret_cast<const v4u_t *>(r);
+        const uint32_t mask = CR ? (w.w & 0xFFFFu) : r[ME2 + 2];
+        const int mlt = CR ? (int)((w.w >> 16) & 0xFFu) : (int)r[ME2 + 3];
+        auto fcor = [&](int i) -> double {
+            if constexpr (CR) return tF[idb(w, i)];
+            else return rf[i];
+        };
         const double g = L.g[ei];
         const uint32_t own = (uint32_t)e * rowB + voff;
         double sv = 0.0;
@@ -299,9 +351,16 @@
             v4u_t raw[ME2];
 #pragma unroll
             for (int i = 0; i < ME2; ++i) {
-                const uint32_t off = r[i];
-                ad[i] = urow_addr(off, cached[i]);
-                goff[i] = off + voff;
+                if constexpr (CR) {
+                    const uint32_t ie = idb(w, i);
+                    cached[i] = ie < (uint32_t)nOwnE;
+                    ad[i] = ldsU + (cached[i] ? ie * rowB : 0u);
+                    goff[i] = tOffE[ie] + voff;
+                } else {
+                    const uint32_t off = r[i];
+                    ad[i] = urow_addr(off, cached[i]);
+                    goff[i] = off + voff;
+                }
                 asm("" : "+v"(goff[i]));
             }
             lds_burst<ME2>(raw, ad);
@@ -327,7 +386,7 @@
                 }
             }
         }
-        if (l < 2) sv = a.ssh[r[ME2 + l]];
+        if (l < 2) sv = a.ssh[CR ? Lecell[2 * ei + l] : r[ME2 + l]];
         __builtin_amdgcn_s_waitcnt(0x0F70);
         if (pend) flush_edge();
         const double ds = __shfl(sv, 1, 32) - __shfl(sv, 0, 32);
@@ -340,8 +399,9 @@
                 t.y -= g * ds;
 #pragma unroll
                 for (int i = 0; i < ME2; ++i) {
-                    t.x += rw[i] * uv[i].x * rf[i];
-                    t.y += rw[i] * uv[i].y * rf[i];
+                    const double f = fcor(i);
+                    t.x += rw[i] * uv[i].x * f;
+                    t.y += rw[i] * uv[i].y * f;
                 }
             } else {
                 if (ax) t.x -= g * ds;
@@ -349,7 +409,8 @@
 #pragma unroll
                 for (int i = 0; i < ME2; ++i) {
                     const bool on = (mask >> i) & 1u;
-                    const double px = rw[i] * uv[i].x * rf[i], py = rw[i] * uv[i].y * rf[i];
+                    const double f = fcor(i);
+                    const double px = rw[i] * uv[i].x * f, py = rw[i] * uv[i].y * f;
                     if (on && ax) t.x += px;
                     if (on && ay) t.y += py;
                 }
@@ -1446,6 +1507,8 @@
     if (tuning(TUNE_FE_LEAN_INST) && colp_lean(a, mode)) mode += 5;
     const size_t lds = rec2c_lds_bytes(md) + (a.vort ? vert_lds_bytes(md) : 0);
     if (mode < 0 || md.K > 64 || (md.K & 1) || lds > 64 * 1024 || md.maxOwnC < 1 || md.maxOwnE < 1) return hipErrorNotSupported;
+    const bool crMode = mode == 2 || mode == 3 || mode == 8;
+    if (crMode) note_stage_records(mode, 0);
     const int pair = tuning(TUNE_PAIR);
     if (((pair >> mode) & 1) && md.tailPatch < 0 && (md.nPatches >= 4096 || ((pair >> 16) & 1)) && md.nPatches >= 2 &&
         md.ME == 6 && md.ME2 == 10) {
@@ -1458,6 +1521,20 @@
             mp.pairEnd = md.patchBegin + md.nPatches;
             const hipError_t e = launch_rec2c_pair<6, 10>(mp, a, mode, dim3(8 * ((nPair + 7) / 8)), lds2, two.maxOwnE, two.maxOwnC, s);
             if (e != hipErrorNotSupported) return e;
+        }
+    }
+    if (crMode) {
+        const int form = stage_records();
+        const size_t ldsC = (size_t)md.crMaxUnits * 16 + (size_t)md.maxOwnE * md.K * 8 + 16;
+        const bool compact = form != 0 && md.crBlk && md.patchBegin == 0 && md.nPatches == md.crPatches && md.tailPatch < 0 &&
+                             md.ME == 6 && md.ME2 == 10 && (md.nPatches >= 4096 || form == 2) && ldsC <= lds;
+        if (compact) {
+            note_stage_records(mode, 1);
+            ColMeshC mc{m, md.crIdx, md.crBlk, md.crMaxUnits};
+            if (mode == 2) hipLaunchKernelGGL((k_stage_rec2c<6, 10, 2, BLOCK, true>), g, b, ldsC, s, mc, a, md.maxOwnE, md.maxOwnC);
+            else if (mode == 3) hipLaunchKernelGGL((k_stage_rec2c<6, 10, 3, BLOCK, true>), g, b, ldsC, s, mc, a, md.maxOwnE, md.maxOwnC);
+            else hipLaunchKernelGGL((k_stage_rec2c<6, 10, 8, BLOCK, true>), g, b, ldsC, s, mc, a, md.maxOwnE, md.maxOwnC);
+            return hipGetLastError();
         }
     }
     bool ok = false;
diff --git a/mpas-ocean.jl_amd/csrc/kernels.hpp b/mpas-ocean.jl_amd/csrc/kernels.hpp
--- a/mpas-ocean.jl_amd/csrc/kernels.hpp
+++ b/mpas-ocean.jl_amd/csrc/kernels.hpp
@@ -2,6 +2,7 @@
 #include <hip/hip_runtime.h>
 
 #include <initializer_list>
+#include <type_traits>
 
 #include "moka_internal.hpp"
 
@@ -41,6 +42,10 @@
     int32_t maxOwnV;
     int32_t pairEnd;
 };
+struct ColMeshC : ColMesh {
+    const uint32_t *crIdx, *crBlk;
+    int32_t crMaxUnits;
+};
 
 enum : int {
     FE_FLUX = 1, FE_DIV = 2, FE_CURL = 4, FE_HEDGE = 8, FE_TENDU = 16, FE_TENDH = 32, FE_UPDATE = 64,
@@ -90,6 +95,8 @@
     TUNE_FE_LEAN_INST = 9,
 };
 int tuning(TuningKey key);
+int stage_records();
+void note_stage_records(int mode, int form);
 
 hipError_t raise_dyn_lds(std::initializer_list<const void *> fns, int bytes);
 hipError_t launch_update_ssh_f32(const MeshDev &m, const float *h, float *ssh, int nlev, int lpc, hipStream_t s);
diff --git a/mpas-ocean.jl_amd/csrc/moka_internal.hpp b/mpas-ocean.jl_amd/csrc/moka_internal.hpp
--- a/mpas-ocean.jl_amd/csrc/moka_internal.hpp
+++ b/mpas-ocean.jl_amd/csrc/moka_internal.hpp
@@ -66,7 +66,35 @@
     std::vector<uint16_t> lvoe;
     int32_t maxPV = 0;
     bool nl5Ok = false;
+    std::vector<uint32_t> crIdx;
+    std::vector<uint32_t> crBlk;
+    int32_t crMaxUnits = 0;
 };
+
+struct CompactCarve {
+    uint32_t e16, c16, woe, sdv, g, ecell, invA, rsum, offE, fE, offC, total;
+};
+#if defined(__HIPCC__)
+__host__ __device__
+#endif
+inline CompactCarve compact_carve(uint32_t nE, uint32_t nC, uint32_t rE, uint32_t rC, uint32_t ME, uint32_t ME2)
+{
+    auto up = [](uint32_t b) { return (b + 15u) & ~15u; };
+    CompactCarve v;
+    v.e16 = 0;
+    v.c16 = v.e16 + nE * 16u;
+    v.woe = v.c16 + nC * 16u;
+    v.sdv = v.woe + up(nE * ME2 * 8u);
+    v.g = v.sdv + up(nC * ME * 8u);
+    v.ecell = v.g + up(nE * 8u);
+    v.invA = v.ecell + up(nE * 8u);
+    v.rsum = v.invA + up(nC * 8u);
+    v.offE = v.rsum + up(nC * 8u);
+    v.fE = v.offE + up(rE * 4u);
+    v.offC = v.fE + up(rE * 8u);
+    v.total = v.offC + up(rC * 4u);
+    return v;
+}
 
 int build_plan(const moka_mesh_desc *d, Plan &out);
 
@@ -96,6 +124,8 @@
     const uint16_t *lvoe;
     int32_t maxPV, pvCap;
     int32_t tailPatch;
+    const uint32_t *crIdx, *crBlk;
+    int32_t crMaxUnits, crPatches;
 };
 
 inline int64_t lds_stage_bytes(int K, int ME, int ME2, int maxRows, int maxOwnE, int maxOwnC)
diff --git a/mpas-ocean.jl_amd/csrc/plan.cpp b/mpas-ocean.jl_amd/csrc/plan.cpp
--- a/mpas-ocean.jl_amd/csrc/plan.cpp
+++ b/mpas-ocean.jl_amd/csrc/plan.cpp
@@ -1,6 +1,7 @@
 #include <algorithm>
 #include <array>
 #include <cmath>
+#include <cstring>
 #include <new>
 #include <numeric>
 #include <queue>
@@ -507,6 +508,89 @@
         for (int q = 0; q < p.nPatches; ++q) p.maxOwnV = std::max(p.maxOwnV, p.patchVertStart[q + 1] - p.patchVertStart[q]);
     }
 
+    p.crIdx.clear(); p.crBlk.clear(); p.crMaxUnits = 0;
+    if (p.colOk && p.stateBytes == 8 && !d->cellClass && ME == 6 && ME2 == 10 && p.K <= 255) {
+        const uint64_t rowB = (uint64_t)p.K * 8;
+        std::vector<int32_t> idE(nE, -1), idC(nC, -1), rowsE, rowsC;
+        auto rowE = [&](int e) { if (idE[e] < 0) { idE[e] = (int32_t)rowsE.size(); rowsE.push_back(e); } return idE[e]; };
+        auto rowC = [&](int c) { if (idC[c] < 0) { idC[c] = (int32_t)rowsC.size(); rowsC.push_back(c); } return idC[c]; };
+        bool ok = true;
+        p.crIdx.assign((size_t)p.nPatches * 4, 0u);
+        for (int q = 0; q < p.nPatches && ok; ++q) {
+            const int c0 = p.patchCellStart[q], c1 = p.patchCellStart[q + 1], e0 = p.patchEdgeStart[q], e1 = p.patchEdgeStart[q + 1];
+            rowsE.clear(); rowsC.clear();
+            for (int e = e0; e < e1; ++e) rowE(e);
+            for (int c = c0; c < c1; ++c) rowC(c);
+            for (int c = c0; c < c1; ++c)
+                for (int i = 0; i < ME; ++i)
+                    if (p.eoc[IX(i, c, ME)] >= 0) { rowE(p.eoc[IX(i, c, ME)]); rowC(p.coc[IX(i, c, ME)]); }
+            for (int e = e0; e < e1; ++e)
+                for (int i = 0; i < ME2; ++i)
+                    if (p.eoe[IX(i, e, ME2)] >= 0) rowE(p.eoe[IX(i, e, ME2)]);
+            if (rowsE.size() > 255 || rowsC.size() > 255) ok = false;
+            if (ok) {
+                const uint32_t nOE = (uint32_t)(e1 - e0), nOC = (uint32_t)(c1 - c0);
+                const CompactCarve v = compact_carve(nOE, nOC, (uint32_t)rowsE.size(), (uint32_t)rowsC.size(), ME, ME2);
+                const size_t base = p.crBlk.size();
+                p.crBlk.resize(base + v.total / 4, 0u);
+                unsigned char *b = reinterpret_cast<unsigned char *>(p.crBlk.data() + base);
+                auto put = [&](uint32_t off, const void *src, size_t n) { std::memcpy(b + off, src, n); };
+                for (int e = e0; e < e1; ++e) {
+                    const uint32_t j = (uint32_t)(e - e0);
+                    unsigned char r[16] = {0};
+                    uint16_t mask = 0;
+                    for (int i = 0; i < ME2; ++i) {
+                        const int x = p.eoe[IX(i, e, ME2)];
+                        if (x >= 0) mask |= (uint16_t)(1u << i);
+                        r[i] = (unsigned char)idE[x >= 0 ? x : e];
+                    }
+                    std::memcpy(r + 12, &mask, 2);
+                    r[14] = (unsigned char)p.ehdr[4 * (size_t)e + 3];
+                    put(v.e16 + j * 16, r, 16);
+                    put(v.woe + j * ME2 * 8, &p.woe[IX(0, e, ME2)], (size_t)ME2 * 8);
+                    put(v.g + j * 8, &p.gInvDc[e], 8);
+                    put(v.ecell + j * 8, &p.ehdr[4 * (size_t)e], 8);
+                }
+                for (int c = c0; c < c1; ++c) {
+                    const uint32_t j = (uint32_t)(c - c0);
+                    unsigned char r[16] = {0};
+                    unsigned char mask = 0, all = 1;
+                    for (int i = 0; i < ME; ++i) {
+                        const int e = p.eoc[IX(i, c, ME)];
+                        if (e >= 0) {
+                            mask |= (unsigned char)(1u << i);
+                            if (p.mltc[IX(i, c, ME)] < p.K) all = 0;
+                        }
+                        r[i] = (unsigned char)idE[e >= 0 ? e : p.eoc[IX(0, c, ME)]];
+                        r[ME + i] = (unsigned char)idC[e >= 0 ? p.coc[IX(i, c, ME)] : c];
+                    }
+                    r[12] = mask;
+                    r[13] = all;
+                    put(v.c16 + j * 16, r, 16);
+                    put(v.sdv + j * ME * 8, &p.sdv[IX(0, c, ME)], (size_t)ME * 8);
+                    put(v.invA + j * 8, &p.invArea[c], 8);
+                    put(v.rsum + j * 8, &p.rsum[c], 8);
+                }
+                for (size_t k = 0; k < rowsE.size(); ++k) {
+                    const uint32_t off = (uint32_t)((uint64_t)rowsE[k] * rowB);
+                    put(v.offE + (uint32_t)k * 4, &off, 4);
+                    put(v.fE + (uint32_t)k * 8, &p.fEdge[rowsE[k]], 8);
+                }
+                for (size_t k = 0; k < rowsC.size(); ++k) {
+                    const uint32_t off = (uint32_t)((uint64_t)rowsC[k] * rowB);
+                    put(v.offC + (uint32_t)k * 4, &off, 4);
+                }
+                uint32_t *ix = &p.crIdx[(size_t)q * 4];
+                ix[0] = (uint32_t)(base / 4); ix[1] = v.total / 16; ix[2] = (uint32_t)rowsE.size(); ix[3] = (uint32_t)rowsC.size();
+                p.crMaxUnits = std::max(p.crMaxUnits, (int32_t)(v.total / 16));
+                ok = base / 4 + v.total / 16 < (1ull << 32);
+            }
+            for (int e : rowsE) idE[e] = -1;
+            for (int c : rowsC) idC[c] = -1;
+        }
+        if (!ok) { p.crIdx.clear(); p.crBlk.clear(); p.crMaxUnits = 0; }
+    }
+
     p.haloStart.assign(p.nPatches + 1, 0);
     p.haloEdge.clear();
     p.leoc.assign((size_t)nC * 8, 0xFF);
@@ -656,6 +740,7 @@
     info->meshBytesDevice =
         (int64_t)p.nC * (p.ME * (3 * 4 + 8) + 3 * 8) + (int64_t)p.nE * (16 + p.ME2 * 12 + 4 * 8) +
         (int64_t)p.nV * p.VD * 12 + (int64_t)(p.nPatches + 1) * 12 + 4ll * (p.nC + p.nE + p.nV);
+    info->compactRecordBytes = (int64_t)(p.crBlk.size() + p.crIdx.size()) * 4;
 }
 
 int moka_plan_info(const moka_plan *plan, moka_mesh_info *info)
@@ -714,7 +799,7 @@
         VEC(MOKA_PA_HALO_START, haloStart) VEC(MOKA_PA_HALO_EDGE, haloEdge) VEC(MOKA_PA_LEOC, leoc) VEC(MOKA_PA_LEOE, leoe)
         VEC(MOKA_PA_CREC, cRec) VEC(MOKA_PA_EREC, eRec) VEC(MOKA_PA_FEOE, feoe)
         VEC(MOKA_PA_PVSTART, pvStart) VEC(MOKA_PA_PVLIST, pvList) VEC(MOKA_PA_LVOE, lvoe)
-        VEC(MOKA_PA_NLEV, nLev)
+        VEC(MOKA_PA_NLEV, nLev) VEC(MOKA_PA_CR_IDX, crIdx) VEC(MOKA_PA_CR_BLK, crBlk)
         default: moka::set_error("unknown plan array id"); return MOKA_ERR_ARG;
     }
 #undef VEC
diff --git a/mpas-ocean.jl_amd/moka_hip/lib.py b/mpas-ocean.jl_amd/moka_hip/lib.py
--- a/mpas-ocean.jl_amd/moka_hip/lib.py
+++ b/mpas-ocean.jl_amd/moka_hip/lib.py
@@ -67,6 +67,7 @@
         ("meshBytesDevice", C.c_int64), ("cellBandwidth", C.c_int64),
         ("maxPatchRows", C.c_int32), ("ldsBytesPerBlock", C.c_int32),
         ("maxPatchCells", C.c_int32), ("maxPatchEdges", C.c_int32),
+        ("compactRecordBytes", C.c_int64),
     ]
 
     def as_dict(self):
@@ -92,7 +93,7 @@
     "moka_rk4_dist_stage_launch", "moka_rk4_dist_step", "moka_fe_dist_launch", "moka_fe_dist_end", "moka_fe_dist_step",
     "moka_set_nonlinear", "moka_last_fe_path", "moka_set_viscosity_del2", "moka_set_viscosity_del4", "moka_state_del4_path", "moka_tape_create", "moka_tape_destroy", "moka_step_fe_taped", "moka_step_rk4_taped", "moka_adjoint_seed_sum_sq_ssh", "moka_adjoint_sweep",
     "moka_adjoint_download",
-    "moka_mark", "moka_marks_reset", "moka_marks_read", "moka_bw_probe", "moka_bw_probe_streams", "moka_bw_probe_reread", "moka_bw_probe_gather_big", "moka_ctx_pci_bus_id", "moka_halo_set_acquire", "moka_set_tuning", "moka_get_tuning", "moka_rk4_dist_parts_available", "moka_adjoint_rk4_stage_part", "moka_adjoint_rk4_parts_available", "moka_adjoint_rk4_stage_out_fields",
+    "moka_mark", "moka_marks_reset", "moka_marks_read", "moka_bw_probe", "moka_bw_probe_streams", "moka_bw_probe_reread", "moka_bw_probe_gather_big", "moka_ctx_pci_bus_id", "moka_halo_set_acquire", "moka_set_tuning", "moka_get_tuning", "moka_set_stage_records", "moka_get_stage_records", "moka_last_stage_records", "moka_rk4_dist_parts_available", "moka_adjoint_rk4_stage_part", "moka_adjoint_rk4_parts_available", "moka_adjoint_rk4_stage_out_fields",
     "moka_gradient_on_edge_vjp", "moka_gradient_on_edge_jvp", "moka_divergence_on_cell_vjp", "moka_divergence_on_cell_jvp",
     "moka_curl_on_vertex_vjp", "moka_curl_on_vertex_jvp", "moka_fe_lazy_pending",
     "moka_state_optimize_placement", "moka_state_placement_log", "moka_state_download_rows",
@@ -304,6 +305,9 @@
     L.moka_ctx_pci_bus_id.argtypes = [vp, C.c_char_p, C.c_int32]
     L.moka_set_tuning.argtypes = [C.c_int, C.c_int]
     L.moka_get_tuning.argtypes = [C.c_int, C.POINTER(C.c_int)]
+    L.moka_set_stage_records.argtypes = [C.c_int]
+    L.moka_get_stage_records.argtypes = [C.POINTER(C.c_int)]
+    L.moka_last_stage_records.argtypes = [C.c_int, C.POINTER(C.c_int)]
     _lib = L
     return L
 
@@ -312,6 +316,19 @@
     if rc != OK:
         msg = lib().moka_last_error(ctx)
         raise MokaError(rc, msg.decode() if msg else "unknown")
+
+
+def set_stage_records(form):
+    old = C.c_int()
+    check(lib().moka_get_stage_records(C.byref(old)))
+    check(lib().moka_set_stage_records(int(form)))
+    return old.value
+
+
+def last_stage_records(mode):
+    v = C.c_int()
+    check(lib().moka_last_stage_records(int(mode), C.byref(v)))
+    return v.value
 
 
 def f64(a):
@@ -375,7 +392,7 @@
     "haloStart": (16, np.int32), "haloEdge": (17, np.int32), "leoc": (18, np.uint8), "leoe": (19, np.uint8),
     "cRec": (20, np.uint32), "eRec": (21, np.uint32), "feoe": (22, np.float64),
     "pvStart": (23, np.int32), "pvList": (24, np.int32), "lvoe": (25, np.uint16),
-    "nLev": (26, np.int32),
+    "nLev": (26, np.int32), "crIdx": (27, np.uint32), "crBlk": (28, np.uint32),
 }
 
 
@@ -429,6 +446,8 @@
         which, dt = PLAN_ARRAYS[name]
         ptr, cnt = C.c_void_p(), C.c_int64()
         check(lib().moka_plan_array(self._h, which, C.byref(ptr), C.byref(cnt)))
+        if not cnt.value:
+            return np.empty(0, dtype=dt)
         buf = (C.c_char * (cnt.value * np.dtype(dt).itemsize)).from_address(ptr.value)
         return np.frombuffer(buf, dtype=dt).copy()
 
```

Result: faster. 9.330 billion, median of 6 (+1.7%).
